# DethRaid/AndroidRenderer

Measured on AMD Instinct MI355X. Metric: lit Mpixels/sec (deferred+GI pass) at 4K, higher is better.
Workload: dtype f32

## Files before the change

androidrenderer_amd/_abi.py:

```python
import ctypes as C

SAH_OK = 0
SAH_ERR_INVALID_ARGUMENT = -1
SAH_ERR_UNSUPPORTED_FORMAT = -2
SAH_ERR_HIP = -3
SAH_ERR_NO_DEVICE = -4
SAH_ERR_COMM = -5
SAH_ERR_UNSUPPORTED = -6

FORMAT_R8_UNORM = 9
FORMAT_R8G8B8A8_UNORM = 37
FORMAT_R8G8B8A8_SRGB = 43
FORMAT_R16_SFLOAT = 76
FORMAT_R16G16_SFLOAT = 83
FORMAT_R16G16B16A16_SFLOAT = 97
FORMAT_R32_SFLOAT = 100
FORMAT_B10G11R11_UFLOAT_PACK32 = 122
FORMAT_D16_UNORM = 124
FORMAT_D32_SFLOAT = 126
FORMAT_R8_UINT = 13

FORMAT_BPP = {9: 1, 13: 1, 37: 4, 43: 4, 76: 2, 83: 4, 97: 8, 100: 4, 122: 4, 124: 2, 126: 4}

SHADOW_MODE_OFF, SHADOW_MODE_CSM, SHADOW_MODE_RT = 0, 1, 2
GI_NONE, GI_LPV, GI_CACHE, GI_RTGI = 0, 1, 2, 3
LIGHTING_QUIRK_SUN_BLEND = 1 << 0
LIGHTING_BRUTE_FORCE_LIGHTS = 1 << 1
LIGHTING_DEFAULT_FLAGS = LIGHTING_QUIRK_SUN_BLEND
MAX_BLOOM_MIPS = 8
TONEMAP_TOLERANCE_1CODE = 1 << 0
GENERATION_TRACKED = 0xFFFFFFFF


class Plane(C.Structure):
    _fields_ = [("ptr", C.c_void_p), ("width", C.c_uint32), ("height", C.c_uint32), ("row_pitch_bytes", C.c_uint32),
                ("format", C.c_uint32)]


class Volume(C.Structure):
    _fields_ = [("ptr", C.c_void_p), ("width", C.c_uint32), ("height", C.c_uint32), ("depth", C.c_uint32),
                ("row_pitch_bytes", C.c_uint32), ("slice_pitch_bytes", C.c_uint32), ("format", C.c_uint32)]


TAA_HISTORY_INVALID, TAA_HDR_WEIGHTS = 1, 2


class TaaParams(C.Structure):
    _fields_ = [("blend", C.c_float), ("jitter", C.c_float * 2), ("previous_jitter", C.c_float * 2), ("flags", C.c_uint32)]


class SsaoParams(C.Structure):
    _fields_ = [("radius", C.c_float), ("max_radius_pixels", C.c_float), ("shadow_multiplier", C.c_float), ("shadow_clamp", C.c_float),
                ("horizon_angle_threshold", C.c_float), ("fade_out_from", C.c_float), ("fade_out_to", C.c_float), ("edge_sharpness", C.c_float),
                ("blur_passes", C.c_uint32), ("flags", C.c_uint32)]

    @classmethod
    def default(cls, **changes):
        values = dict(radius=8.0, max_radius_pixels=32.0, shadow_multiplier=1.0, shadow_clamp=0.98, horizon_angle_threshold=0.06, fade_out_from=50.0,
                      fade_out_to=300.0, edge_sharpness=50.0, blur_passes=2, flags=0)
        values.update(changes)
        return cls(**values)


EXPOSURE_HISTORY_INVALID = 1


class ExposureParams(C.Structure):
    _fields_ = [("key", C.c_float), ("low_fraction", C.c_float), ("high_fraction", C.c_float), ("min_exposure", C.c_float), ("max_exposure", C.c_float),
                ("adaptation", C.c_float), ("max_workgroups", C.c_uint32), ("flags", C.c_uint32)]

    @classmethod
    def default(cls, **changes):
        values = dict(key=0.18, low_fraction=0.5, high_fraction=0.95, min_exposure=1.0 / 64.0, max_exposure=64.0, adaptation=1.0, max_workgroups=0, flags=0)
        values.update(changes)
        return cls(**values)


class ExposureState(C.Structure):
    _fields_ = [("exposure", C.c_float), ("adapted", C.c_float), ("metered", C.c_uint32), ("window", C.c_uint32)]


RT_DENOISE_HISTORY_INVALID = 1


class RtDenoiseParams(C.Structure):
    _fields_ = [("max_history", C.c_float), ("depth_tolerance", C.c_float), ("depth_sharpness", C.c_float), ("normal_squarings", C.c_uint32),
                ("passes", C.c_uint32), ("jitter", C.c_float * 2), ("previous_jitter", C.c_float * 2), ("flags", C.c_uint32)]

    @classmethod
    def default(cls, **changes):
        values = dict(max_history=32.0, depth_tolerance=0.1, depth_sharpness=50.0, normal_squarings=5, passes=3, jitter=(0.0, 0.0),
                      previous_jitter=(0.0, 0.0), flags=0)
        values.update(changes)
        for k in ("jitter", "previous_jitter"):
            values[k] = (C.c_float * 2)(*values[k])
        return cls(**values)


class RtDenoiseDesc(C.Structure):
    PLANES = ("noisy", "depth", "normals", "motion_vectors", "previous_depth", "history", "history_length", "accum_out", "length_out", "denoised")
    _fields_ = [(name, C.POINTER(Plane)) for name in PLANES]

    @classmethod
    def of(cls, **planes):
        unknown = set(planes) - set(cls.PLANES)
        if unknown:
            raise TypeError(f"not planes of sah_rt_denoise_desc: {sorted(unknown)}")
        self = cls()
        self._planes = dict(planes)
        for name, p in planes.items():
            if p is not None:
                setattr(self, name, C.pointer(p))
        return self


RTGI_DENOISE_HISTORY_INVALID = 1
FORMAT_R32G32_SFLOAT = 103
FORMAT_R32G32B32A32_SFLOAT = 109
FORMAT_BPP.update({FORMAT_R32G32_SFLOAT: 8, FORMAT_R32G32B32A32_SFLOAT: 16})


class RtgiDenoiseParams(C.Structure):
    _fields_ = [("max_history", C.c_float), ("min_history", C.c_float), ("depth_tolerance", C.c_float), ("depth_sharpness", C.c_float),
                ("normal_squarings", C.c_uint32), ("passes", C.c_uint32), ("luminance_sigma", C.c_float), ("luminance_floor", C.c_float),
                ("jitter", C.c_float * 2), ("previous_jitter", C.c_float * 2), ("flags", C.c_uint32)]

    @classmethod
    def default(cls, **changes):
        values = dict(max_history=32.0, min_history=4.0, depth_tolerance=0.1, depth_sharpness=50.0, normal_squarings=5, passes=3, luminance_sigma=4.0,
                      luminance_floor=1e-6, jitter=(0.0, 0.0), previous_jitter=(0.0, 0.0), flags=0)
        values.update(changes)
        for k in ("jitter", "previous_jitter"):
            values[k] = (C.c_float * 2)(*values[k])
        return cls(**values)


class RtgiDenoiseDesc(C.Structure):
    PLANES = ("ray_buffer", "ray_irradiance", "depth", "normals", "motion_vectors", "previous_depth", "history", "history_moments", "accum_out",
              "moments_out", "denoised_ray_buffer", "denoised_irradiance")
    _fields_ = [(name, C.POINTER(Plane)) for name in PLANES]

    @classmethod
    def of(cls, **planes):
        unknown = set(planes) - set(cls.PLANES)
        if unknown:
            raise TypeError(f"not planes of sah_rtgi_denoise_desc: {sorted(unknown)}")
        self = cls()
        self._planes = dict(planes)
        for name, p in planes.items():
            if p is not None:
                setattr(self, name, C.pointer(p))
        return self


class TaaUpscaleParams(C.Structure):
    _fields_ = [("blend", C.c_float), ("min_confidence", C.c_float), ("jitter", C.c_float * 2), ("previous_jitter", C.c_float * 2), ("flags", C.c_uint32)]


class ShadingRateParams(C.Structure):
    _fields_ = [("contrast_image_resolution", C.c_uint32 * 2), ("shading_rate_image_resolution", C.c_uint32 * 2), ("max_rate", C.c_uint32 * 2),
                ("num_shading_rates", C.c_uint32), ("rates", (C.c_uint32 * 2) * 8)]


class ProbeAtlases(C.Structure):
    _fields_ = [("rtgi", Volume), ("light_cache", Volume), ("depth", Volume), ("average", Volume), ("validity", Volume)]


PRIMITIVE_TYPE_SOLID, PRIMITIVE_TYPE_CUTOUT = 0, 1
RASTER_STATS_WORDS = 8
RT_STATS_WORDS = 4
IPC_HANDLE_BYTES = 128


class VertexData(C.Structure):
    _fields_ = [("normal", C.c_float * 3), ("tangent", C.c_float * 4), ("texcoord", C.c_float * 2), ("color", C.c_uint32)]


class Material(C.Structure):
    _fields_ = [("base_color_tint", C.c_float * 4), ("emission_factor", C.c_float * 4), ("metalness_factor", C.c_float),
                ("roughness_factor", C.c_float), ("opacity_threshold", C.c_float), ("padding1", C.c_float),
                ("base_color_texel", C.c_float * 4), ("normal_texel", C.c_float * 4), ("data_texel", C.c_float * 4),
                ("emission_texel", C.c_float * 4)]


class Primitive(C.Structure):
    _fields_ = [("model", C.c_float * 16), ("first_index", C.c_uint32), ("index_count", C.c_uint32), ("vertex_offset", C.c_int32),
                ("type", C.c_uint32), ("material", C.c_uint32), ("padding", C.c_uint32 * 3)]


FILTER_NEAREST, FILTER_LINEAR = 0, 1
ADDRESS_REPEAT, ADDRESS_MIRRORED_REPEAT, ADDRESS_CLAMP_TO_EDGE = 0, 1, 2
MAX_TEXTURE_MIPS = 14
TEXTURE_NONE = 0xFFFFFFFF


class Sampler(C.Structure):
    _fields_ = [("mag_filter", C.c_uint32), ("min_filter", C.c_uint32), ("mipmap_mode", C.c_uint32), ("address_u", C.c_uint32),
                ("address_v", C.c_uint32), ("mip_lod_bias", C.c_float), ("min_lod", C.c_float), ("max_lod", C.c_float),
                ("max_anisotropy", C.c_float), ("reserved", C.c_uint32)]


class Texture(C.Structure):
    _fields_ = [("mips", Plane * MAX_TEXTURE_MIPS), ("num_mips", C.c_uint32), ("padding", C.c_uint32), ("sampler", Sampler)]


class MaterialTextures(C.Structure):
    _fields_ = [("base_color", C.c_uint32), ("normal", C.c_uint32), ("data", C.c_uint32), ("emission", C.c_uint32)]


class SceneGeometry(C.Structure):
    _fields_ = [("vertex_positions", C.c_void_p), ("vertex_data", C.c_void_p), ("indices", C.c_void_p), ("primitives", C.c_void_p),
                ("materials", C.c_void_p), ("num_vertices", C.c_uint32), ("num_indices", C.c_uint32), ("num_primitives", C.c_uint32),
                ("num_materials", C.c_uint32), ("textures", C.c_void_p), ("material_textures", C.c_void_p), ("num_textures", C.c_uint32),
                ("padding", C.c_uint32)]


class RsmTargets(C.Structure):
    _fields_ = [("flux", Volume), ("normals", Volume), ("depth", Volume)]


class GBuffer(C.Structure):
    _fields_ = [("color", Plane), ("normals", Plane), ("data", Plane), ("emission", Plane), ("depth", Plane)]


class MipChain(C.Structure):
    _fields_ = [("mips", Plane * MAX_BLOOM_MIPS), ("num_mips", C.c_uint32)]


class ViewData(C.Structure):
    _fields_ = [("view", C.c_float * 16), ("projection", C.c_float * 16), ("inverse_view", C.c_float * 16),
                ("inverse_projection", C.c_float * 16), ("last_frame_view", C.c_float * 16),
                ("last_frame_projection", C.c_float * 16), ("frustum", C.c_float * 4), ("z_near", C.c_float),
                ("material_texture_mip_bias", C.c_float), ("render_resolution", C.c_float * 2), ("jitter", C.c_float * 2),
                ("previous_jitter", C.c_float * 2)]


class SunLightConstants(C.Structure):
    _fields_ = [("direction_and_tan_size", C.c_float * 4), ("color", C.c_float * 4), ("csm_resolution", C.c_uint32 * 4),
                ("data", (C.c_float * 4) * 4), ("cascade_matrices", (C.c_float * 16) * 4),
                ("cascade_inverse_matrices", (C.c_float * 16) * 4), ("shadow_mode", C.c_uint32),
                ("num_shadow_samples", C.c_float), ("padding1", C.c_uint32), ("padding2", C.c_uint32)]


class LpvCascadeMatrices(C.Structure):
    _fields_ = [("rsm_vp", C.c_float * 16), ("inverse_rsm_vp", C.c_float * 16), ("world_to_cascade", C.c_float * 16),
                ("cascade_to_world", C.c_float * 16)]


class ProbeCascade(C.Structure):
    _fields_ = [("min", C.c_float * 3), ("probe_spacing", C.c_float)]


class GI(C.Structure):
    _fields_ = [("kind", C.c_uint32),
                ("lpv_red", Volume), ("lpv_green", Volume), ("lpv_blue", Volume),
                ("lpv_cascades", C.POINTER(LpvCascadeMatrices)), ("lpv_num_cascades", C.c_uint32), ("lpv_exposure", C.c_float),
                ("probe_irradiance", Volume), ("probe_depth", Volume), ("probe_validity", Volume),
                ("probe_cascades", ProbeCascade * 4), ("probe_size", C.c_uint32 * 2), ("cache_debug_mode", C.c_uint32),
                ("ray_buffer", Plane), ("ray_irradiance", Plane), ("noise", Plane), ("num_extra_rays", C.c_uint32),
                ("extra_ray_radius", C.c_float), ("lpv_generation", C.c_uint32), ("probe_generation", C.c_uint32)]


class SkyLuts(C.Structure):
    _fields_ = [("transmittance", Plane), ("sky_view", Plane)]


class PointLight(C.Structure):
    _fields_ = [("position", C.c_float * 3), ("radius", C.c_float), ("color", C.c_float * 3), ("intensity", C.c_float)]


class LightList(C.Structure):
    _fields_ = [("lights", C.c_void_p), ("count", C.c_uint32)]


class LightingDesc(C.Structure):
    _fields_ = [("gbuffer", C.POINTER(GBuffer)), ("ao", C.POINTER(Plane)), ("lit", C.POINTER(Plane)),
                ("view", C.POINTER(ViewData)), ("sun", C.POINTER(SunLightConstants)), ("shadowmap", C.POINTER(Volume)),
                ("shadow_mask", C.POINTER(Plane)), ("lights", C.POINTER(LightList)), ("gi", C.POINTER(GI)),
                ("sky", C.POINTER(SkyLuts)), ("flags", C.c_uint32), ("row_begin", C.c_uint32), ("row_end", C.c_uint32)]


class ChainPlan(C.Structure):
    _fields_ = [("aa_rows", C.c_uint32 * 2), ("mip0_rows", C.c_uint32 * 2), ("mip1_rows", C.c_uint32 * 2), ("out_rows", C.c_uint32 * 2),
                ("mip1_rows_per_rank", C.c_uint32), ("mip1_allocated_rows", C.c_uint32), ("rows_per_rank", C.c_uint32),
                ("out_allocated_rows", C.c_uint32)]


class ChainFrame(C.Structure):
    _fields_ = [("lighting", C.POINTER(LightingDesc) * 2), ("lit", Plane), ("antialiased", Plane), ("bloom", MipChain), ("out", Plane)]


CHAIN_NO_EXCHANGE = 1 << 0
CHAIN_CAPTURE = 1 << 1

assert C.sizeof(ViewData) == 432
assert C.sizeof(SunLightConstants) == 640
assert C.sizeof(LpvCascadeMatrices) == 256
assert C.sizeof(ProbeCascade) == 16
assert C.sizeof(PointLight) == 32


class ProbeTraceDesc(C.Structure):
    _fields_ = [("cascades", ProbeCascade * 4), ("probes_to_update", C.c_void_p), ("num_probes", C.c_uint32),
                ("sun", C.POINTER(SunLightConstants)), ("sky", C.POINTER(SkyLuts)), ("noise", C.POINTER(Plane)),
                ("probe_irradiance", Volume), ("probe_depth", Volume), ("probe_validity", Volume), ("probe_size", C.c_uint32 * 2),
                ("trace_results", Volume)]
```

androidrenderer_amd/csrc/api.cpp:

```cpp
#include <dlfcn.h>
#include <hip/hip_runtime.h>

#include <cmath>
#include <cstdarg>
#include <cstdio>
#include <cstdlib>
#include <cstring>
#include <string>
#include <vector>

#include "../../include/sah_hip.h"
#include "ctx.hpp"
#include "fast_pixel_map.hpp"
#include "launch.hpp"

namespace {

bool vec_ok(const sah_plane* p, uint32_t bytes) { return ((uintptr_t)p->ptr % bytes) == 0 && (p->row_pitch_bytes % bytes) == 0; }

void normalize3(const float in[3], float out[3]) {
    const float d = in[0] * in[0] + in[1] * in[1] + in[2] * in[2];
    const float inv = 1.0f / std::sqrt(d);
    for (int i = 0; i < 3; i++) out[i] = in[i] * inv;
}
void cross3(const float a[3], const float b[3], float o[3]) {
    o[0] = a[1] * b[2] - b[1] * a[2];
    o[1] = a[2] * b[0] - b[2] * a[0];
    o[2] = a[0] * b[1] - b[0] * a[1];
}
float round_to_half(float f) { return (float)(_Float16)f; }

bool is_zero(float x) { return x == 0.0f; }
bool all_finite(const float* m, int n) {
    for (int i = 0; i < n; i++)
        if (!std::isfinite(m[i])) return false;
    return true;
}
bool all_bounded(const float* m, int n) {
    for (int i = 0; i < n; i++)
        if (!(std::fabs(m[i]) <= 0x1p+40f)) return false;
    return true;
}

}

namespace sah {
namespace {


enum DispatchField {
    kDispFamily, kDispPpt, kDispPosDivNr, kDispNcascPow2, kDispRowMagic, kDispSkyRatio, kDispSkyWorkgroups, kDispTiledFastGeom, kDispTiledFastLpv,
    kDispRepack, kDispTableRebuilt, kDispPosDivShared, kDispFields
};
static_assert(kDispFields == sizeof(sah_ctx::last_dispatch) / sizeof(uint32_t), "sah_debug_lighting_dispatch reports uint32_t[12]");

struct LightingCall {
    uint32_t W, H, r0, r1;
    uint32_t sun_mode, gi_kind;
    bool vec4ok;
};

int lighting_targets(sah_ctx* ctx, const sah_lighting_desc* d, LightingCall& call, LightingArgs& a) {
    if (!d->gbuffer || !d->lit || !d->view) return fail(ctx, SAH_ERR_INVALID_ARGUMENT, "gbuffer, lit and view are required");
    const sah_gbuffer& g = *d->gbuffer;
    const uint32_t W = d->lit->width, H = d->lit->height;
    if (W == 0 || H == 0) return fail(ctx, SAH_ERR_INVALID_ARGUMENT, "empty render target");
    if (!plane_ok(d->lit, SAH_FORMAT_R16G16B16A16_SFLOAT, SAH_FORMAT_R16G16B16A16_SFLOAT, W, H))
        return fail(ctx, SAH_ERR_UNSUPPORTED_FORMAT, "lit must be R16G16B16A16_SFLOAT");
    if (!plane_ok(&g.color, SAH_FORMAT_R8G8B8A8_SRGB, SAH_FORMAT_R8G8B8A8_SRGB, W, H) ||
        !plane_ok(&g.normals, SAH_FORMAT_R16G16B16A16_SFLOAT, SAH_FORMAT_R16G16B16A16_SFLOAT, W, H) ||
        !plane_ok(&g.data, SAH_FORMAT_R8G8B8A8_UNORM, SAH_FORMAT_R8G8B8A8_UNORM, W, H) ||
        !plane_ok(&g.emission, SAH_FORMAT_R8G8B8A8_SRGB, SAH_FORMAT_R8G8B8A8_SRGB, W, H) ||
        !plane_ok(&g.depth, SAH_FORMAT_D32_SFLOAT, SAH_FORMAT_R32_SFLOAT, W, H))
        return fail(ctx, SAH_ERR_UNSUPPORTED_FORMAT, "g-buffer planes must match the reference formats and the lit extent");
    uint32_t r0 = d->row_begin, r1 = d->row_end;
    if (r0 == 0 && r1 == 0) r1 = H;
    if (r1 > H || r0 > r1) return fail(ctx, SAH_ERR_INVALID_ARGUMENT, "row range [%u,%u) outside image height %u", r0, r1, H);

    const uint32_t sun_mode = d->sun ? d->sun->shadow_mode : SAH_SHADOW_MODE_OFF;
    if (sun_mode > SAH_SHADOW_MODE_RT) return fail(ctx, SAH_ERR_INVALID_ARGUMENT, "bad shadow_mode %u", sun_mode);
    const uint32_t gi_kind = d->gi ? d->gi->kind : SAH_GI_NONE;
    if (gi_kind > SAH_GI_RTGI) return fail(ctx, SAH_ERR_INVALID_ARGUMENT, "bad gi kind %u", gi_kind);
    if ((d->sky || d->lights) && !d->sun) return fail(ctx, SAH_ERR_INVALID_ARGUMENT, "sun constants are required with sky");

    memset(&a, 0, sizeof(a));
    a.color = parg(&g.color);
    a.normals = parg(&g.normals);
    a.data = parg(&g.data);
    a.emission = parg(&g.emission);
    a.depth = parg(&g.depth);
    a.lit = parg(d->lit);
    a.width = W;
    a.height = H;
    a.row_begin = r0;
    a.row_end = r1;
    a.flags = d->flags;
    a.res[0] = d->view->render_resolution[0];
    a.res[1] = d->view->render_resolution[1];
    memcpy(a.inv_proj, d->view->inverse_projection, 64);
    memcpy(a.inv_view, d->view->inverse_view, 64);
    for (int i = 0; i < 3; i++) a.view_pos[i] = -d->view->view[12 + i];
    a.luts = ctx->luts;
    if (d->sun) {
        const float neg[3] = {-d->sun->direction_and_tan_size[0], -d->sun->direction_and_tan_size[1], -d->sun->direction_and_tan_size[2]};
        normalize3(neg, a.sun_L);
        for (int i = 0; i < 3; i++) a.sun_color[i] = d->sun->color[i];
    }
    bool vec4ok = (W % 4 == 0) && vec_ok(&g.color, 16) && vec_ok(&g.normals, 16) && vec_ok(&g.data, 16) && vec_ok(&g.emission, 16) &&
                  vec_ok(&g.depth, 16) && vec_ok(d->lit, 16);

    if (gi_kind == SAH_GI_LPV && d->ao && d->ao->ptr) {
        if (!plane_ok(d->ao, SAH_FORMAT_R32_SFLOAT, SAH_FORMAT_R32_SFLOAT, W, H)) return fail(ctx, SAH_ERR_UNSUPPORTED_FORMAT, "ao must be R32_SFLOAT");
        a.ao = parg(d->ao);
        a.has_ao = 1;
        vec4ok = vec4ok && vec_ok(d->ao, 16);
    }
    if (sun_mode == SAH_SHADOW_MODE_RT && d->shadow_mask && d->shadow_mask->ptr) {
        if (!plane_ok(d->shadow_mask, SAH_FORMAT_R32_SFLOAT, SAH_FORMAT_R32_SFLOAT, W, H))
            return fail(ctx, SAH_ERR_UNSUPPORTED_FORMAT, "shadow_mask must be R32_SFLOAT");
        a.shadow_mask = parg(d->shadow_mask);
        a.has_mask = 1;
        vec4ok = vec4ok && vec_ok(d->shadow_mask, 16);
    }
    call = LightingCall{W, H, r0, r1, sun_mode, gi_kind, vec4ok};
    return SAH_OK;
}

int lighting_csm(sah_ctx* ctx, const sah_lighting_desc* d, const LightingCall& call, CsmArgs& csm) {
    memset(&csm, 0, sizeof(csm));
    if (call.sun_mode != SAH_SHADOW_MODE_CSM) return SAH_OK;
    if (d->shadowmap && d->shadowmap->ptr) {
        if (d->shadowmap->format != SAH_FORMAT_D16_UNORM && d->shadowmap->format != SAH_FORMAT_D32_SFLOAT)
            return fail(ctx, SAH_ERR_UNSUPPORTED_FORMAT, "shadowmap must be D16_UNORM or D32_SFLOAT");
        if (d->shadowmap->depth < 4) return fail(ctx, SAH_ERR_INVALID_ARGUMENT, "shadowmap needs 4 layers");
        csm.shadowmap = varg(*d->shadowmap);
        csm.is_d16 = d->shadowmap->format == SAH_FORMAT_D16_UNORM;
        csm.d16_recip = 1.0f / 65535.0f;
        static const bool recip_ok = [] {
            const float y = 1.0f / 65535.0f;
            for (uint32_t i = 0; i < 65536; i++) {
                const float v = (float)i;
                const float q = v * y;
                const float q2 = std::fmaf(std::fmaf(-q, 65535.0f, v), y, q);
                if (q2 != v / 65535.0f) return false;
            }
            return true;
        }();
        csm.d16_recip_ok = recip_ok;
    }
    for (int c = 0; c < 4; c++) {
        csm.splits[c] = d->sun->data[c][0];
        const float* M = d->sun->cascade_matrices[c];
        for (int col = 0; col < 4; col++) {
            const float* m = M + col * 4;
            csm.biased[c][col * 4 + 0] = ((0.5f * m[0] + 0.0f * m[1]) + 0.0f * m[2]) + 0.5f * m[3];
            csm.biased[c][col * 4 + 1] = ((0.0f * m[0] + 0.5f * m[1]) + 0.0f * m[2]) + 0.5f * m[3];
            csm.biased[c][col * 4 + 2] = ((0.0f * m[0] + 0.0f * m[1]) + 1.0f * m[2]) + 0.0f * m[3];
            csm.biased[c][col * 4 + 3] = ((0.0f * m[0] + 0.0f * m[1]) + 0.0f * m[2]) + 1.0f * m[3];
        }
    }
    return SAH_OK;
}

int lighting_gi_lpv(sah_ctx* ctx, const sah_lighting_desc* d, const LightingCall& call, LpvArgs& lpv) {
    memset(&lpv, 0, sizeof(lpv));
    if (call.gi_kind != SAH_GI_LPV) return SAH_OK;
    const sah_gi& gi = *d->gi;
    if (gi.lpv_num_cascades == 0 || gi.lpv_num_cascades > 4 || !gi.lpv_cascades)
        return fail(ctx, SAH_ERR_INVALID_ARGUMENT, "LPV needs 1..4 cascades and their matrices");
    const sah_volume* vols[3] = {&gi.lpv_red, &gi.lpv_green, &gi.lpv_blue};
    for (const sah_volume* v : vols) {
        if (!v->ptr || v->format != SAH_FORMAT_R16G16B16A16_SFLOAT) return fail(ctx, SAH_ERR_UNSUPPORTED_FORMAT, "LPV volumes must be RGBA16F");
        if ((uint64_t)v->row_pitch_bytes < (uint64_t)v->width * 8 || (uint64_t)v->slice_pitch_bytes < (uint64_t)v->row_pitch_bytes * v->height)
            return fail(ctx, SAH_ERR_INVALID_ARGUMENT, "LPV volume pitches too small");
    }
    lpv.red = varg(gi.lpv_red);
    lpv.green = varg(gi.lpv_green);
    lpv.blue = varg(gi.lpv_blue);
    for (uint32_t c = 0; c < gi.lpv_num_cascades; c++) memcpy(lpv.world_to_cascade[c], gi.lpv_cascades[c].world_to_cascade, 64);
    lpv.num_cascades = gi.lpv_num_cascades;
    lpv.num_cascades_f = (float)gi.lpv_num_cascades;
    lpv.exposure = gi.lpv_exposure;
    return SAH_OK;
}

int lighting_irr32_copy(sah_ctx* ctx, const sah_gi& gi, CacheArgs& cache) {
    if (cache.hot_ok) {
        const size_t need = 4 * (size_t)((uint64_t)gi.probe_irradiance.slice_pitch_bytes * gi.probe_irradiance.depth);
        const hipError_t ge = ctx->irr32_copy.reserve(ctx->stream, ctx->cache_epoch, need);
        if (ge == hipErrorOutOfMemory) {
            (void)hipGetLastError();
            cache.hot_ok = 0;
        } else {
            HIP_TRY(ctx, ge);
        }
    }
    if (cache.hot_ok) {
        if (!ctx->irr32_copy.reusable_for(gi.probe_generation, cache.irradiance)) {
            HIP_TRY(ctx, launch_probe_irr_unpack(cache.irradiance, ctx->irr32_copy.data(), ctx->stream));
            ctx->dbg_irr_unpacks++;
            ctx->irr32_copy.rebuilt(ctx->cache_epoch, gi.probe_generation, cache.irradiance);
        }
        cache.irr32 = ctx->irr32_copy.data();
    }
    return SAH_OK;
}

int lighting_gi_cache(sah_ctx* ctx, const sah_lighting_desc* d, const LightingCall& call, CacheArgs& cache) {
    memset(&cache, 0, sizeof(cache));
    if (call.gi_kind != SAH_GI_CACHE) return SAH_OK;
    const sah_gi& gi = *d->gi;
    if (!gi.probe_irradiance.ptr || gi.probe_irradiance.format != SAH_FORMAT_B10G11R11_UFLOAT_PACK32 || !gi.probe_depth.ptr ||
        gi.probe_depth.format != SAH_FORMAT_R16G16_SFLOAT || !gi.probe_validity.ptr || gi.probe_validity.format != SAH_FORMAT_R8_UNORM)
        return fail(ctx, SAH_ERR_UNSUPPORTED_FORMAT, "probe atlases must be B10G11R11 / R16G16F / R8_UNORM arrays");
    cache.irradiance = varg(gi.probe_irradiance);
    cache.depth = varg(gi.probe_depth);
    cache.validity = varg(gi.probe_validity);
    for (int c = 0; c < 4; c++) {
        const float ext[3] = {32.f, 8.f, 32.f};
        for (int i = 0; i < 3; i++) {
            cache.cascade_min[c][i] = gi.probe_cascades[c].min[i];
            cache.cascade_max[c][i] = gi.probe_cascades[c].min[i] + ext[i] * gi.probe_cascades[c].probe_spacing;
        }
        cache.spacing[c] = gi.probe_cascades[c].probe_spacing;
    }
    cache.spacing_pow2 = 1;
    for (int c = 0; c < 4; c++) {
        int e = 0;
        const float sp = cache.spacing[c], m = frexpf(sp, &e);
        cache.spacing_pow2 = cache.spacing_pow2 && m == 0.5f && e > -60 && e < 60;
        cache.inv_spacing[c] = 1.0f / sp;
    }
    cache.probe_size[0] = gi.probe_size[0];
    cache.probe_size[1] = gi.probe_size[1];
    for (int i = 0; i < 2; i++) cache.inv_tex[i] = 1.0f / (((float)gi.probe_size[i] + 2.0f) * 32.0f);
    cache.debug_mode = gi.cache_debug_mode;
    auto bytes = [](const sah_volume& v) { return (uint64_t)v.slice_pitch_bytes * v.depth; };
    cache.hot_ok = bytes(gi.probe_irradiance) < (1ull << 32) && bytes(gi.probe_depth) < (1ull << 32) && bytes(gi.probe_validity) < (1ull << 32) &&
                   gi.probe_validity.width <= 32 && gi.probe_validity.height <= 32 && gi.probe_validity.depth <= 32 &&
                   gi.probe_size[0] >= 1 && gi.probe_size[0] <= 30 && gi.probe_size[1] >= 1 && gi.probe_size[1] <= 30 &&
                   gi.probe_irradiance.width == 32u * (gi.probe_size[0] + 2u) && gi.probe_irradiance.height == 32u * (gi.probe_size[1] + 2u) &&
                   gi.probe_depth.width == 32u * 12u && gi.probe_depth.height == 32u * 12u &&
                   bytes(gi.probe_irradiance) < (1ull << 30) && gi.probe_irradiance.row_pitch_bytes % 4 == 0 && gi.probe_irradiance.slice_pitch_bytes % 4 == 0 &&
                   ((uintptr_t)gi.probe_irradiance.ptr % 4) == 0;
    return lighting_irr32_copy(ctx, gi, cache);
}

int lighting_gi_rtgi(sah_ctx* ctx, const sah_lighting_desc* d, const LightingCall& call, RtgiArgs& rtgi) {
    memset(&rtgi, 0, sizeof(rtgi));
    if (call.gi_kind != SAH_GI_RTGI) return SAH_OK;
    const sah_gi& gi = *d->gi;
    if (!plane_ok(&gi.ray_buffer, SAH_FORMAT_R16G16B16A16_SFLOAT, SAH_FORMAT_R16G16B16A16_SFLOAT, call.W, call.H) ||
        !plane_ok(&gi.ray_irradiance, SAH_FORMAT_R16G16B16A16_SFLOAT, SAH_FORMAT_R16G16B16A16_SFLOAT, call.W, call.H))
        return fail(ctx, SAH_ERR_UNSUPPORTED_FORMAT, "ray_buffer / ray_irradiance must be RGBA16F at render resolution");
    rtgi.ray_buffer = parg(&gi.ray_buffer);
    rtgi.ray_irradiance = parg(&gi.ray_irradiance);
    if (gi.num_extra_rays) {
        if (!gi.noise.ptr || gi.noise.format != SAH_FORMAT_R8G8B8A8_UNORM || gi.noise.width < 128 || gi.noise.height < 128)
            return fail(ctx, SAH_ERR_UNSUPPORTED_FORMAT, "noise must be R8G8B8A8_UNORM, at least 128x128");
        rtgi.noise = parg(&gi.noise);
        rtgi.noise_w = gi.noise.width;
        rtgi.noise_h = gi.noise.height;
    }
    rtgi.num_extra_rays = gi.num_extra_rays;
    rtgi.extra_ray_radius = gi.extra_ray_radius;
    return SAH_OK;
}

int lighting_sky(sah_ctx* ctx, const sah_lighting_desc* d, SkyArgs& sky) {
    memset(&sky, 0, sizeof(sky));
    if (!d->sky) return SAH_OK;
    const float dirn[3] = {d->sun->direction_and_tan_size[0], d->sun->direction_and_tan_size[1], d->sun->direction_and_tan_size[2]};
    float nd[3];
    normalize3(dirn, nd);
    const float sun_dir[3] = {-nd[0], -nd[1], -nd[2]};
    if (!fill_sky_args(*d->sky, sun_dir, &sky)) return fail(ctx, SAH_ERR_UNSUPPORTED_FORMAT, "sky LUTs must be RGBA16F");
    return SAH_OK;
}

int lighting_ppt(const sah_ctx* ctx, const LightingCall& call) {
    const uint32_t W = call.W;
    int ppt = call.vec4ok ? 4 : 1;
    while (ppt > 1 && (uint64_t)(W / (uint32_t)ppt) * (call.r1 - call.r0) < 1536ull * 256ull) ppt /= 2;
    if (ctx->force_ppt == 1 || ctx->force_ppt == 2 || ctx->force_ppt == 4) {
        if (ctx->force_ppt == 1 || (call.vec4ok && W % ctx->force_ppt == 0)) ppt = ctx->force_ppt;
    }
    return ppt;
}


bool fast_view_ok(const sah_lighting_desc* d, FastArgs* f) {
    const float* P = d->view->inverse_projection;
    const float* V = d->view->inverse_view;
    if (!all_finite(P, 16) || !all_finite(V, 16)) return false;
    if (!std::isfinite(d->view->render_resolution[0]) || !std::isfinite(d->view->render_resolution[1])) return false;
    if (!(is_zero(P[4]) && is_zero(P[8]) && is_zero(P[1]) && is_zero(P[9]) && is_zero(P[2]) && is_zero(P[6]) && is_zero(P[3]) && is_zero(P[7])))
        return false;
    if (!(is_zero(V[3]) && is_zero(V[7]) && is_zero(V[11]) && V[15] == 1.0f)) return false;
    if (!all_bounded(d->view->view + 12, 3)) return false;
    f->p0 = P[0]; f->p12 = P[12]; f->p5 = P[5]; f->p13 = P[13];
    f->p10 = P[10]; f->p14 = P[14]; f->p11 = P[11]; f->p15 = P[15];
    auto in = [](float v, float lo, float hi) { return std::fabs(v) >= lo && std::fabs(v) <= hi; };
    const float r0 = d->view->render_resolution[0], r1 = d->view->render_resolution[1];
    const bool bounded = P[10] == 0.0f && P[12] == 0.0f && P[13] == 0.0f && in(P[0], 0x1p-16f, 0x1p+30f) && in(P[5], 0x1p-16f, 0x1p+30f) &&
                         in(P[14], 0x1p-40f, 0x1p+40f) && r0 > 0.f && r1 > 0.f && (float)d->lit->width <= 256.0f * r0 &&
                         (float)d->lit->height <= 256.0f * r1;
    f->pos_div_nr = bounded && !std::signbit(P[12]) && !std::signbit(P[13]);
    f->pos_div_shared = bounded && !f->pos_div_nr;
    return true;
}

bool fast_csm_ok(const CsmArgs& csm) {
    if (!csm.shadowmap.ptr || (uint64_t)csm.shadowmap.slice_pitch * csm.shadowmap.depth >= (1ull << 32)) return false;
    if (!csm.is_d16 || !csm.d16_recip_ok) return false;
    for (int c = 0; c < 4; c++) {
        const float* b = csm.biased[c];
        if (!all_bounded(b, 16)) return false;
        if (!(is_zero(b[3]) && is_zero(b[7]) && is_zero(b[11]) && b[15] == 1.0f)) return false;
    }
    return true;
}

bool fast_lpv_ok(const sah_gi& gi, FastArgs* f) {
    if (gi.lpv_red.width != gi.lpv_green.width || gi.lpv_red.width != gi.lpv_blue.width || gi.lpv_red.height != gi.lpv_green.height ||
        gi.lpv_red.height != gi.lpv_blue.height || gi.lpv_red.depth != gi.lpv_green.depth || gi.lpv_red.depth != gi.lpv_blue.depth ||
        gi.lpv_red.row_pitch_bytes != gi.lpv_green.row_pitch_bytes || gi.lpv_red.row_pitch_bytes != gi.lpv_blue.row_pitch_bytes ||
        gi.lpv_red.slice_pitch_bytes != gi.lpv_green.slice_pitch_bytes || gi.lpv_red.slice_pitch_bytes != gi.lpv_blue.slice_pitch_bytes ||
        (uint64_t)gi.lpv_red.slice_pitch_bytes * gi.lpv_red.depth >= (1ull << 32))
        return false;
    for (uint32_t c = 0; c < gi.lpv_num_cascades; c++) {
        const float* m = gi.lpv_cascades[c].world_to_cascade;
        if (!all_bounded(m, 16)) return false;
        if (!(is_zero(m[1]) && is_zero(m[2]) && is_zero(m[3]) && is_zero(m[4]) && is_zero(m[6]) && is_zero(m[7]) && is_zero(m[8]) &&
              is_zero(m[9]) && is_zero(m[11]) && m[15] == 1.0f))
            return false;
        if (is_zero(m[0]) || is_zero(m[5]) || is_zero(m[10])) return false;
        f->lpv_s[c][0] = m[0]; f->lpv_s[c][1] = m[5]; f->lpv_s[c][2] = m[10];
        f->lpv_t[c][0] = m[12]; f->lpv_t[c][1] = m[13]; f->lpv_t[c][2] = m[14];
    }
    const uint32_t n = gi.lpv_num_cascades;
    f->ncasc_pow2 = (n & (n - 1)) == 0;
    f->inv_ncasc = 1.0f / (float)n;
    return std::isfinite(gi.lpv_exposure);
}

struct FastPath {
    bool use_fast;
    bool tiled_fast_geom;
    bool tiled_fast_lpv;
    LightingFamily family;
};
FastPath detect_fast_path(const sah_ctx* ctx, const sah_lighting_desc* d, const LightingCall& call, const LightingArgs& a, const CsmArgs& csm, FastArgs* f) {
    memset(f, 0, sizeof(*f));
    const bool lpv_gi = call.gi_kind == SAH_GI_LPV;
    const bool fast_kind = (call.gi_kind == SAH_GI_NONE || lpv_gi) && a.num_lights == 0;
    const bool geom = !ctx->force_general && fast_view_ok(d, f) && (call.sun_mode != SAH_SHADOW_MODE_CSM || fast_csm_ok(csm));
    const bool lpv = geom && lpv_gi && (fast_kind || ctx->state) && fast_lpv_ok(*d->gi, f);
    FastPath p;
    p.use_fast = fast_kind && geom && (!lpv_gi || lpv);
    p.family = !fast_kind ? kLightingTiled : (p.use_fast ? kLightingFast : kLightingGeneral);
    p.tiled_fast_geom = !fast_kind && geom;
    p.tiled_fast_lpv = p.tiled_fast_geom && lpv;
    f->lpv_fast = p.tiled_fast_lpv ? 1u : 0u;
    return p;
}

int prepare_lpv_copy(sah_ctx* ctx, const sah_lighting_desc* d, const LpvArgs& lpv, FastArgs& fast) {
    SahLpvCopy& copy = ctx->lpv_copy;
    const SahLpvPackLayout pk = SahLpvCopy::layout(lpv.red.width, lpv.red.height, lpv.red.depth);
    if (pk.total >= (1ull << 32)) return fail(ctx, SAH_ERR_UNSUPPORTED, "LPV volumes too large for the packed gather copy");
    HIP_TRY(ctx, copy.reserve(ctx->stream, ctx->cache_epoch, pk.total));
    fast.lpv_packed = copy.data();
    fast.pk_row_pitch = pk.row_pitch;
    fast.pk_slice_pitch = pk.slice_pitch;
    const VolumeArg src[3] = {lpv.red, lpv.green, lpv.blue};
    const uint32_t gen = d->gi->lpv_generation;
    const bool reuse = copy.reusable_for(gen, src);
    fast.repack = reuse ? 0u : 1u;
    if (!reuse) {
        ctx->dbg_lpv_packs++;
        copy.rebuilt_by_pack(ctx->cache_epoch, gen, src, lpv.red.width, lpv.red.height, lpv.red.depth);
    }
    return SAH_OK;
}

int lighting_fast_layout(sah_ctx* ctx, const sah_lighting_desc* d, const LightingCall& call, int ppt, const LpvArgs& lpv, const SkyArgs& sky, FastArgs& fast) {
    const uint32_t W = call.W, r0 = call.r0, r1 = call.r1;
    const uint64_t groups = (uint64_t)(W / (uint32_t)ppt) * (r1 - r0);
    const uint32_t nseg = (uint32_t)((groups + 63) / 64);
    const uint32_t seg_stride = 64u * (uint32_t)ppt;
    const size_t codes_bytes = ((size_t)nseg * seg_stride + 255) & ~(size_t)255;
    const size_t need = codes_bytes + (size_t)nseg * sizeof(uint16_t) + 256;
    HIP_TRY(ctx, ctx->list.grow_in_epoch(ctx->stream, ctx->cache_epoch, need));
    fast.seg_list = (uint8_t*)ctx->list.ptr;
    fast.seg_count = (uint16_t*)((uint8_t*)ctx->list.ptr + codes_bytes);
    fast.num_segments = nseg;
    fast.seg_stride = seg_stride;
    if (call.gi_kind == SAH_GI_LPV && r1 > r0) {
        if (const int rc = prepare_lpv_copy(ctx, d, lpv, fast); rc != SAH_OK) return rc;
    }
    fast.sky_enabled = sky.enabled;
    {
        const uint64_t blocks = (groups + 255) / 256;
        const uint64_t want = (blocks + 511) / 512;
        fast.sky_ratio = (uint32_t)(want < 4 ? 4 : (want > 32 ? 32 : want));
        fast.sky_first = sky.enabled ? (uint32_t)((blocks + fast.sky_ratio - 1u) / fast.sky_ratio) : 0u;
    }
    {
        const uint64_t gpr = W / (uint32_t)ppt, threads = (gpr * (r1 - r0) + 255) / 256 * 256;
        fast.row_magic = (gpr >= 2 && threads * gpr < (1ull << 32)) ? (uint32_t)((1ull << 32) / gpr) + 1u : 0u;
    }
    fast.tile_rows = fast_tile_rows_for(call.sun_mode == SAH_SHADOW_MODE_CSM || call.gi_kind == SAH_GI_LPV, W, r1 - r0, (uint32_t)ppt);
    fast.state = ctx->state;
    fast.hint_slot = ctx->hint_slot;
    ctx->hint_slot ^= 1u;
    return SAH_OK;
}

int lighting_colx_table(sah_ctx* ctx, const LightingCall& call, const LightingArgs& a, const FastPath& path, int ppt, FastArgs& fast, bool* table_rebuilt) {
    const uint32_t W = call.W, H = call.H;
    const bool lit_px = call.sun_mode != SAH_SHADOW_MODE_OFF || call.gi_kind == SAH_GI_LPV;
    const bool geom_fast = path.use_fast && (call.sun_mode == SAH_SHADOW_MODE_CSM || call.gi_kind == SAH_GI_LPV);
    *table_rebuilt = false;
    if ((path.use_fast && ppt == 4 && lit_px) || (geom_fast && fast.pos_div_shared) || path.tiled_fast_geom) {
        const struct {
            float f[7];
            uint32_t width;
        } key = {{a.res[0], fast.p0, fast.p12, a.res[1], fast.p5, fast.p13, (float)H}, W};
        const uint32_t stride = (W + 63u) & ~63u, row_stride = (H + 63u) & ~63u;
        HIP_TRY(ctx, ctx->colx.prepare(ctx->stream, ctx->cache_epoch, ((size_t)2 * stride + 2 * row_stride) * sizeof(float), &key, sizeof(key), true, table_rebuilt));
        fast.state = ctx->state;
        if (*table_rebuilt) {
            HIP_TRY(ctx, launch_colx_table(a, fast, (float*)ctx->colx.buf.ptr, stride, row_stride, ctx->stream));
            ctx->colx.built(ctx->cache_epoch, &key, sizeof(key));
        }
        fast.colx_tab = (const float*)ctx->colx.buf.ptr;
        fast.colx_stride = stride;
        fast.rowy_stride = row_stride;
    }
    if (!fast.colx_tab || !ctx->state || !(geom_fast || path.tiled_fast_geom)) fast.pos_div_shared = 0u;
    return SAH_OK;
}

void lighting_report(sah_ctx* ctx, const LightingCall& call, const FastPath& path, int ppt, const FastArgs& fast, bool table_rebuilt) {
    uint32_t* w = ctx->last_dispatch;
    w[kDispFamily] = path.family;
    w[kDispPpt] = path.family == kLightingTiled ? 0u : (uint32_t)ppt;
    w[kDispPosDivNr] = (path.use_fast || path.tiled_fast_geom) ? fast.pos_div_nr : 0u;
    w[kDispNcascPow2] = ((path.use_fast && call.gi_kind == SAH_GI_LPV) || path.tiled_fast_lpv) ? fast.ncasc_pow2 : 0u;
    w[kDispRowMagic] = (path.use_fast && fast.row_magic != 0u) ? 1u : 0u;
    w[kDispSkyRatio] = path.use_fast ? fast.sky_ratio : 0u;
    w[kDispSkyWorkgroups] = path.use_fast ? fast.sky_first : 0u;
    w[kDispTiledFastGeom] = path.tiled_fast_geom ? 1u : 0u;
    w[kDispTiledFastLpv] = path.tiled_fast_lpv ? 1u : 0u;
    w[kDispRepack] = fast.repack;
    w[kDispTableRebuilt] = table_rebuilt ? 1u : 0u;
    w[kDispPosDivShared] = fast.pos_div_shared;
}

}
}

void SahRange::resolve(push_fn& push, pop_fn& pop) {
    const char* on = getenv("SAH_ROCTX");
    if (!on || atoi(on) == 0) return;
    for (const char* lib : {"librocprofiler-sdk-roctx.so", "librocprofiler-sdk-roctx.so.1", "libroctx64.so", "libroctx64.so.4"}) {
        void* h = dlopen(lib, RTLD_NOW | RTLD_GLOBAL);
        if (!h) continue;
        push = reinterpret_cast<push_fn>(dlsym(h, "roctxRangePushA"));
        pop = reinterpret_cast<pop_fn>(dlsym(h, "roctxRangePop"));
        if (push && pop) return;
        push = nullptr;
        pop = nullptr;
    }
}

extern "C" {

int sah_abi_version(void) { return SAH_ABI_VERSION; }

const char* sah_status_string(int s) {
    switch (s) {
        case SAH_OK: return "ok";
        case SAH_ERR_INVALID_ARGUMENT: return "invalid argument";
        case SAH_ERR_UNSUPPORTED_FORMAT: return "unsupported format";
        case SAH_ERR_HIP: return "HIP error";
        case SAH_ERR_NO_DEVICE: return "no HIP device";
        case SAH_ERR_COMM: return "communicator error";
        case SAH_ERR_UNSUPPORTED: return "unsupported";
    }
    return "unknown";
}

const char* sah_last_error(const sah_ctx* ctx) { return ctx ? ctx->last_error.c_str() : ""; }

int sah_comm_init(sah_ctx* ctx, const void* comm_id);
void sah_comm_destroy(sah_ctx* ctx);
void sah_ipc_destroy(sah_ctx* ctx);

int sah_create(sah_ctx** out, int device, int rank, int world, const void* comm_id) {
    if (!out || world < 1 || rank < 0 || rank >= world) return SAH_ERR_INVALID_ARGUMENT;
    *out = nullptr;
    int n = 0;
    if (hipGetDeviceCount(&n) != hipSuccess || n == 0) return SAH_ERR_NO_DEVICE;
    if (device < 0 || device >= n) return SAH_ERR_INVALID_ARGUMENT;
    sah_ctx* ctx = new sah_ctx();
    ctx->device = device;
    ctx->rank = rank;
    ctx->world = world;
    if (hipSetDevice(device) != hipSuccess) { delete ctx; return SAH_ERR_HIP; }
    if (hipStreamCreateWithFlags(&ctx->stream, hipStreamNonBlocking) != hipSuccess) { delete ctx; return SAH_ERR_HIP; }
    ctx->own_stream = true;
    float host[512];
    for (int i = 0; i < 256; i++) {
        const double c = (double)i / 255.0;
        host[i] = (float)((c <= 0.04045) ? c / 12.92 : std::pow((c + 0.055) / 1.055, 2.4));
        host[256 + i] = (float)i / 255.0f;
    }
    if (hipMalloc((void**)&ctx->luts, sizeof(host)) != hipSuccess ||
        hipMemcpy(ctx->luts, host, sizeof(host), hipMemcpyHostToDevice) != hipSuccess) {
        sah_destroy(ctx);
        return SAH_ERR_HIP;
    }
    if (comm_id) {
        int rc = sah_comm_init(ctx, comm_id);
        if (rc != SAH_OK) { sah_destroy(ctx); return rc; }
    }
    if (hipMalloc((void**)&ctx->state, sizeof(sah::FrameState)) != hipSuccess ||
        hipMemset(ctx->state, 0, sizeof(sah::FrameState)) != hipSuccess) {
        sah_destroy(ctx);
        return SAH_ERR_HIP;
    }
    if (ctx->mip_chain_counter.create() != hipSuccess) {
        sah_destroy(ctx);
        return SAH_ERR_HIP;
    }
    const char* mc = getenv("SAH_RASTER_MERGE_CAPACITY");
    if (mc) ctx->raster_merge_cap = (uint32_t)atoi(mc);
    *out = ctx;
    return SAH_OK;
}

int sah_debug_create_detached(sah_ctx** out) {
    if (!out) return SAH_ERR_INVALID_ARGUMENT;
    *out = nullptr;
    int n = 0;
    if (hipGetDeviceCount(&n) == hipSuccess && n > 0) return SAH_ERR_UNSUPPORTED;
    (void)hipGetLastError();
    sah_ctx* ctx = new sah_ctx();
    ctx->device = -1;
    *out = ctx;
    return SAH_OK;
}

void sah_destroy(sah_ctx* ctx) {
    if (!ctx) return;
    (void)hipSetDevice(ctx->device);
    sah_comm_destroy(ctx);
    sah_ipc_destroy(ctx);
    if (ctx->comm_ready) (void)hipEventDestroy(ctx->comm_ready);
    if (ctx->comm_done) (void)hipEventDestroy(ctx->comm_done);
    if (ctx->luts) (void)hipFree(ctx->luts);
    if (ctx->probe_slots) (void)hipFree(ctx->probe_slots);
    if (ctx->probe_done) (void)hipEventDestroy(ctx->probe_done);
    if (ctx->state) (void)hipFree(ctx->state);
    std::vector<SahBuffer*> buffers = {&ctx->list, &ctx->lpv_copy.buf, &ctx->gv_keys, &ctx->gv_factors, &ctx->ml_scratch, &ctx->irr32_copy.buf, &ctx->colx.buf, &ctx->tm_axis.buf};
    for (SahBuffer& b : ctx->raster.buf) buffers.push_back(&b);
    for (SahBuffer& b : ctx->rt.buf) buffers.push_back(&b);
    for (SahBuffer* b : buffers) b->release();
    ctx->tm_codes.release();
    ctx->mip_chain_counter.release();
    for (SahCacheGuard* g : {&ctx->guard_lighting, &ctx->guard_tonemap, &ctx->guard_raster, &ctx->guard_rt, &ctx->guard_mip_chain})
        if (g->done) (void)hipEventDestroy(g->done);
    if (ctx->raster.half_to_srgb8) (void)hipFree(ctx->raster.half_to_srgb8);
    if (ctx->raster.host_counters) (void)hipHostFree(ctx->raster.host_counters);
    if (ctx->own_stream && ctx->stream) (void)hipStreamDestroy(ctx->stream);
    delete ctx;
}

int sah_set_stream(sah_ctx* ctx, void* hip_stream) {
    if (!ctx) return SAH_ERR_INVALID_ARGUMENT;
    if ((hipStream_t)hip_stream == ctx->stream && !ctx->own_stream) return SAH_OK;
    const bool drained = ctx->own_stream && ctx->stream;
    if (drained) (void)hipStreamSynchronize(ctx->stream);
    SahCacheGuard* guards[] = {&ctx->guard_lighting, &ctx->guard_tonemap, &ctx->guard_raster, &ctx->guard_rt, &ctx->guard_mip_chain};
    for (SahCacheGuard* g : guards) HIP_TRY(ctx, sah_guard_leave(ctx, *g, drained));
    if (drained) (void)hipStreamDestroy(ctx->stream);
    ctx->stream = (hipStream_t)hip_stream;
    ctx->own_stream = false;
    return SAH_OK;
}

void* sah_get_stream(sah_ctx* ctx) { return ctx ? (void*)ctx->stream : nullptr; }

int sah_debug_set(sah_ctx* ctx, int force_general, int force_ppt) {
    if (!ctx) return SAH_ERR_INVALID_ARGUMENT;
    ctx->force_general = force_general != 0;
    ctx->force_ppt = force_ppt;
    return SAH_OK;
}

int sah_debug_deferred_pixels(sah_ctx* ctx, uint64_t* out) {
    if (!ctx || !out) return SAH_ERR_INVALID_ARGUMENT;
    *out = 0;
    if (!ctx->last_seg_count || !ctx->last_num_segments) return SAH_OK;
    HIP_TRY(ctx, hipSetDevice(ctx->device));
    HIP_TRY(ctx, hipStreamSynchronize(ctx->stream));
    std::vector<uint16_t> counts(ctx->last_num_segments);
    HIP_TRY(ctx, hipMemcpy(counts.data(), ctx->last_seg_count, counts.size() * sizeof(uint16_t), hipMemcpyDeviceToHost));
    uint64_t n = 0;
    for (uint16_t c : counts) n += c;
    *out = n;
    return SAH_OK;
}

int sah_debug_copy_rebuilds(sah_ctx* ctx, uint32_t out[2]) {
    if (!ctx || !out) return SAH_ERR_INVALID_ARGUMENT;
    out[0] = ctx->dbg_lpv_packs;
    out[1] = ctx->dbg_irr_unpacks;
    return SAH_OK;
}

int sah_debug_cache_epoch(sah_ctx* ctx, uint64_t* out) {
    if (!ctx || !out) return SAH_ERR_INVALID_ARGUMENT;
    *out = ctx->cache_epoch;
    return SAH_OK;
}

int sah_debug_lighting_dispatch(sah_ctx* ctx, uint32_t out[12]) {
    if (!ctx || !out) return SAH_ERR_INVALID_ARGUMENT;
    memcpy(out, ctx->last_dispatch, sizeof(ctx->last_dispatch));
    if (out[sah::kDispPosDivShared] && ctx->state) {
        uint32_t neg_zero = 0;
        HIP_TRY(ctx, hipSetDevice(ctx->device));
        HIP_TRY(ctx, hipStreamSynchronize(ctx->stream));
        HIP_TRY(ctx, hipMemcpy(&neg_zero, &ctx->state->colx_neg_zero, sizeof(neg_zero), hipMemcpyDeviceToHost));
        out[sah::kDispPosDivShared] = neg_zero == 0u ? 1u : 0u;
    }
    return SAH_OK;
}

int sah_sync(sah_ctx* ctx) {
    if (!ctx) return SAH_ERR_INVALID_ARGUMENT;
    HIP_TRY(ctx, hipStreamSynchronize(ctx->stream));
    if (ctx->comm_stream && ctx->comm_stream != ctx->stream) HIP_TRY(ctx, hipStreamSynchronize(ctx->comm_stream));
    if (sah_ipc_timed_out(ctx)) return fail(ctx, SAH_ERR_COMM, "direct exchange: a peer did not arrive within 2 s; the gathered rows are not valid");
    return SAH_OK;
}

int sah_lighting(sah_ctx* ctx, const sah_lighting_desc* d) {
    SAH_RANGE();
    using namespace sah;
    if (!ctx || !d) return SAH_ERR_INVALID_ARGUMENT;
    memset(ctx->last_dispatch, 0, sizeof(ctx->last_dispatch));
    LightingCall call;
    LightingArgs a;
    CsmArgs csm;
    LpvArgs lpv;
    CacheArgs cache;
    RtgiArgs rtgi;
    SkyArgs sky;
    if (const int rc = lighting_targets(ctx, d, call, a); rc != SAH_OK) return rc;
    if (const int rc = lighting_csm(ctx, d, call, csm); rc != SAH_OK) return rc;
    if (const int rc = lighting_gi_lpv(ctx, d, call, lpv); rc != SAH_OK) return rc;
    if (const int rc = lighting_gi_cache(ctx, d, call, cache); rc != SAH_OK) return rc;
    if (const int rc = lighting_gi_rtgi(ctx, d, call, rtgi); rc != SAH_OK) return rc;
    if (const int rc = lighting_sky(ctx, d, sky); rc != SAH_OK) return rc;
    const int ppt = lighting_ppt(ctx, call);
    if (d->lights && d->lights->count) {
        if (!d->lights->lights) return fail(ctx, SAH_ERR_INVALID_ARGUMENT, "light list pointer is null");
        a.lights = d->lights->lights;
        a.num_lights = d->lights->count;
    }
    HIP_TRY(ctx, hipSetDevice(ctx->device));
    HIP_TRY(ctx, sah_guard_touch(ctx, ctx->guard_lighting));
    FastArgs fast;
    const FastPath path = detect_fast_path(ctx, d, call, a, csm, &fast);
    if (path.tiled_fast_lpv && call.r1 > call.r0) {
        if (const int rc = prepare_lpv_copy(ctx, d, lpv, fast); rc != SAH_OK) return rc;
        fast.state = ctx->state;
    }
    if (path.use_fast) {
        if (const int rc = lighting_fast_layout(ctx, d, call, ppt, lpv, sky, fast); rc != SAH_OK) return rc;
    }
    bool table_rebuilt = false;
    if (const int rc = lighting_colx_table(ctx, call, a, path, ppt, fast, &table_rebuilt); rc != SAH_OK) return rc;
    lighting_report(ctx, call, path, ppt, fast, table_rebuilt);
    HIP_TRY(ctx, launch_lighting(a, csm, lpv, cache, rtgi, sky, path.family, (path.use_fast || path.tiled_fast_geom) ? &fast : nullptr, (int)call.sun_mode,
                                 (int)call.gi_kind, ppt, (d->flags & SAH_LIGHTING_BRUTE_FORCE_LIGHTS) != 0, ctx->stream));
    if (path.use_fast) {
        ctx->last_seg_count = fast.seg_count;
        ctx->last_num_segments = fast.num_segments;
    } else {
        ctx->last_seg_count = nullptr;
        ctx->last_num_segments = 0;
    }
    return SAH_OK;
}

}
```

androidrenderer_amd/csrc/ctx.hpp:

```cpp
#pragma once
#include <hip/hip_runtime.h>

#include <cstdarg>
#include <cstdio>
#include <string>
#include <vector>

#include "../../include/sah_hip.h"
#include "ctx_cache.hpp"
#include "params.hpp"
#include "rt_args.hpp"

struct SahCacheGuard {
    hipEvent_t done = nullptr;
    hipStream_t last = nullptr;
    bool used = false, closed = false;
};

struct sah_ctx {
    int device = 0;
    int rank = 0, world = 1;
    hipStream_t stream = nullptr;
    bool own_stream = false;
    float* luts = nullptr;
    uint32_t* probe_slots = nullptr;
    hipEvent_t probe_done = nullptr;
    hipStream_t probe_stream = nullptr;
    bool lpv_tables_built = false;
    bool lpv_hot_structure = false;
    void* comm = nullptr;
    void* comm_reversed = nullptr;
    void* rccl = nullptr;
    hipStream_t comm_stream = nullptr;
    hipEvent_t comm_ready = nullptr, comm_done = nullptr;
    bool comm_pending = false;
    int force_ppt = 0;
    bool force_general = false;
    sah::FrameState* state = nullptr;
    SahBuffer list;
    SahBuffer gv_keys;
    SahBuffer gv_factors;
    SahBuffer ml_scratch;
    SahLpvCopy lpv_copy;
    SahIrr32Copy irr32_copy;
    SahKeyedTable colx;
    SahKeyedTable tm_axis;
    SahTonemapCodeTables tm_codes;
    SahTicketCounter mip_chain_counter;
    uint64_t cache_epoch = 0;
    uint32_t hint_slot = 0;
    uint32_t dbg_lpv_packs = 0, dbg_irr_unpacks = 0;
    const uint16_t* last_seg_count = nullptr;
    uint32_t last_num_segments = 0;
    uint32_t last_dispatch[12] = {};
    struct RasterScratch {
        SahBuffer buf[16];
        uint8_t* half_to_srgb8 = nullptr;
        uint32_t* host_counters = nullptr;
        uint32_t last_pass[4] = {};
    } raster;
    struct RtState {
        SahBuffer buf[7];
        sah::RtBvh bvh = {};
        sah::RtScene scene = {};
        bool built = false;
        bool refitted = false;
        uint32_t row_begin = 0, row_end = 0;
        uint32_t num_bounces = 0;
    } rt;
    struct IpcState {
        bool open = false, connected = false;
        uint32_t* mailbox = nullptr;
        uint32_t* peer_mailbox[SAH_IPC_MAX_WORLD] = {};
        uint32_t* timed_out = nullptr;
        struct Mapping {
            unsigned char handle[64];
            void* base;
            uint32_t users;
        };
        std::vector<Mapping> mappings;
        struct Buffer {
            bool in_use = false;
            uint8_t* local = nullptr;
            uint64_t bytes = 0;
            uint8_t* peer[SAH_IPC_MAX_WORLD] = {};
            unsigned char peer_handle[SAH_IPC_MAX_WORLD][SAH_IPC_HANDLE_BYTES] = {};
            uint32_t seq = 0;
        } buffers[SAH_IPC_MAX_BUFFERS];
    } ipc;
    SahCacheGuard guard_lighting, guard_tonemap, guard_raster, guard_rt, guard_mip_chain;
    uint32_t raster_merge_cap = 2048;
    std::string last_error;
};

struct SahRange {
    using push_fn = int (*)(const char*);
    using pop_fn = int (*)();
    static void resolve(push_fn& push, pop_fn& pop);
    explicit SahRange(const char* name) {
        static push_fn push = nullptr;
        static pop_fn pop_ = nullptr;
        static bool tried = false;
        if (!tried) {
            tried = true;
            resolve(push, pop_);
        }
        pop = pop_;
        if (push) push(name);
    }
    ~SahRange() {
        if (pop) pop();
    }
    pop_fn pop = nullptr;
};
#define SAH_RANGE() SahRange sah_range_(__func__)

inline int fail(sah_ctx* ctx, int code, const char* fmt, ...) {
    char buf[512];
    va_list ap;
    va_start(ap, fmt);
    vsnprintf(buf, sizeof(buf), fmt, ap);
    va_end(ap);
    if (ctx) ctx->last_error = buf;
    return code;
}

inline hipError_t sah_guard_touch(sah_ctx* ctx, SahCacheGuard& g) {
    hipError_t e = hipSuccess;
    if (g.used && g.closed && g.last != ctx->stream) e = hipStreamWaitEvent(ctx->stream, g.done, 0);
    g.used = true;
    g.closed = false;
    g.last = ctx->stream;
    return e;
}
inline hipError_t sah_guard_leave(sah_ctx* ctx, SahCacheGuard& g, bool drained) {
    if (!g.used || g.closed || g.last != ctx->stream) return hipSuccess;
    if (drained) {
        g.used = false;
        return hipSuccess;
    }
    hipError_t e = hipSuccess;
    if (!g.done) e = hipEventCreateWithFlags(&g.done, hipEventDisableTiming);
    if (e == hipSuccess) e = hipEventRecord(g.done, ctx->stream);
    g.closed = e == hipSuccess;
    return e;
}

#define HIP_TRY(ctx, expr)                                                                          \
    do {                                                                                            \
        hipError_t e_ = (expr);                                                                     \
        if (e_ != hipSuccess) return fail(ctx, SAH_ERR_HIP, "%s: %s", #expr, hipGetErrorString(e_)); \
    } while (0)

inline bool fill_sky_args(const sah_sky_luts& s, const float sun_dir[3], sah::SkyArgs* sky) {
    if (!s.transmittance.ptr || !s.sky_view.ptr || s.transmittance.format != SAH_FORMAT_R16G16B16A16_SFLOAT || s.sky_view.format != SAH_FORMAT_R16G16B16A16_SFLOAT)
        return false;
    auto cross3 = [](const float a[3], const float b[3], float o[3]) {
        o[0] = a[1] * b[2] - b[1] * a[2];
        o[1] = a[2] * b[0] - b[2] * a[0];
        o[2] = a[0] * b[1] - b[0] * a[1];
    };
    sky->enabled = 1;
    sky->transmittance = sah::PlaneArg{(const uint8_t*)s.transmittance.ptr, s.transmittance.row_pitch_bytes};
    sky->sky_view = sah::PlaneArg{(const uint8_t*)s.sky_view.ptr, s.sky_view.row_pitch_bytes};
    sky->t_w = s.transmittance.width;
    sky->t_h = s.transmittance.height;
    sky->s_w = s.sky_view.width;
    sky->s_h = s.sky_view.height;
    const float sky_pi = 3.14159265358f;
    const float ground = 6.360f;
    for (int i = 0; i < 3; i++) sky->sun_dir[i] = sun_dir[i];
    sky->view_pos_y = 6.360f + 0.0002f;
    sky->height = __builtin_sqrtf((0.0f * 0.0f + sky->view_pos_y * sky->view_pos_y) + 0.0f * 0.0f);
    sky->up_y = sky->view_pos_y / sky->height;
    {
        float q = __builtin_sqrtf(sky->height * sky->height - ground * ground) / sky->height;
        q = __builtin_fminf(__builtin_fmaxf(q, -1.0f), 1.0f);
        sky->horizon_angle = (float)__builtin_acos((double)q);
    }
    sky->azimuth_limit = 0.5f * sky_pi - .0001f;
    sky->min_sun_cos = (float)__builtin_cos((double)(0.53f * sky_pi / 180.0f));
    const float up[3] = {0.0f / sky->height, sky->up_y, 0.0f / sky->height};
    cross3(sky->sun_dir, up, sky->right);
    cross3(up, sky->right, sky->forward);
    sky->smooth_e0 = (float)(_Float16)0.002f;
    return true;
}

inline uint32_t format_bpp(uint32_t f) {
    switch (f) {
        case SAH_FORMAT_R8_UNORM: return 1;
        case SAH_FORMAT_R16_SFLOAT: case SAH_FORMAT_D16_UNORM: return 2;
        case SAH_FORMAT_R8G8B8A8_UNORM: case SAH_FORMAT_R8G8B8A8_SRGB: case SAH_FORMAT_R16G16_SFLOAT: case SAH_FORMAT_R32_SFLOAT:
        case SAH_FORMAT_B10G11R11_UFLOAT_PACK32: case SAH_FORMAT_D32_SFLOAT: return 4;
        case SAH_FORMAT_R16G16B16A16_SFLOAT: return 8;
    }
    return 0;
}

inline bool plane_ok(const sah_plane* p, uint32_t fmt_a, uint32_t fmt_b, uint32_t w, uint32_t h) {
    if (!p || !p->ptr) return false;
    if (p->format != fmt_a && p->format != fmt_b) return false;
    if (p->width != w || p->height != h) return false;
    return (uint64_t)p->row_pitch_bytes >= (uint64_t)w * format_bpp(p->format);
}

inline bool rgba16f_ok(const sah_plane* p) {
    return p && p->ptr && p->format == SAH_FORMAT_R16G16B16A16_SFLOAT && p->width && p->height &&
           (uint64_t)p->row_pitch_bytes >= (uint64_t)p->width * 8 && ((uintptr_t)p->ptr % 8) == 0 && (p->row_pitch_bytes % 8) == 0;
}

inline sah::PlaneArg parg(const sah_plane* p) { return sah::PlaneArg{p ? (const uint8_t*)p->ptr : nullptr, p ? p->row_pitch_bytes : 0}; }
inline sah::VolumeArg varg(const sah_volume& v) {
    return sah::VolumeArg{(const uint8_t*)v.ptr, v.width, v.height, v.depth, v.row_pitch_bytes, v.slice_pitch_bytes};
}
```

androidrenderer_amd/csrc/ctx_cache.hpp:

```cpp
#pragma once
#include <hip/hip_runtime.h>

#include <cstring>

#include "../../include/sah_hip.h"
#include "params.hpp"

inline bool same_volume(const sah::VolumeArg& a, const sah::VolumeArg& b) {
    return a.ptr == b.ptr && a.width == b.width && a.height == b.height && a.depth == b.depth && a.row_pitch == b.row_pitch && a.slice_pitch == b.slice_pitch;
}

struct SahBuffer {
    void* ptr = nullptr;
    size_t bytes = 0;

    hipError_t grow(hipStream_t stream, size_t need, bool* grew = nullptr) {
        if (grew) *grew = false;
        if (bytes >= need) return hipSuccess;
        if (ptr) {
            const hipError_t e = hipStreamSynchronize(stream);
            if (e != hipSuccess) return e;
            (void)hipFree(ptr);
        }
        ptr = nullptr;
        bytes = 0;
        const hipError_t e = hipMalloc(&ptr, need);
        if (e != hipSuccess) return e;
        bytes = need;
        if (grew) *grew = true;
        return hipSuccess;
    }
    hipError_t grow_in_epoch(hipStream_t stream, uint64_t& cache_epoch, size_t need) {
        bool grew = false;
        const hipError_t e = grow(stream, need, &grew);
        if (grew) cache_epoch++;
        return e;
    }
    void release() {
        if (ptr) (void)hipFree(ptr);
        ptr = nullptr;
        bytes = 0;
    }
};

struct SahLpvPackLayout {
    uint32_t row_pitch, slice_pitch;
    uint64_t total;
};

struct SahLpvCopy {
    SahBuffer buf;
    uint32_t generation = 0;
    sah::VolumeArg source[3] = {};
    uint32_t extent[3] = {0, 0, 0};
    bool all_zero = false;

    uint8_t* data() const { return (uint8_t*)buf.ptr; }

    static SahLpvPackLayout layout(uint32_t w, uint32_t h, uint32_t d) {
        const uint64_t row = (uint64_t)(w + 2 * sah::kLpvPackBorder) * sah::kLpvPackTexel;
        const uint64_t slice = row * (h + 2 * sah::kLpvPackBorder);
        return {(uint32_t)row, (uint32_t)slice, slice * (d + 2 * sah::kLpvPackBorder) + 64};
    }
    void drop(uint64_t& cache_epoch) {
        if (generation != 0) cache_epoch++;
        generation = 0;
    }
    hipError_t reserve(hipStream_t stream, uint64_t& cache_epoch, uint64_t total) {
        if (buf.bytes >= total) return hipSuccess;
        const hipError_t e = buf.grow(stream, total);
        if (e != hipSuccess && buf.ptr) return e;
        generation = 0;
        cache_epoch++;
        if (e != hipSuccess) return e;
        extent[0] = extent[1] = extent[2] = 0;
        all_zero = true;
        return hipMemsetAsync(buf.ptr, 0, total, stream);
    }
    bool reusable_for(uint32_t gen, const sah::VolumeArg src[3]) const {
        return gen != 0 && gen == generation && same_volume(src[0], source[0]) && same_volume(src[1], source[1]) && same_volume(src[2], source[2]);
    }
    void rebuilt_by_pack(uint64_t& cache_epoch, uint32_t gen, const sah::VolumeArg src[3], uint32_t w, uint32_t h, uint32_t d) {
        if (gen != 0) cache_epoch++;
        generation = gen;
        for (int i = 0; i < 3; i++) source[i] = src[i];
        extent[0] = w, extent[1] = h, extent[2] = d;
        all_zero = false;
    }
    hipError_t borders_for(hipStream_t stream, uint32_t w, uint32_t h, uint32_t d, uint64_t total) {
        const bool same = extent[0] == w && extent[1] == h && extent[2] == d;
        hipError_t e = hipSuccess;
        if (!same && !all_zero) e = hipMemsetAsync(buf.ptr, 0, total, stream);
        extent[0] = w, extent[1] = h, extent[2] = d;
        all_zero = false;
        return e;
    }
    struct Rewrite {
        uint32_t generation;
        uint64_t epoch;
        sah::VolumeArg source[3];
    };
    Rewrite begin_rewrite(uint64_t& cache_epoch) {
        const Rewrite was = {generation, cache_epoch, {source[0], source[1], source[2]}};
        drop(cache_epoch);
        return was;
    }
    void commit_rewrite(uint64_t& cache_epoch, const Rewrite& was, const sah::VolumeArg* last) {
        if (last) {
            generation = SAH_GENERATION_TRACKED;
            for (int i = 0; i < 3; i++) source[i] = last[i];
        }
        bool same = last && was.generation == SAH_GENERATION_TRACKED;
        for (int i = 0; i < 3 && same; i++) same = same_volume(was.source[i], last[i]);
        if (same && cache_epoch == was.epoch + 1) cache_epoch = was.epoch;
        else if (!same && last && was.generation == 0) cache_epoch++;
    }
};

struct SahIrr32Copy {
    SahBuffer buf;
    uint32_t generation = 0;
    sah::VolumeArg source = {};

    uint8_t* data() const { return (uint8_t*)buf.ptr; }

    void drop(uint64_t& cache_epoch) {
        if (generation != 0) cache_epoch++;
        generation = 0;
    }
    hipError_t reserve(hipStream_t stream, uint64_t& cache_epoch, size_t need) {
        bool grew = false;
        const hipError_t e = buf.grow(stream, need, &grew);
        if (grew) {
            generation = 0;
            cache_epoch++;
        }
        return e;
    }
    bool reusable_for(uint32_t gen, const sah::VolumeArg& atlas) const { return gen != 0 && gen == generation && same_volume(atlas, source); }
    void rebuilt(uint64_t& cache_epoch, uint32_t gen, const sah::VolumeArg& atlas) {
        if (gen != 0) cache_epoch++;
        generation = gen;
        source = atlas;
    }
    bool patchable_for(const sah::VolumeArg& atlas) const { return buf.ptr && generation == SAH_GENERATION_TRACKED && same_volume(atlas, source); }
};

struct SahKeyedTable {
    SahBuffer buf;
    uint32_t key[20] = {};
    bool valid = false;

    hipError_t prepare(hipStream_t stream, uint64_t& cache_epoch, size_t need, const void* k, size_t k_bytes, bool new_buffer_in_epoch, bool* rebuild) {
        static_assert(sizeof(key) >= 7 * sizeof(float) + sizeof(uint32_t) && sizeof(key) >= 19 * sizeof(uint32_t), "the two keys in use");
        bool grew = false;
        const hipError_t e = buf.grow(stream, need, &grew);
        if (grew) {
            valid = false;
            if (new_buffer_in_epoch) cache_epoch++;
        }
        *rebuild = !valid || memcmp(k, key, k_bytes) != 0;
        return e;
    }
    void built(uint64_t& cache_epoch, const void* k, size_t k_bytes) {
        cache_epoch++;
        memcpy(key, k, k_bytes);
        valid = true;
    }
};

struct SahTicketCounter {
    uint32_t* word = nullptr;

    hipError_t create() {
        const hipError_t e = hipMalloc((void**)&word, sizeof(uint32_t));
        return e != hipSuccess ? e : hipMemset(word, 0, sizeof(uint32_t));
    }
    void release() {
        if (word) (void)hipFree(word);
        word = nullptr;
    }
};

struct SahTonemapCodeTables {
    float* thresholds = nullptr;
    float* code_table = nullptr;
    uint32_t bucket_base = 0, bucket_count = 0;
    float thr_lo = 0.f, thr_hi = 0.f;

    bool ready() const { return thresholds && code_table; }
    void publish(uint64_t& cache_epoch, float* d_thresholds, float* d_code_table, uint32_t base, uint32_t count, float lo, float hi) {
        release();
        thresholds = d_thresholds;
        cache_epoch++;
        code_table = d_code_table;
        bucket_base = base;
        bucket_count = count;
        thr_lo = lo;
        thr_hi = hi;
    }
    void release() {
        if (thresholds) (void)hipFree(thresholds);
        if (code_table) (void)hipFree(code_table);
        thresholds = code_table = nullptr;
    }
};
```

androidrenderer_amd/csrc/launch.hpp:

```cpp
#pragma once
#include <hip/hip_runtime.h>
#include <stdint.h>

#include "../../include/sah_exposure.h"
#include "../../include/sah_hip.h"
#include "../../include/sah_mip_chain.h"
#include "../../include/sah_rt_denoise.h"
#include "../../include/sah_rtgi_denoise.h"
#include "../../include/sah_ssao.h"
#include "../../include/sah_taa.h"
#include "../../include/sah_taa_upscale.h"
#include "../../include/sah_vrsaa.h"
#include "params.hpp"
#include "post_args.hpp"
#include "raster_args.hpp"
#include "rt_args.hpp"

struct sah_ctx;

namespace sah {

hipError_t launch_lighting(const LightingArgs& a, const CsmArgs& csm, const LpvArgs& lpv, const CacheArgs& cache, const RtgiArgs& rtgi,
                           const SkyArgs& sky, LightingFamily family, const FastArgs* fast, int sun_mode, int gi, int ppt, bool brute_force_lights,
                           hipStream_t st);
hipError_t launch_lighting_tiled(const LightingArgs& a, const CsmArgs& csm, const LpvArgs& lpv, const CacheArgs& cache, const RtgiArgs& rtgi,
                                 const SkyArgs& sky, int sun_mode, int gi, bool brute_force_lights, const FastArgs* fast, hipStream_t st);
hipError_t launch_colx_table(const LightingArgs& a, const FastArgs& f, float* out, uint32_t stride, uint32_t row_stride, hipStream_t st);
hipError_t launch_probe_irr_unpack(const VolumeArg& src, uint8_t* dst, hipStream_t st);
hipError_t launch_probe_irr_unpack_probes(const VolumeArg& src, uint8_t* dst, const uint32_t* probes, uint32_t num_probes, hipStream_t st);

hipError_t launch_copy_scene(const PlaneArg& src, uint32_t sw, uint32_t sh, const PlaneArg& dst, uint32_t dw, uint32_t dh, uint32_t row_begin,
                             uint32_t row_end, hipStream_t st);
hipError_t launch_bloom_downsample(const PlaneArg& src, uint32_t sw, uint32_t sh, const PlaneArg& dst, uint32_t dw, uint32_t dh, uint32_t row_begin,
                                   uint32_t row_end, hipStream_t st);
bool launch_copy_bloom_mip0(const PlaneArg& lit, uint32_t lw, uint32_t lh, const PlaneArg& aa, uint32_t aw, uint32_t ah, const PlaneArg& mip0, uint32_t mw, uint32_t mh,
                            uint32_t mip_row_begin, uint32_t mip_row_end, uint32_t aa_row_begin, uint32_t aa_row_end, hipStream_t st, hipError_t* err);
bool launch_bloom_pair(const PlaneArg& s, uint32_t sw, uint32_t sh, const PlaneArg& a, uint32_t aw, uint32_t ah, const PlaneArg& b, uint32_t bw, uint32_t bh,
                       hipStream_t st, hipError_t* err);
hipError_t launch_fill_r32f(const PlaneArg& dst, uint32_t w, uint32_t h, float value, hipStream_t st);
hipError_t launch_tonemap(const TonemapArgs& t, hipStream_t st);
hipError_t launch_tonemap_tol(const TonemapArgs& t, hipStream_t st);
hipError_t launch_tonemap_axis_tables(const TonemapArgs& t, TmAxis* out, hipStream_t st);
hipError_t launch_sky_luts(const PlaneArg& transmittance, const PlaneArg& multiscattering, const PlaneArg& sky_view, const float light_vector[3], hipStream_t st);

hipError_t launch_vrsaa_contrast(const PlaneArg& color, const PlaneArg& depth, const PlaneArg& out, uint32_t w, uint32_t h, uint32_t row_begin,
                                 uint32_t row_end, const float* luts, hipStream_t st);
hipError_t launch_vrsaa_shading_rate(const PlaneArg& contrast, uint32_t cw, uint32_t ch, const PlaneArg& out, uint32_t sw, uint32_t sh, uint32_t d,
                                     const sah_shading_rate_params& params, hipStream_t st);

struct TaaArgs {
    PlaneArg lit, depth, mv, history, out;
    uint32_t W, H, row_begin, row_end;
    float blend, djx, djy;
};
hipError_t launch_taa_resolve(const TaaArgs& a, bool history, bool hdr_weights, hipStream_t st);

struct TaaUpscaleArgs {
    PlaneArg lit, depth, mv, history, out;
    uint32_t w, h, W, H, row_begin, row_end;
    float blend, min_confidence, jx, jy, djx, djy;
    float sx, sy, rx, ry;
};
hipError_t launch_taa_upscale(const TaaUpscaleArgs& a, bool history, bool hdr_weights, hipStream_t st);

struct SsaoArgs {
    PlaneArg depth, normals, raw, out;
    uint32_t W, H;
    uint32_t raw_begin, raw_end;
    uint32_t row_begin, row_end;
    float m[9];
    float p20, p21, ipx, ipy, tx, ty;
    float sx, rs, z_near;
    float max_radius_pixels, threshold, shadow_multiplier, shadow_clamp, fade_to, fade_span, edge_sharpness;
};
hipError_t launch_ssao(const SsaoArgs& a, uint32_t blur_passes, hipStream_t st);

struct ExposureArgs {
    PlaneArg scene, out;
    uint32_t W, H;
    uint32_t row_begin, row_end;
    uint32_t tiles_x, tiles;
    uint32_t* work;
    const sah_exposure_state* state_in;
    sah_exposure_state* state_out;
    float key, low_fraction, high_fraction, min_exposure, max_exposure, adaptation;
    bool history;
};
hipError_t launch_exposure_meter(const ExposureArgs& a, bool apply, uint32_t max_workgroups, hipStream_t st);
hipError_t launch_exposure_apply(const ExposureArgs& a, hipStream_t st);

struct RtDenoiseArgs {
    PlaneArg noisy, depth, normals, mv, prev_depth, history, hist_len, accum, length, out;
    uint32_t W, H;
    uint32_t acc_begin, acc_end;
    uint32_t row_begin, row_end;
    float iv[12];
    float l2[4];
    float p20, p21, ipx, ipy, tx, ty;
    float z_near, djx, djy;
    float max_history, depth_tolerance, depth_sharpness;
    uint32_t normal_squarings;
};
hipError_t launch_rt_denoise(const RtDenoiseArgs& a, uint32_t passes, bool history, hipStream_t st);

struct RtgiDenoiseArgs {
    PlaneArg rays, irr, depth, normals, mv, prev_depth, history, hist_mom, accum, moments, out_rays, out_irr;
    uint32_t W, H;
    uint32_t acc_begin, acc_end;
    uint32_t row_begin, row_end;
    float iv[12];
    float l2[4];
    float p20, p21, ipx, ipy, tx, ty;
    float z_near, djx, djy;
    float max_history, min_history, depth_tolerance, depth_sharpness, luminance_sigma, luminance_floor;
    uint32_t normal_squarings;
};
hipError_t launch_rtgi_denoise(const RtgiDenoiseArgs& a, uint32_t passes, bool history, hipStream_t st);

struct MipChainArgs {
    PlaneArg src;
    uint32_t src_w, src_h;
    float inv_w, inv_h;
    PlaneArg slot[SAH_MIP_CHAIN_MAX_LEVELS];
    uint32_t slot_w[SAH_MIP_CHAIN_MAX_LEVELS], slot_h[SAH_MIP_CHAIN_MAX_LEVELS];
    uint32_t mips, num_workgroups;
    uint32_t* counter;
};
enum MipChainKind : int { kMipChainR32Min = 0, kMipChainR16 = 1, kMipChainRGBA16 = 2, kMipChainR11G11B10 = 3 };
hipError_t launch_mip_chain(const MipChainArgs& a, MipChainKind kind, hipStream_t st);

hipError_t launch_lpv_clear(const VolumeArg* vols, int n, uint32_t num_cascades, hipStream_t st);
hipError_t launch_lpv_build_tables(hipStream_t st, bool* hot_structure);
hipError_t launch_lpv_propagate(const VolumeArg src[3], const VolumeArg dst[3], uint32_t num_cascades, const LpvPackEmit* emit, bool hot, hipStream_t st,
                                const LpvGvStep* gv = nullptr);
hipError_t launch_lpv_gv_factors(const VolumeArg& gv, void* factors, uint32_t num_cascades, hipStream_t st);
hipError_t launch_gv_inject_rsm(const VolumeArg& normals, const VolumeArg& depth, const sah_lpv_cascade_matrices* cascades, uint32_t first_cascade,
                                uint32_t cascade_count, uint32_t num_cascades, const VolumeArg& gv, uint32_t* keys, hipStream_t st);
hipError_t launch_gv_inject_scene(const PlaneArg& depth, const PlaneArg& normals, uint32_t width, uint32_t height, const sah_view_data& view,
                                  const sah_lpv_cascade_matrices* cascades, uint32_t num_cascades, const VolumeArg& gv, uint32_t* keys, hipStream_t st);
hipError_t launch_extract_vpls(const VolumeArg& flux, const VolumeArg& normals, const VolumeArg& depth, const sah_lpv_cascade_matrices& c, uint32_t cascade,
                               float grid_cell_size, const float* luts, sah_packed_vpl* list, uint32_t* count, void* scratch, hipStream_t st);
hipError_t launch_inject_vpls(const sah_packed_vpl* list, const uint32_t* count, uint32_t capacity, const sah_lpv_cascade_matrices& c, uint32_t cascade,
                              uint32_t num_cascades, const VolumeArg rgb[3], uint32_t* cells_scratch, hipStream_t st);

hipError_t launch_probe_copy(const ProbeAtlasArgs& src, const ProbeAtlasArgs& dst, const float movement[4][3], hipStream_t st);
hipError_t launch_probe_update(const ProbeAtlasArgs& atl, const VolumeArg& trace, const uint32_t* probes, uint32_t num_probes, uint32_t* slots,
                               hipStream_t st);

hipError_t launch_raster_setup(const RasterArgs& a, hipStream_t st);
void launch_raster_fill_bins(const RasterArgs& a, hipStream_t st);
hipError_t launch_raster_tiles(const RasterArgs& a, hipStream_t st);

hipError_t launch_rt_scan(const sah_primitive* prims, uint32_t n, uint32_t* tri_base, RtBuildState* st, hipStream_t s);
hipError_t launch_rt_world(const RtScene& sc, const uint32_t* tri_base, uint32_t total, RtTriangle* out, RtBuildState* st, hipStream_t s);
hipError_t launch_rt_sort(const RtTriangle* tris, const RtBuildState* st, unsigned long long* keys, uint32_t padded, hipStream_t s);
hipError_t launch_rt_nodes(const RtTriangle* unsorted, const unsigned long long* keys, RtTriangle* sorted, RtNodeGroup* nodes, const RtBvh& bvh, hipStream_t s);
hipError_t launch_rtao(const RtaoArgs& a, const RtBvh& bvh, const RtScene& sc, hipStream_t s);
hipError_t launch_sun_shadow_mask(const ShadowMaskArgs& a, const RtBvh& bvh, const RtScene& sc, hipStream_t s);
hipError_t launch_noise_dirs(const PlaneArg& noise, const float* luts, float* out, hipStream_t s);
hipError_t launch_probe_trace(const ProbeTraceArgs& a, const RtBvh& bvh, const RtScene& sc, hipStream_t s);
hipError_t launch_rtgi_trace(const RtgiTraceArgs& a, const RtBvh& bvh, const RtScene& sc, hipStream_t s);

hipError_t launch_rt_refit(const RtScene& sc, const RtBvh& bvh, RtTriangle* tris, RtNodeGroup* nodes, RtBuildState* st, uint32_t* stats, hipStream_t s);

struct IpcPeers {
    uint32_t* slot[SAH_IPC_MAX_WORLD];
};
struct IpcCopies {
    uint8_t* dst[SAH_IPC_MAX_WORLD];
};
hipError_t launch_ipc_signal(const IpcPeers& peers, uint32_t value, const uint32_t* abort, hipStream_t st);
hipError_t launch_ipc_wait(const IpcPeers& own, uint32_t value, uint32_t* abort, uint32_t* timed_out, const IpcPeers& notes, hipStream_t st);
hipError_t launch_ipc_copy(const IpcCopies& c, int world, const uint8_t* src, uint64_t bytes, const uint32_t* abort, const uint32_t* gave_up, hipStream_t st);

}

int sah_ipc_find(const sah_ctx* ctx, const void* ptr, uint64_t bytes);
int sah_ipc_gather(sah_ctx* ctx, uint32_t id, uint8_t* buffer, uint64_t bytes_per_rank, bool reversed, hipStream_t st);
bool sah_ipc_timed_out(const sah_ctx* ctx);
```

androidrenderer_amd/csrc/lighting.hip:

```cpp
#include <hip/hip_runtime.h>

#include <type_traits>

#include "../../include/sah_hip.h"
#include "fast_pixel_map.hpp"
#include "lighting_common.hpp"
#include "lighting_fast.hpp"
#include "launch.hpp"
#include "numerics.hpp"
#include "params.hpp"

namespace sah {

template <int SUN, int GI, int PPT>
__global__ void __launch_bounds__(256) k_lighting_general(const LightingArgs a, const CsmArgs csm, const LpvArgs lpv, const SkyArgs sky) {
    __shared__ float s_lut[512];
    stage_format_tables(s_lut, a.luts);
    __syncthreads();

    const uint32_t groups_per_row = a.width / PPT;
    const uint32_t gid = blockIdx.x * 256u + threadIdx.x;
    const uint32_t rows = a.row_end - a.row_begin;
    if (gid >= groups_per_row * rows) return;
    const uint32_t ry = gid / groups_per_row;
    const uint32_t y = a.row_begin + ry;
    const uint32_t x0 = (gid - ry * groups_per_row) * PPT;

    uint32_t wc[PPT], wd[PPT], we[PPT], wz[PPT], wn[2 * PPT], wao[PPT], wm[PPT];
    load_words<PPT>(a.color.ptr + (size_t)y * a.color.pitch + (size_t)x0 * 4, wc);
    load_words<PPT>(a.data.ptr + (size_t)y * a.data.pitch + (size_t)x0 * 4, wd);
    load_words<PPT>(a.emission.ptr + (size_t)y * a.emission.pitch + (size_t)x0 * 4, we);
    load_words<PPT>(a.depth.ptr + (size_t)y * a.depth.pitch + (size_t)x0 * 4, wz);
    load_words<2 * PPT>(a.normals.ptr + (size_t)y * a.normals.pitch + (size_t)x0 * 8, wn);
    if (GI == SAH_GI_LPV && a.has_ao) load_words<PPT>(a.ao.ptr + (size_t)y * a.ao.pitch + (size_t)x0 * 4, wao);
    if (SUN == SAH_SHADOW_MODE_RT && a.has_mask) load_words<PPT>(a.shadow_mask.ptr + (size_t)y * a.shadow_mask.pitch + (size_t)x0 * 4, wm);

    uint32_t out[2 * PPT];
#pragma unroll
    for (int i = 0; i < PPT; i++) {
        Px p;
        p.color = wc[i];
        p.data = wd[i];
        p.emission = we[i];
        p.n01 = wn[2 * i];
        p.n23 = wn[2 * i + 1];
        p.depth = __uint_as_float(wz[i]);
        p.ao = (GI == SAH_GI_LPV && a.has_ao) ? __uint_as_float(wao[i]) : 1.0f;
        p.mask = (SUN == SAH_SHADOW_MODE_RT && a.has_mask) ? __uint_as_float(wm[i]) : 1.0f;
        const uint2 r = shade_pixel_general<SUN, GI>(a, csm, lpv, sky, x0 + i, y, p, s_lut);
        out[2 * i] = r.x;
        out[2 * i + 1] = r.y;
    }
    uint8_t* dst = const_cast<uint8_t*>(a.lit.ptr) + (size_t)y * a.lit.pitch + (size_t)x0 * 8;
    if constexpr (PPT == 1) {
        *reinterpret_cast<uint2*>(dst) = make_uint2(out[0], out[1]);
    } else {
        store_words<2 * PPT>(dst, out);
    }
}

constexpr uint32_t kFixupSegs = 16;
constexpr uint32_t kFixupMaxWorkgroups = 2048;
template <int SUN, int GI, int PPT>
__global__ void __launch_bounds__(256) k_lighting_fixup(const LightingArgs a, const CsmArgs csm, const LpvArgs lpv, const SkyArgs sky,
                                                        const FastArgs f) {
    if (__hip_atomic_load(&f.state->deferred_hint[f.hint_slot], __ATOMIC_RELAXED, __HIP_MEMORY_SCOPE_AGENT) == 0u) return;
    __shared__ uint32_t s_pref[kFixupSegs + 1];
    __shared__ float s_lut[512];
    stage_format_tables(s_lut, a.luts);
    const uint32_t ngroups = (f.num_segments + kFixupSegs - 1u) / kFixupSegs;
    for (uint32_t grp = blockIdx.x; grp < ngroups; grp += gridDim.x) {
    __syncthreads();
    const uint32_t seg0 = grp * kFixupSegs;
    if (threadIdx.x < 64) {
        const uint32_t lane = threadIdx.x;
        const uint32_t c = (lane < kFixupSegs && seg0 + lane < f.num_segments) ? (uint32_t)f.seg_count[seg0 + lane] : 0u;
        uint32_t incl = c;
#pragma unroll
        for (int d = 1; d < (int)kFixupSegs; d <<= 1) {
            const uint32_t t = __shfl_up(incl, d, 64);
            if ((int)lane >= d) incl += t;
        }
        if (lane < kFixupSegs) s_pref[lane + 1] = incl;
        if (lane == 0) s_pref[0] = 0;
    }
    __syncthreads();
    const uint32_t total = s_pref[kFixupSegs];
    if (total == 0) continue;
    const uint32_t groups_per_row = a.width / PPT;
    for (uint32_t i = threadIdx.x; i < total; i += 256u) {
        uint32_t s = 0;
#pragma unroll
        for (uint32_t step = kFixupSegs / 2; step >= 1; step >>= 1)
            if (s_pref[s + step] <= i) s += step;
        const uint32_t code = f.seg_list[(size_t)(seg0 + s) * f.seg_stride + (i - s_pref[s])];
        const uint32_t g = (seg0 + s) * 64u + code / PPT;
        const FastPixel at = fast_pixel_of(g, groups_per_row, a.row_end - a.row_begin, PPT, f.tile_rows, f.row_magic);
        const uint32_t y = a.row_begin + at.row, x = at.x0 + code % PPT;
        Px p;
        p.color = *reinterpret_cast<const uint32_t*>(a.color.ptr + (size_t)y * a.color.pitch + (size_t)x * 4);
        p.data = *reinterpret_cast<const uint32_t*>(a.data.ptr + (size_t)y * a.data.pitch + (size_t)x * 4);
        p.emission = *reinterpret_cast<const uint32_t*>(a.emission.ptr + (size_t)y * a.emission.pitch + (size_t)x * 4);
        p.depth = *reinterpret_cast<const float*>(a.depth.ptr + (size_t)y * a.depth.pitch + (size_t)x * 4);
        const uint2 n = *reinterpret_cast<const uint2*>(a.normals.ptr + (size_t)y * a.normals.pitch + (size_t)x * 8);
        p.n01 = n.x;
        p.n23 = n.y;
        p.ao = (GI == SAH_GI_LPV && a.has_ao) ? *reinterpret_cast<const float*>(a.ao.ptr + (size_t)y * a.ao.pitch + (size_t)x * 4) : 1.0f;
        p.mask = (SUN == SAH_SHADOW_MODE_RT && a.has_mask)
                     ? *reinterpret_cast<const float*>(a.shadow_mask.ptr + (size_t)y * a.shadow_mask.pitch + (size_t)x * 4)
                     : 1.0f;
        const uint2 r = shade_pixel_general<SUN, GI>(a, csm, lpv, sky, x, y, p, s_lut);
        *reinterpret_cast<uint2*>(const_cast<uint8_t*>(a.lit.ptr) + (size_t)y * a.lit.pitch + (size_t)x * 8) = r;
    }
    }
}

__global__ void __launch_bounds__(256) k_lpv_pack(const VolumeArg r, const VolumeArg g, const VolumeArg b, uint8_t* packed, uint32_t pk_row_pitch,
                                                  uint32_t pk_slice_pitch, FrameState* state) {
    const uint32_t prow = blockIdx.x;
    const uint32_t ph = r.height + 2 * kLpvPackBorder;
    const uint32_t pz = prow / ph, py = prow - pz * ph;
    const int z = (int)pz - (int)kLpvPackBorder, y = (int)py - (int)kLpvPackBorder;
    const bool row_inside = z >= 0 && z < (int)r.depth && y >= 0 && y < (int)r.height;
    uint32_t bad = 0;
    uint8_t* dst_row = packed + (size_t)pz * pk_slice_pitch + (size_t)py * pk_row_pitch;
    for (uint32_t px = threadIdx.x; px < r.width + 2 * kLpvPackBorder; px += 256) {
        const int x = (int)px - (int)kLpvPackBorder;
        uint2 t[3] = {make_uint2(0u, 0u), make_uint2(0u, 0u), make_uint2(0u, 0u)};
        if (row_inside && x >= 0 && x < (int)r.width) {
            t[0] = *reinterpret_cast<const uint2*>(r.ptr + (size_t)z * r.slice_pitch + (size_t)y * r.row_pitch + (size_t)x * 8);
            t[1] = *reinterpret_cast<const uint2*>(g.ptr + (size_t)z * g.slice_pitch + (size_t)y * g.row_pitch + (size_t)x * 8);
            t[2] = *reinterpret_cast<const uint2*>(b.ptr + (size_t)z * b.slice_pitch + (size_t)y * b.row_pitch + (size_t)x * 8);
#pragma unroll
            for (int c = 0; c < 3; c++) {
                bad |= ((t[c].x & 0x7c00u) == 0x7c00u) | ((t[c].x & 0x7c000000u) == 0x7c000000u) | ((t[c].y & 0x7c00u) == 0x7c00u) |
                       ((t[c].y & 0x7c000000u) == 0x7c000000u);
            }
        }
        uint2* dst = reinterpret_cast<uint2*>(dst_row + (size_t)px * kLpvPackTexel);
        dst[0] = t[0];
        dst[1] = t[1];
        dst[2] = t[2];
    }
    if (wave_any(bad != 0) && (threadIdx.x & 63) == 0) atomicMax(&state->nonfinite, 1u);
}

__global__ void __launch_bounds__(256) k_colx_table(const LightingArgs a, const FastArgs f, float* out, uint32_t stride, uint32_t row_stride) {
    const uint32_t i = blockIdx.x * 256u + threadIdx.x;
    bool neg_zero = false;
    auto put = [&](uint32_t at, float v) {
        out[at] = v;
        neg_zero = neg_zero || __float_as_uint(v) == 0x80000000u;
    };
    if (i < a.width) {
        put(i, colx_glsl_of(a, f, i));
        put(stride + i, colx_slang_of(a, f, i));
    }
    if (i < a.height) {
        put(2u * stride + i, rowy_glsl_of(a, f, i));
        put(2u * stride + row_stride + i, rowy_slang_of(a, f, i));
    }
    if (wave_any(neg_zero) && (threadIdx.x & 63u) == 0u) atomicOr(&f.state->colx_neg_zero, 1u);
}


template <int SUN, int GI, int PPT, bool SKY>
__global__ void __launch_bounds__(256, SKY ? 4 : 1) k_lighting_fast(const LightingArgs a, const CsmArgs csm, const LpvArgs lpv, const SkyArgs sky,
                                                                                 const FastArgs f) {
    uint32_t block_id = blockIdx.x;
    if (SKY) {
        if (blockIdx.x < f.sky_first) {
            const uint32_t ratio = f.sky_ratio;
            const uint32_t groups_per_row = a.width / PPT, rows = a.row_end - a.row_begin, total = groups_per_row * rows;
#pragma unroll 1
            for (uint32_t k = 0; k < ratio; k++) {
                const uint32_t gid = (blockIdx.x * ratio + k) * 256u + threadIdx.x;
                if (gid >= total) break;
                const FastPixel at = fast_pixel_of(gid, groups_per_row, rows, PPT, f.tile_rows, f.row_magic);
                const uint32_t y = a.row_begin + at.row, x0 = at.x0;
                uint32_t wz[PPT];
                load_words<PPT>(a.depth.ptr + (size_t)y * a.depth.pitch + (size_t)x0 * 4, wz);
#pragma unroll 1
                for (int i = 0; i < PPT; i++) {
                    if (__uint_as_float(wz[i]) != 0.f) continue;
                    Hn lit[4];
                    sky_frag(a, sky, x0 + (uint32_t)i, y, lit);
                    *reinterpret_cast<uint2*>(const_cast<uint8_t*>(a.lit.ptr) + (size_t)y * a.lit.pitch + (size_t)(x0 + i) * 8) = pack_lit(lit);
                }
            }
            return;
        }
        block_id = blockIdx.x - f.sky_first;
    }
    const uint32_t groups_per_row = a.width / PPT;
    const uint32_t gid = block_id * 256u + threadIdx.x;
    const uint32_t rows = a.row_end - a.row_begin;
    const bool active = gid < groups_per_row * rows;
    FastPixel at = {0u, 0u};
    if (active) at = fast_pixel_of(gid, groups_per_row, rows, PPT, f.tile_rows, f.row_magic);
    const uint32_t y = a.row_begin + at.row;
    const uint32_t x0 = at.x0;
    const bool lpv_bad = (GI == SAH_GI_LPV) ? (f.state->nonfinite != 0u) : false;
    const bool div_shared = (SUN == SAH_SHADOW_MODE_CSM || GI == SAH_GI_LPV) ? pos_div_shared_of(f) : false;

    uint32_t wc[PPT], wd[PPT], we[PPT], wz[PPT], wn[2 * PPT], wao[PPT], wm[PPT];
    float colx_g[PPT], colx_s[PPT];
    if (active) {
        load_words<PPT>(a.color.ptr + (size_t)y * a.color.pitch + (size_t)x0 * 4, wc);
        load_words<PPT>(a.data.ptr + (size_t)y * a.data.pitch + (size_t)x0 * 4, wd);
        load_words<PPT>(a.emission.ptr + (size_t)y * a.emission.pitch + (size_t)x0 * 4, we);
        load_words<PPT>(a.depth.ptr + (size_t)y * a.depth.pitch + (size_t)x0 * 4, wz);
        load_words<2 * PPT>(a.normals.ptr + (size_t)y * a.normals.pitch + (size_t)x0 * 8, wn);
        if (GI == SAH_GI_LPV && a.has_ao) load_words<PPT>(a.ao.ptr + (size_t)y * a.ao.pitch + (size_t)x0 * 4, wao);
        if (SUN == SAH_SHADOW_MODE_RT && a.has_mask) load_words<PPT>(a.shadow_mask.ptr + (size_t)y * a.shadow_mask.pitch + (size_t)x0 * 4, wm);
        if (f.colx_tab) {
            uint32_t t[PPT];
            if (SUN == SAH_SHADOW_MODE_CSM || GI == SAH_GI_LPV) {
                load_words<PPT>(reinterpret_cast<const uint8_t*>(f.colx_tab + x0), t);
#pragma unroll
                for (int i = 0; i < PPT; i++) colx_g[i] = __uint_as_float(t[i]);
            }
            if (SUN == SAH_SHADOW_MODE_RT) {
                load_words<PPT>(reinterpret_cast<const uint8_t*>(f.colx_tab + f.colx_stride + x0), t);
#pragma unroll
                for (int i = 0; i < PPT; i++) colx_s[i] = __uint_as_float(t[i]);
            }
        }
    }
    __shared__ __attribute__((aligned(16))) float s_lut[TAB_SIZE];
    stage_fast_tables<SUN == SAH_SHADOW_MODE_CSM, GI == SAH_GI_LPV>(s_lut, a, csm, f);
    __syncthreads();
    LpvBox box;
    box.lds = nullptr;
    box.valid = false;
    if constexpr (GI == SAH_GI_LPV) {
        __shared__ __attribute__((aligned(16))) uint8_t s_box[4 * kLpvBoxBytes];
        box.lds = s_box + (uint32_t)__builtin_amdgcn_readfirstlane((int)(threadIdx.x >> 6)) * kLpvBoxBytes;
    }

    float rowy_glsl = 0.f, rowy_slang = 0.f;
    if (f.colx_tab) {
        if (SUN == SAH_SHADOW_MODE_CSM || GI == SAH_GI_LPV) rowy_glsl = f.colx_tab[2u * f.colx_stride + y];
        if (SUN == SAH_SHADOW_MODE_RT) rowy_slang = f.colx_tab[2u * f.colx_stride + f.rowy_stride + y];
    } else {
        if (SUN == SAH_SHADOW_MODE_CSM || GI == SAH_GI_LPV) rowy_glsl = rowy_glsl_of(a, f, y);
        if (SUN == SAH_SHADOW_MODE_RT) rowy_slang = rowy_slang_of(a, f, y);
    }

    uint32_t out[2 * PPT];
    uint32_t deferred_mask = 0, sky_mask = 0;
    bool emissive_wave;
    {
        uint32_t any_e = 0;
#pragma unroll
        for (int i = 0; i < PPT; i++) any_e |= we[i];
        emissive_wave = wave_any(active && (any_e & 0xffffffu) != 0u);
    }
#pragma unroll
    for (int i = 0; i < PPT; i++) {
        if (!active) break;
        Px p;
        p.color = wc[i];
        p.data = wd[i];
        p.emission = we[i];
        p.n01 = wn[2 * i];
        p.n23 = wn[2 * i + 1];
        p.depth = __uint_as_float(wz[i]);
        p.ao = (GI == SAH_GI_LPV && a.has_ao) ? __uint_as_float(wao[i]) : 1.0f;
        p.mask = (SUN == SAH_SHADOW_MODE_RT && a.has_mask) ? __uint_as_float(wm[i]) : 1.0f;
        const uint32_t x = x0 + i;
        float colx_glsl = 0.f, colx_slang = 0.f;
        if (f.colx_tab) {
            if (SUN == SAH_SHADOW_MODE_CSM || GI == SAH_GI_LPV) colx_glsl = colx_g[i];
            if (SUN == SAH_SHADOW_MODE_RT) colx_slang = colx_s[i];
        } else {
            if (SUN == SAH_SHADOW_MODE_CSM || GI == SAH_GI_LPV) colx_glsl = colx_glsl_of(a, f, x);
            if (SUN == SAH_SHADOW_MODE_RT) colx_slang = colx_slang_of(a, f, x);
        }
        const FastPixelOut r = shade_pixel_fast_sl<SUN, GI>(a, csm, lpv, f, colx_glsl, rowy_glsl, colx_slang, rowy_slang, p, s_lut, lpv_bad, emissive_wave, div_shared, box, i == 0,
                                                                   lpv_box_centre_lane(PPT));
        out[2 * i] = r.lit.x;
        out[2 * i + 1] = r.lit.y;
        if (r.deferred) deferred_mask |= 1u << i;
        if (p.depth == 0.f) sky_mask |= 1u << i;
    }
    if (active) {
        uint8_t* dst = const_cast<uint8_t*>(a.lit.ptr) + (size_t)y * a.lit.pitch + (size_t)x0 * 8;
        if (SKY && sky_mask != 0u) {
#pragma unroll
            for (int i = 0; i < PPT; i++)
                if (!((sky_mask >> i) & 1u)) *reinterpret_cast<uint2*>(dst + 8 * i) = make_uint2(out[2 * i], out[2 * i + 1]);
        } else if constexpr (PPT == 1) {
            *reinterpret_cast<uint2*>(dst) = make_uint2(out[0], out[1]);
        } else {
            store_words<2 * PPT>(dst, out);
        }
    }
    const uint32_t seg = gid >> 6, lane = threadIdx.x & 63u;
    uint32_t front = 0;
    const uint32_t listed = SKY ? deferred_mask & ~sky_mask : deferred_mask;
    if (wave_any(listed != 0u)) {
        uint8_t* seg_codes = f.seg_list + (size_t)seg * f.seg_stride;
#pragma unroll
        for (int i = 0; i < PPT; i++) {
            const bool mine = (listed >> i) & 1u;
            const uint64_t m = __ballot(mine);
            if (m) {
                const uint32_t before = __builtin_amdgcn_mbcnt_hi((uint32_t)(m >> 32), __builtin_amdgcn_mbcnt_lo((uint32_t)m, 0u));
                if (mine) seg_codes[front + before] = (uint8_t)(lane * PPT + (uint32_t)i);
                front += (uint32_t)__builtin_popcountll(m);
            }
        }
    }
    if (lane == 0 && seg < f.num_segments) {
        f.seg_count[seg] = (uint16_t)front;
        if (front != 0u) f.state->deferred_hint[f.hint_slot] = 1u;
    }
    if (gid == 0u) f.state->deferred_hint[f.hint_slot ^ 1u] = 0u;
}

static hipError_t launch_lpv_pack(const LpvArgs& lpv, const FastArgs& f, hipStream_t st) {
    const uint32_t prows = (lpv.red.height + 2 * kLpvPackBorder) * (lpv.red.depth + 2 * kLpvPackBorder);
    const hipError_t me = hipMemsetAsync(&f.state->nonfinite, 0, sizeof(uint32_t), st);
    if (me != hipSuccess) return me;
    hipLaunchKernelGGL(k_lpv_pack, dim3(prows), dim3(256), 0, st, lpv.red, lpv.green, lpv.blue, const_cast<uint8_t*>(f.lpv_packed), f.pk_row_pitch,
                       f.pk_slice_pitch, f.state);
    return hipGetLastError();
}
template <int SUN, int GI>
static hipError_t launch_general_ppt(const LightingArgs& a, const CsmArgs& csm, const LpvArgs& lpv, const SkyArgs& sky, int ppt, hipStream_t st) {
    const uint32_t rows = a.row_end - a.row_begin;
    const uint64_t groups = (uint64_t)(a.width / ppt) * rows;
    if (groups == 0) return hipSuccess;
    const dim3 grid((uint32_t)((groups + 255) / 256)), block(256);
    if (ppt == 4) hipLaunchKernelGGL((k_lighting_general<SUN, GI, 4>), grid, block, 0, st, a, csm, lpv, sky);
    else if (ppt == 2) hipLaunchKernelGGL((k_lighting_general<SUN, GI, 2>), grid, block, 0, st, a, csm, lpv, sky);
    else hipLaunchKernelGGL((k_lighting_general<SUN, GI, 1>), grid, block, 0, st, a, csm, lpv, sky);
    return hipGetLastError();
}

template <int SUN, int GI>
static hipError_t launch_fast_ppt(const LightingArgs& a, const CsmArgs& csm, const LpvArgs& lpv, const SkyArgs& sky, const FastArgs& f, int ppt,
                                  hipStream_t st) {
    const uint32_t rows = a.row_end - a.row_begin;
    const uint64_t groups = (uint64_t)(a.width / ppt) * rows;
    if (groups == 0) return hipSuccess;
    if (GI == SAH_GI_LPV && f.repack) {
        const hipError_t pe = launch_lpv_pack(lpv, f, st);
        if (pe != hipSuccess) return pe;
    }
    const uint32_t blocks = (uint32_t)((groups + 255) / 256);
    const dim3 block(256);
    auto launch = [&](auto ppt_c) {
        constexpr int P = decltype(ppt_c)::value;
        if (sky.enabled) hipLaunchKernelGGL((k_lighting_fast<SUN, GI, P, true>), dim3(f.sky_first + blocks), block, 0, st, a, csm, lpv, sky, f);
        else hipLaunchKernelGGL((k_lighting_fast<SUN, GI, P, false>), dim3(blocks), block, 0, st, a, csm, lpv, sky, f);
    };
    if (ppt == 4) launch(std::integral_constant<int, 4>{});
    else if (ppt == 2) launch(std::integral_constant<int, 2>{});
    else launch(std::integral_constant<int, 1>{});
    const uint32_t fgroups = (f.num_segments + kFixupSegs - 1) / kFixupSegs;
    const dim3 fgrid(fgroups < kFixupMaxWorkgroups ? fgroups : kFixupMaxWorkgroups);
    if (ppt == 4) hipLaunchKernelGGL((k_lighting_fixup<SUN, GI, 4>), fgrid, block, 0, st, a, csm, lpv, sky, f);
    else if (ppt == 2) hipLaunchKernelGGL((k_lighting_fixup<SUN, GI, 2>), fgrid, block, 0, st, a, csm, lpv, sky, f);
    else hipLaunchKernelGGL((k_lighting_fixup<SUN, GI, 1>), fgrid, block, 0, st, a, csm, lpv, sky, f);
    return hipGetLastError();
}

template <int SUN>
static hipError_t launch_gi(const LightingArgs& a, const CsmArgs& csm, const LpvArgs& lpv, const SkyArgs& sky, const FastArgs* f, int gi, int ppt,
                            hipStream_t st) {
    switch (gi) {
        case SAH_GI_NONE:
            return f ? launch_fast_ppt<SUN, SAH_GI_NONE>(a, csm, lpv, sky, *f, ppt, st) : launch_general_ppt<SUN, SAH_GI_NONE>(a, csm, lpv, sky, ppt, st);
        case SAH_GI_LPV:
            return f ? launch_fast_ppt<SUN, SAH_GI_LPV>(a, csm, lpv, sky, *f, ppt, st) : launch_general_ppt<SUN, SAH_GI_LPV>(a, csm, lpv, sky, ppt, st);
        default: return hipErrorNotSupported;
    }
}

hipError_t launch_colx_table(const LightingArgs& a, const FastArgs& f, float* out, uint32_t stride, uint32_t row_stride, hipStream_t st) {
    const hipError_t me = hipMemsetAsync(&f.state->colx_neg_zero, 0, sizeof(uint32_t), st);
    if (me != hipSuccess) return me;
    hipLaunchKernelGGL(k_colx_table, dim3((max(a.width, a.height) + 255u) / 256u), dim3(256), 0, st, a, f, out, stride, row_stride);
    return hipGetLastError();
}

hipError_t launch_lighting(const LightingArgs& a, const CsmArgs& csm, const LpvArgs& lpv, const CacheArgs& cache, const RtgiArgs& rtgi,
                           const SkyArgs& sky, LightingFamily family, const FastArgs* fast, int sun_mode, int gi, int ppt, bool brute_force_lights,
                           hipStream_t st) {
    if (family == kLightingTiled) {
        if (gi == SAH_GI_LPV && fast && fast->lpv_fast && fast->repack && a.row_end > a.row_begin) {
            const hipError_t pe = launch_lpv_pack(lpv, *fast, st);
            if (pe != hipSuccess) return pe;
        }
        return launch_lighting_tiled(a, csm, lpv, cache, rtgi, sky, sun_mode, gi, brute_force_lights, fast, st);
    }
    switch (sun_mode) {
        case SAH_SHADOW_MODE_OFF: return launch_gi<SAH_SHADOW_MODE_OFF>(a, csm, lpv, sky, fast, gi, ppt, st);
        case SAH_SHADOW_MODE_CSM: return launch_gi<SAH_SHADOW_MODE_CSM>(a, csm, lpv, sky, fast, gi, ppt, st);
        case SAH_SHADOW_MODE_RT: return launch_gi<SAH_SHADOW_MODE_RT>(a, csm, lpv, sky, fast, gi, ppt, st);
        default: return hipErrorInvalidValue;
    }
}

}
```

androidrenderer_amd/csrc/lighting_common.hpp:

```cpp
#pragma once
#include <hip/hip_runtime.h>

#include "../../include/sah_hip.h"
#include "lpv_box.hpp"
#include "numerics.hpp"
#include "params.hpp"

namespace sah {

static_assert(kLpvBoxSrcTexel == kLpvPackTexel && kLpvBoxPad == kLpvPackBorder, "lpv_box.hpp restates the gather copy's texel and border");

template <int NW> SAH_DEV void load_words(const uint8_t* p, uint32_t (&w)[NW]) {
    if constexpr (NW == 1) {
        w[0] = *reinterpret_cast<const uint32_t*>(p);
    } else if constexpr (NW == 2) {
        uint2 v = *reinterpret_cast<const uint2*>(p);
        w[0] = v.x; w[1] = v.y;
    } else if constexpr (NW == 4) {
        uint4 v = *reinterpret_cast<const uint4*>(p);
        w[0] = v.x; w[1] = v.y; w[2] = v.z; w[3] = v.w;
    } else {
        static_assert(NW == 8, "unsupported width");
        uint4 v0 = *reinterpret_cast<const uint4*>(p);
        uint4 v1 = *reinterpret_cast<const uint4*>(p + 16);
        w[0] = v0.x; w[1] = v0.y; w[2] = v0.z; w[3] = v0.w;
        w[4] = v1.x; w[5] = v1.y; w[6] = v1.z; w[7] = v1.w;
    }
}
template <int NW> SAH_DEV void store_words(uint8_t* p, const uint32_t (&w)[NW]) {
    if constexpr (NW == 2) {
        *reinterpret_cast<uint2*>(p) = make_uint2(w[0], w[1]);
    } else if constexpr (NW == 4) {
        *reinterpret_cast<uint4*>(p) = make_uint4(w[0], w[1], w[2], w[3]);
    } else {
        static_assert(NW == 8, "unsupported width");
        *reinterpret_cast<uint4*>(p) = make_uint4(w[0], w[1], w[2], w[3]);
        *reinterpret_cast<uint4*>(p + 16) = make_uint4(w[4], w[5], w[6], w[7]);
    }
}

struct Px {
    uint32_t color, data, emission, n01, n23;
    float depth, ao, mask;
};

SAH_DEV int clamp_to_int(float f) { return (int)__builtin_fminf(__builtin_fmaxf(f, -1.0e9f), 1.0e9f); }
SAH_DEV int clamp_index(float f, int hi) {
    int i, r;
    asm("v_cvt_i32_f32 %0, %1" : "=v"(i) : "v"(f));
    asm("v_med3_i32 %0, %1, 0, %2" : "=v"(r) : "v"(i), "s"(hi));
    return r;
}
SAH_DEV _Float16 hbits(uint32_t b) { return __builtin_bit_cast(_Float16, (uint16_t)b); }


struct TriSetup {
    float w[8];
    int x0, y0, z0;
    bool nan;
};
SAH_DEV TriSetup tri_setup(uint32_t W, uint32_t H, uint32_t D, float u, float v, float ww) {
    TriSetup s;
    const float px = u * (float)W - 0.5f, py = v * (float)H - 0.5f, pz = ww * (float)D - 0.5f;
    s.nan = isnan_f(px) || isnan_f(py) || isnan_f(pz);
    const float fx0 = __builtin_floorf(px), fy0 = __builtin_floorf(py), fz0 = __builtin_floorf(pz);
    const float fx = px - fx0, fy = py - fy0, fz = pz - fz0;
    const float wx0 = 1.0f - fx, wy0 = 1.0f - fy, wz0 = 1.0f - fz;
    s.x0 = clamp_to_int(fx0);
    s.y0 = clamp_to_int(fy0);
    s.z0 = clamp_to_int(fz0);
    const float wxy[4] = {wx0 * wy0, fx * wy0, wx0 * fy, fx * fy};
#pragma unroll
    for (int k = 0; k < 8; k++) s.w[k] = wxy[k & 3] * ((k >> 2) ? fz : wz0);
    return s;
}
typedef _Float16 half4_t __attribute__((ext_vector_type(4)));

SAH_DEV half4_t load_texel8_border(const VolumeArg& v, int x, int y, int z) {
    if ((unsigned)x < v.width && (unsigned)y < v.height && (unsigned)z < v.depth) {
        const uint32_t off = (uint32_t)z * v.slice_pitch + (uint32_t)y * v.row_pitch + (uint32_t)x * 8u;
        return *reinterpret_cast<const half4_t*>(v.ptr + off);
    }
    return half4_t{(_Float16)0.f, (_Float16)0.f, (_Float16)0.f, (_Float16)0.f};
}
SAH_DEV void tri_accumulate(const VolumeArg& v, const TriSetup& s, float (&out)[4]) {
    if (s.nan) {
        out[0] = out[1] = out[2] = out[3] = __builtin_nanf("");
        return;
    }
    half4_t t[8];
#pragma unroll
    for (int k = 0; k < 8; k++) t[k] = load_texel8_border(v, s.x0 + (k & 1), s.y0 + ((k >> 1) & 1), s.z0 + (k >> 2));
    out[0] = out[1] = out[2] = out[3] = 0.0f;
#pragma unroll
    for (int k = 0; k < 8; k++) {
#pragma unroll
        for (int c = 0; c < 4; c++) out[c] = __builtin_fmaf(s.w[k], (float)t[k][c], out[c]);
    }
}

SAH_DEV void sample_bilinear_repeat_rgba16f(const PlaneArg& p, uint32_t W, uint32_t H, float u, float v, float (&out)[4]) {
    const float px = u * (float)W - 0.5f, py = v * (float)H - 0.5f;
    if (isnan_f(px) || isnan_f(py)) {
        out[0] = out[1] = out[2] = out[3] = __builtin_nanf("");
        return;
    }
    const float fx0 = __builtin_floorf(px), fy0 = __builtin_floorf(py);
    const float fx = px - fx0, fy = py - fy0;
    const float wx0 = 1.0f - fx, wy0 = 1.0f - fy;
    int x0 = clamp_to_int(fx0) % (int)W, y0 = clamp_to_int(fy0) % (int)H;
    if (x0 < 0) x0 += (int)W;
    if (y0 < 0) y0 += (int)H;
    const int x1 = x0 + 1 == (int)W ? 0 : x0 + 1, y1 = y0 + 1 == (int)H ? 0 : y0 + 1;
    const int xs[4] = {x0, x1, x0, x1}, ys[4] = {y0, y0, y1, y1};
    const float w[4] = {wx0 * wy0, fx * wy0, wx0 * fy, fx * fy};
    half4_t q[4];
#pragma unroll
    for (int k = 0; k < 4; k++) q[k] = *reinterpret_cast<const half4_t*>(p.ptr + (size_t)ys[k] * p.pitch + (size_t)xs[k] * 8);
    out[0] = out[1] = out[2] = out[3] = 0.0f;
#pragma unroll
    for (int k = 0; k < 4; k++) {
#pragma unroll
        for (int c = 0; c < 4; c++) out[c] = __builtin_fmaf(w[k], (float)q[k][c], out[c]);
    }
}

SAH_DEV F3 viewspace_position_glsl(const LightingArgs& a, uint32_t x, uint32_t y, float depth) {
    const Fn fx = Fn((float)x + 0.5f) + Fn(0.5f), fy = Fn((float)y + 0.5f) + Fn(0.5f);
    const Fn tx = fx / Fn(a.res[0]), ty = fy / Fn(a.res[1]);
    const F4 ndc = {tx * Fn(2.0f) - Fn(1.0f), ty * Fn(2.0f) - Fn(1.0f), Fn(depth), Fn(1.0f)};
    const F4 vs = mul44(a.inv_proj, ndc);
    return {vs.x / vs.w, vs.y / vs.w, vs.z / vs.w};
}

SAH_DEV F3 worldspace_location_slang(const LightingArgs& a, float px, float py, float depth) {
    const Fn tx = (Fn(px) + Fn(0.5f)) / Fn(a.res[0]);
    const Fn ty = (Fn(py) + Fn(0.5f)) / Fn(a.res[1]);
    const F4 ndc = {tx * Fn(2.0f) - Fn(1.0f), ty * Fn(2.0f) - Fn(1.0f), Fn(depth), Fn(1.0f)};
    F4 vs = mul44(a.inv_proj, ndc);
    vs = {vs.x / vs.w, vs.y / vs.w, vs.z / vs.w, vs.w / vs.w};
    const F4 ws = mul44(a.inv_view, vs);
    return {ws.x, ws.y, ws.z};
}

struct SurfIn {
    float color[3];
    float normal[3];
    float rough, metal;
};

SAH_DEV SurfIn unpack_surface(const Px& p, const float* lut) {
    SurfIn s;
    s.color[0] = lut[p.color & 0xffu];
    s.color[1] = lut[(p.color >> 8) & 0xffu];
    s.color[2] = lut[(p.color >> 16) & 0xffu];
    s.normal[0] = (float)hbits(p.n01 & 0xffffu);
    s.normal[1] = (float)hbits(p.n01 >> 16);
    s.normal[2] = (float)hbits(p.n23 & 0xffffu);
    s.rough = lut[256 + ((p.data >> 8) & 0xffu)];
    s.metal = lut[256 + ((p.data >> 16) & 0xffu)];
    return s;
}

SAH_DEV float shadow_pcf(const CsmArgs& c, float u, float v, uint32_t layer, float ref) {
    const VolumeArg& sm = c.shadowmap;
    const float px = u * (float)sm.width - 0.5f, py = v * (float)sm.height - 0.5f;
    const float fx0 = __builtin_floorf(px), fy0 = __builtin_floorf(py);
    const float fx = px - fx0, fy = py - fy0;
    const int x0 = (int)fx0, y0 = (int)fy0;
    float cmp[4];
    const uint8_t* layer_base = sm.ptr + (size_t)layer * sm.slice_pitch;
    const int xa = x0 < 0 ? 0 : (x0 > (int)sm.width - 1 ? (int)sm.width - 1 : x0);
    const int xb = x0 + 1 < 0 ? 0 : (x0 + 1 > (int)sm.width - 1 ? (int)sm.width - 1 : x0 + 1);
    const int ya = y0 < 0 ? 0 : (y0 > (int)sm.height - 1 ? (int)sm.height - 1 : y0);
    const int yb = y0 + 1 < 0 ? 0 : (y0 + 1 > (int)sm.height - 1 ? (int)sm.height - 1 : y0 + 1);
    const uint32_t ra = (uint32_t)ya * sm.row_pitch, rb = (uint32_t)yb * sm.row_pitch;
    const int xs[4] = {xa, xb, xa, xb};
    const uint32_t rs[4] = {ra, ra, rb, rb};
    float d[4];
    if (c.is_d16) {
        uint16_t raw[4];
#pragma unroll
        for (int k = 0; k < 4; k++) raw[k] = *reinterpret_cast<const uint16_t*>(layer_base + rs[k] + (uint32_t)xs[k] * 2u);
        if (c.d16_recip_ok) {
#pragma unroll
            for (int k = 0; k < 4; k++) {
                const float v = (float)raw[k];
                const float q = v * c.d16_recip;
                d[k] = __builtin_fmaf(__builtin_fmaf(-q, 65535.0f, v), c.d16_recip, q);
            }
        } else {
#pragma unroll
            for (int k = 0; k < 4; k++) d[k] = (float)raw[k] / 65535.0f;
        }
    } else {
#pragma unroll
        for (int k = 0; k < 4; k++) d[k] = *reinterpret_cast<const float*>(layer_base + rs[k] + (uint32_t)xs[k] * 4u);
    }
#pragma unroll
    for (int k = 0; k < 4; k++) cmp[k] = (ref < d[k]) ? 1.0f : 0.0f;
    const float wx0 = 1.0f - fx, wy0 = 1.0f - fy;
    float r = __builtin_fmaf(wx0 * wy0, cmp[0], 0.0f);
    r = __builtin_fmaf(fx * wy0, cmp[1], r);
    r = __builtin_fmaf(wx0 * fy, cmp[2], r);
    r = __builtin_fmaf(fx * fy, cmp[3], r);
    return r;
}

SAH_DEV Fn sample_csm(const CsmArgs& c, F3 ws, Fn viewspace_depth, Fn ndotl) {
    uint32_t cascade = 0;
#pragma unroll
    for (uint32_t i = 0; i < 4; i++) {
        if (viewspace_depth.v < c.splits[i]) cascade = i + 1;
    }
    if (cascade > 3) return Fn(0.0f);
    const Fn bias = Fn(0.0005f) * nsqrt(Fn(1.0f) - ndotl * ndotl) / ndotl;
    F4 sp = mul44(c.biased[cascade], F4{ws.x, ws.y, ws.z, Fn(1.0f)});
    sp = {sp.x / sp.w, sp.y / sp.w, sp.z / sp.w, sp.w / sp.w};
    if (sp.x.v < 0.f || sp.y.v < 0.f || sp.z.v < 0.f || sp.x.v > 1.f || sp.y.v > 1.f || sp.z.v > 1.f) return Fn(1.0f);
    if (c.shadowmap.ptr == nullptr) return Fn(1.0f);
    if (isnan_f(sp.x.v) || isnan_f(sp.y.v)) return Fn(__builtin_nanf(""));
    float ref = (sp.z - bias).v;
    if (c.is_d16) ref = ref < 0.f ? 0.f : (ref > 1.f ? 1.f : ref);
    return Fn(shadow_pcf(c, sp.x.v, sp.y.v, cascade, ref));
}

SAH_DEV void sun_frag(const LightingArgs& a, const CsmArgs& csm, uint32_t x, uint32_t y, const Px& p, const SurfIn& si, Fn (&out)[4]) {
    Surface<Fn> s;
    s.base_color = {Fn(si.color[0]), Fn(si.color[1]), Fn(si.color[2])};
    s.normal = normalize(F3{Fn(si.normal[0]), Fn(si.normal[1]), Fn(si.normal[2])});
    s.roughness = Fn(si.rough);
    s.metalness = Fn(si.metal);
    const F3 vs = viewspace_position_glsl(a, x, y, p.depth);
    const F4 ws4 = mul44(a.inv_view, F4{vs.x, vs.y, vs.z, Fn(1.0f)});
    const F3 ws = {ws4.x, ws4.y, ws4.z};
    const F3 V = normalize(ws - F3{Fn(a.view_pos[0]), Fn(a.view_pos[1]), Fn(a.view_pos[2])});
    const F3 L = {Fn(a.sun_L[0]), Fn(a.sun_L[1]), Fn(a.sun_L[2])};
    const Fn ndotl = nclamp(dot(s.normal, L), Fn(0.f), Fn(1.f));
    Fn shadow = Fn(1.0f);
    if (ndotl.v > 0.f) shadow = sample_csm(csm, ws, vs.z, ndotl);
    const F3 b = brdf_sl(s, L, V);
    F3 direct = ndotl * b * F3{Fn(a.sun_color[0]), Fn(a.sun_color[1]), Fn(a.sun_color[2])} * shadow;
    if (any_nan(direct)) direct = F3(Fn(0.f));
    const Fn exposure = Fn(0.00031415927f);
    out[0] = direct.x * exposure;
    out[1] = direct.y * exposure;
    out[2] = direct.z * exposure;
    out[3] = Fn(1.0f);
}

SAH_DEV void sun_rt(const LightingArgs& a, uint32_t x, uint32_t y, const Px& p, const SurfIn& si, float (&add)[3]) {
    Surface<Hn> s;
    s.base_color = {Hn(si.color[0]), Hn(si.color[1]), Hn(si.color[2])};
    s.normal = normalize(H3{Hn(si.normal[0]), Hn(si.normal[1]), Hn(si.normal[2])});
    s.roughness = Hn(si.rough);
    s.metalness = Hn(si.metal);
    const F3 location = worldspace_location_slang(a, (float)x, (float)y, p.depth);
    const F3 L = {Fn(a.sun_L[0]), Fn(a.sun_L[1]), Fn(a.sun_L[2])};
    const Hn ndotl = Hn(nclamp(dot(L, to_f(s.normal)), Fn(0.f), Fn(1.f)).v);
    const H3 V = to_h(normalize(location - F3{Fn(a.view_pos[0]), Fn(a.view_pos[1]), Fn(a.view_pos[2])}));
    const H3 Lh = to_h(L);
    const H3 b = brdf_sl(s, Lh, V);
    const H3 nb = ndotl * b;
    F3 radiance = to_f(nb) * F3{Fn(a.sun_color[0]), Fn(a.sun_color[1]), Fn(a.sun_color[2])};
    if (tof(ndotl) > 0.f) radiance = radiance * Fn(p.mask);
    const Fn exposure = Fn(0.00031415927f);
    add[0] = (radiance.x * exposure).v;
    add[1] = (radiance.y * exposure).v;
    add[2] = (radiance.z * exposure).v;
}

SAH_DEV void dir_to_sh(F3 d, Fn (&o)[4]) {
    const Fn c0 = Fn(0.282094792f), c1 = Fn(0.488602512f);
    o[0] = c0;
    o[1] = -c1 * d.y;
    o[2] = c1 * d.z;
    o[3] = -c1 * d.x;
}
SAH_DEV Fn dot4(const float (&t)[4], const Fn (&n)[4]) { return Fn(t[0]) * n[0] + Fn(t[1]) * n[1] + Fn(t[2]) * n[2] + Fn(t[3]) * n[3]; }

SAH_DEV void lpv_fetch(const LpvArgs& L, F4 p, const Fn (&n)[4], Fn (&out)[3]) {
    const TriSetup s = tri_setup(L.red.width, L.red.height, L.red.depth, p.x.v, p.y.v, p.z.v);
    float r[4], g[4], b[4];
    tri_accumulate(L.red, s, r);
    tri_accumulate(L.green, s, g);
    tri_accumulate(L.blue, s, b);
    out[0] = dot4(r, n);
    out[1] = dot4(g, n);
    out[2] = dot4(b, n);
}

SAH_DEV void lpv_fetch_packed(const LpvArgs& L, const uint8_t* packed, uint32_t row_pitch, uint32_t slice_pitch, float u, float v, float w,
                              const Fn (&n)[4], Fn (&out)[3]) {
    const int W = (int)L.red.width, H = (int)L.red.height, D = (int)L.red.depth;
    const float px = u * (float)W - 0.5f, py = v * (float)H - 0.5f, pz = w * (float)D - 0.5f;
    const float fx0 = __builtin_floorf(px), fy0 = __builtin_floorf(py), fz0 = __builtin_floorf(pz);
    const float fx = px - fx0, fy = py - fy0, fz = pz - fz0;
    const float gx = 1.0f - fx, gy = 1.0f - fy, gz = 1.0f - fz;
    const int b = (int)kLpvPackBorder;
    const uint32_t x0 = (uint32_t)(min(max(clamp_to_int(fx0), -b), W) + b), y0 = (uint32_t)(min(max(clamp_to_int(fy0), -b), H) + b),
                   z0 = (uint32_t)(min(max(clamp_to_int(fz0), -b), D) + b);
    const uint32_t base = z0 * slice_pitch + y0 * row_pitch + x0 * kLpvPackTexel;
    const uint32_t ro[4] = {base, base + row_pitch, base + slice_pitch, base + slice_pitch + row_pitch};
    uint32_t d[4][12];
#pragma unroll
    for (int r = 0; r < 4; r++) {
#pragma unroll
        for (int j = 0; j < 3; j++) {
            const uint4 q = *reinterpret_cast<const uint4*>(packed + ro[r] + 16u * (uint32_t)j);
            d[r][4 * j] = q.x;
            d[r][4 * j + 1] = q.y;
            d[r][4 * j + 2] = q.z;
            d[r][4 * j + 3] = q.w;
        }
    }
    const float wxy[4] = {gx * gy, fx * gy, gx * fy, fx * fy};
    float wt[8];
#pragma unroll
    for (int k = 0; k < 8; k++) wt[k] = wxy[k & 3] * ((k >> 2) ? fz : gz);
#pragma unroll
    for (int c = 0; c < 3; c++) {
        float a[4] = {0.f, 0.f, 0.f, 0.f};
#pragma unroll
        for (int k = 0; k < 8; k++) {
            const int r = k >> 1, xs = k & 1;
            const uint32_t lo = d[r][xs * 6 + c * 2], hi = d[r][xs * 6 + c * 2 + 1];
            a[0] = fma_mix_lo(wt[k], lo, a[0]);
            a[1] = fma_mix_hi(wt[k], lo, a[1]);
            a[2] = fma_mix_lo(wt[k], hi, a[2]);
            a[3] = fma_mix_hi(wt[k], hi, a[3]);
        }
        out[c] = dot4(a, n);
    }
}

SAH_DEV void lpv_packed_base(const LpvArgs& L, float u, float v, float w, uint32_t (&base)[3]) {
    const int W = (int)L.red.width, H = (int)L.red.height, D = (int)L.red.depth;
    const float px = u * (float)W - 0.5f, py = v * (float)H - 0.5f, pz = w * (float)D - 0.5f;
    const float fx0 = __builtin_floorf(px), fy0 = __builtin_floorf(py), fz0 = __builtin_floorf(pz);
    const int b = (int)kLpvPackBorder;
    base[0] = (uint32_t)(min(max(clamp_to_int(fx0), -b), W) + b);
    base[1] = (uint32_t)(min(max(clamp_to_int(fy0), -b), H) + b);
    base[2] = (uint32_t)(min(max(clamp_to_int(fz0), -b), D) + b);
}

SAH_DEV void lpv_fetch_box(const LpvArgs& L, const uint8_t* box_px, float u, float v, float w, const Fn (&n)[4], Fn (&out)[3]) {
    const int W = (int)L.red.width, H = (int)L.red.height, D = (int)L.red.depth;
    const float px = u * (float)W - 0.5f, py = v * (float)H - 0.5f, pz = w * (float)D - 0.5f;
    const float fx0 = __builtin_floorf(px), fy0 = __builtin_floorf(py), fz0 = __builtin_floorf(pz);
    const float fx = px - fx0, fy = py - fy0, fz = pz - fz0;
    const float gx = 1.0f - fx, gy = 1.0f - fy, gz = 1.0f - fz;
    const float wxy[4] = {gx * gy, fx * gy, gx * fy, fx * fy};
    float wt[8];
#pragma unroll
    for (int k = 0; k < 8; k++) wt[k] = wxy[k & 3] * ((k >> 2) ? fz : gz);
#pragma unroll
    for (int c = 0; c < 3; c++) {
        float a[4] = {0.f, 0.f, 0.f, 0.f};
#pragma unroll
        for (int k = 0; k < 8; k++) {
            const float4 t = *reinterpret_cast<const float4*>(box_px + lpv_box_lds_row((uint32_t)k >> 1) + (uint32_t)(k & 1) * kLpvBoxTexel + 16u * (uint32_t)c);
            a[0] = __builtin_fmaf(wt[k], t.x, a[0]);
            a[1] = __builtin_fmaf(wt[k], t.y, a[1]);
            a[2] = __builtin_fmaf(wt[k], t.z, a[2]);
            a[3] = __builtin_fmaf(wt[k], t.w, a[3]);
        }
        out[c] = dot4(a, n);
    }
}

SAH_DEV void gi_lpv_frag(const LightingArgs& a, const LpvArgs& L, uint32_t x, uint32_t y, const Px& p, const SurfIn& si, Fn (&out)[4]) {
    Surface<Fn> s;
    s.base_color = {Fn(si.color[0]), Fn(si.color[1]), Fn(si.color[2])};
    s.normal = normalize(F3{Fn(si.normal[0]), Fn(si.normal[1]), Fn(si.normal[2])});
    s.roughness = Fn(si.rough);
    s.metalness = Fn(si.metal);
    const F3 vs = viewspace_position_glsl(a, x, y, p.depth);
    const F4 ws = mul44(a.inv_view, F4{vs.x, vs.y, vs.z, Fn(1.0f)});
    const F3 V = normalize(F3{ws.x, ws.y, ws.z} - F3{Fn(a.view_pos[0]), Fn(a.view_pos[1]), Fn(a.view_pos[2])});

    uint32_t selected = 0;
    for (int i = (int)L.num_cascades - 1; i >= 0; i--) {
        const F4 cp = mul44(L.world_to_cascade[i], ws);
        if (cp.x.v > 0.f && cp.y.v > 0.f && cp.z.v > 0.f && cp.x.v < 1.f && cp.y.v < 1.f && cp.z.v < 1.f) selected = (uint32_t)i;
    }
    F3 lpv_normal = -s.normal;
    lpv_normal.x = lpv_normal.x * Fn(-1.0f);
    Fn nc[4];
    dir_to_sh(lpv_normal, nc);

    Fn indirect[3];
    {
        const F4 pos = {ws.x + s.normal.x, ws.y + s.normal.y, ws.z + s.normal.z, ws.w + Fn(0.f)};
        F4 cp = mul44(L.world_to_cascade[selected], pos);
        cp.x = cp.x + Fn((float)selected);
        cp.x = cp.x / Fn(L.num_cascades_f);
        lpv_fetch(L, cp, nc, indirect);
    }
    const F3 I = -V;
    const F3 refl = I - s.normal * (Fn(2.0f) * dot(s.normal, I));
    Fn spec[3] = {Fn(0.f), Fn(0.f), Fn(0.f)};
    if (selected == 0) {
        const F4 cp = mul44(L.world_to_cascade[0], ws);
        Fn rc[4];
        dir_to_sh(refl, rc);
        lpv_fetch(L, cp, rc, spec);
        const F3 loc = F3{ws.x, ws.y, ws.z} + refl * Fn(1.0f);
        const F4 cp1 = mul44(L.world_to_cascade[0], F4{loc.x, loc.y, loc.z, Fn(1.f)});
        Fn more[3];
        lpv_fetch(L, cp1, rc, more);
#pragma unroll
        for (int i = 0; i < 3; i++) spec[i] = (spec[i] + more[i]) / Fn(2.0f);
    }
    const F3 diffuse_factor = Fd(s, s.normal, s.normal);
    const F3 fr = Fr(s, s.normal, refl);
    const F3 specular_factor = {fr.x * Fn(0.f), fr.y * Fn(0.f), fr.z * Fn(0.f)};
    const Fn ao = Fn(p.ao);
    F3 total = {indirect[0] * diffuse_factor.x * ao + spec[0] * specular_factor.x,
                indirect[1] * diffuse_factor.y * ao + spec[1] * specular_factor.y,
                indirect[2] * diffuse_factor.z * ao + spec[2] * specular_factor.z};
    if (any_nan(total)) total = F3(Fn(0.f));
    const Fn exposure = Fn(L.exposure);
    out[0] = total.x * exposure;
    out[1] = total.y * exposure;
    out[2] = total.z * exposure;
    out[3] = Fn(1.0f);
}

SAH_DEV Fn cr_acos(Fn x) { return Fn((float)acos((double)x.v)); }
SAH_DEV Fn cr_atan(Fn x) { return Fn((float)atan((double)x.v)); }
SAH_DEV Fn cr_exp(Fn x) { return Fn((float)exp((double)x.v)); }
SAH_DEV Fn fsign(Fn x) { return Fn(x.v > 0.f ? 1.0f : (x.v < 0.f ? -1.0f : 0.0f)); }

SAH_DEV Fn ray_intersect_sphere(F3 ro, F3 rd, Fn rad) {
    const Fn b = dot(ro, rd);
    const Fn c = dot(ro, ro) - rad * rad;
    if (c.v > 0.0f && b.v > 0.0f) return Fn(-1.0f);
    const Fn discr = b * b - c;
    if (discr.v < 0.0f) return Fn(-1.0f);
    if (discr.v > (b * b).v) return (-b + nsqrt(discr));
    return -b - nsqrt(discr);
}

SAH_DEV F3 sky_color(const SkyArgs& k, F3 rayDir) {
    const Fn sky_pi = Fn(3.14159265358f);
    const F3 sunDir = {Fn(k.sun_dir[0]), Fn(k.sun_dir[1]), Fn(k.sun_dir[2])};
    const F3 up = {Fn(0.0f) / Fn(k.height), Fn(k.up_y), Fn(0.0f) / Fn(k.height)};
    const F3 view_pos = {Fn(0.f), Fn(k.view_pos_y), Fn(0.f)};

    const Fn altitudeAngle = Fn(k.horizon_angle) - cr_acos(dot(rayDir, up));
    Fn azimuthAngle;
    if (__builtin_fabsf(altitudeAngle.v) > k.azimuth_limit) {
        azimuthAngle = Fn(0.0f);
    } else {
        const F3 right = {Fn(k.right[0]), Fn(k.right[1]), Fn(k.right[2])};
        const F3 forward = {Fn(k.forward[0]), Fn(k.forward[1]), Fn(k.forward[2])};
        const F3 projectedDir = normalize(rayDir - up * (dot(rayDir, up)));
        const Fn sinTheta = dot(projectedDir, right);
        const Fn cosTheta = dot(projectedDir, forward);
        azimuthAngle = cr_atan(cosTheta / sinTheta) + sky_pi;
    }
    const Fn v = Fn(0.5f) + Fn(0.5f) * fsign(altitudeAngle) * nsqrt(nabs(altitudeAngle) * Fn(2.0f) / sky_pi);
    const Fn u = azimuthAngle / (Fn(2.0f) * sky_pi);
    float lut[4];
    sample_bilinear_repeat_rgba16f(k.sky_view, k.s_w, k.s_h, u.v, v.v, lut);
    F3 lum = {Fn(lut[0]), Fn(lut[1]), Fn(lut[2])};

    Fn sun;
    {
        const Fn cosTheta = dot(rayDir, sunDir);
        if (cosTheta.v >= k.min_sun_cos) {
            sun = Fn(1.f);
        } else {
            const Fn offset = Fn(k.min_sun_cos) - cosTheta;
            const Fn ex = -offset * Fn(50000.0f);
            const Fn gaussianBloom = ex.v <= -110.0f ? Fn(0.0f) : cr_exp(ex) * Fn(0.5f);
            const Fn invBloom = Fn(1.0f) / (Fn(0.02f) + offset * Fn(300.0f)) * Fn(0.01f);
            sun = gaussianBloom + invBloom;
        }
    }
    const Fn t = nclamp((sun - Fn(k.smooth_e0)) / (Fn(1.0f) - Fn(k.smooth_e0)), Fn(0.0f), Fn(1.0f));
    const Fn s = t * t * (Fn(3.0f) - Fn(2.0f) * t);
    F3 sunLum = F3(s);
    if (length(sunLum).v > 0.0f) {
        if (ray_intersect_sphere(view_pos, rayDir, Fn(6.360f)).v >= 0.0f) {
            sunLum = F3(Fn(0.f));
        } else {
            const Fn sunCosZenithAngle = dot(sunDir, up);
            const Fn tu = nclamp(Fn(0.5f) + Fn(0.5f) * sunCosZenithAngle, Fn(0.0f), Fn(1.0f));
            const Fn tv = nmax(Fn(0.0f), nmin(Fn(1.0f), (Fn(k.height) - Fn(6.360f)) / (Fn(6.460f) - Fn(6.360f))));
            float tl[4];
            sample_bilinear_repeat_rgba16f(k.transmittance, k.t_w, k.t_h, tu.v, tv.v, tl);
            sunLum = sunLum * F3{Fn(tl[0]), Fn(tl[1]), Fn(tl[2])};
        }
    }
    lum = lum + sunLum;
    lum = lum * Fn(20.0f);
    lum = lum * Fn(1.0f);
    return lum;
}

SAH_DEV void sky_frag(const LightingArgs& a, const SkyArgs& k, uint32_t x, uint32_t y, Hn (&out)[4]) {
    const Fn sx = (Fn((float)x + 0.5f) + Fn(0.5f)) / Fn(a.res[0]);
    const Fn sy = (Fn((float)y + 0.5f) + Fn(0.5f)) / Fn(a.res[1]);
    F4 vs = mul44(a.inv_proj, F4{sx, sy, Fn(1.f), Fn(1.f)});
    vs = {vs.x / vs.w, vs.y / vs.w, vs.z / vs.w, vs.w / vs.w};
    const F4 wv = mul44(a.inv_view, F4{vs.x, vs.y, vs.z, Fn(0.f)});
    F3 rayDir = -normalize(F3{wv.x, wv.y, wv.z});
    rayDir.y = rayDir.y * Fn(-1.0f);
    const F3 lum = sky_color(k, rayDir);
    out[0] = Hn(lum.x.v);
    out[1] = Hn(lum.y.v);
    out[2] = Hn(lum.z.v);
    out[3] = Hn(1.0f);
}

SAH_DEV uint2 pack_lit(const Hn (&lit)[4]) {
    uint2 r;
    r.x = (uint32_t)__builtin_bit_cast(uint16_t, lit[0].v) | ((uint32_t)__builtin_bit_cast(uint16_t, lit[1].v) << 16);
    r.y = (uint32_t)__builtin_bit_cast(uint16_t, lit[2].v) | ((uint32_t)__builtin_bit_cast(uint16_t, lit[3].v) << 16);
    return r;
}

template <int SUN, int GI>
SAH_DEV uint2 shade_pixel_general(const LightingArgs& a, const CsmArgs& csm, const LpvArgs& lpv, const SkyArgs& sky, uint32_t x, uint32_t y,
                                  const Px& p, const float* lut) {
    Hn lit[4] = {Hn::lit(0.f), Hn::lit(0.f), Hn::lit(0.f), Hn::lit(0.f)};
    const bool surface = p.depth != 0.f;
    SurfIn si;
    if (surface) si = unpack_surface(p, lut);

    if constexpr (SUN == SAH_SHADOW_MODE_CSM) {
        if (surface) {
            Fn s[4];
            sun_frag(a, csm, x, y, p, si, s);
            if (a.flags & SAH_LIGHTING_QUIRK_SUN_BLEND) {
#pragma unroll
                for (int i = 0; i < 3; i++) lit[i] = Hn((s[i] * s[i] + Fn(tof(lit[i])) * Fn(tof(lit[i]))).v);
                lit[3] = Hn((s[3] * Fn(0.f) + Fn(tof(lit[3])) * Fn(0.f)).v);
            } else {
#pragma unroll
                for (int i = 0; i < 4; i++) lit[i] = Hn(tof(lit[i]) + s[i].v);
            }
        }
    }
    if constexpr (GI == SAH_GI_LPV) {
        if (surface) {
            Fn s[4];
            gi_lpv_frag(a, lpv, x, y, p, si, s);
#pragma unroll
            for (int i = 0; i < 4; i++) lit[i] = Hn(tof(lit[i]) + s[i].v);
        }
    }
    {
        const Fn e = Fn(3.1415927f);
        lit[0] = Hn(tof(lit[0]) + (Fn(lut[p.emission & 0xffu]) * e).v);
        lit[1] = Hn(tof(lit[1]) + (Fn(lut[(p.emission >> 8) & 0xffu]) * e).v);
        lit[2] = Hn(tof(lit[2]) + (Fn(lut[(p.emission >> 16) & 0xffu]) * e).v);
        lit[3] = Hn(tof(lit[3]) + 1.0f);
    }
    if (sky.enabled && !surface) sky_frag(a, sky, x, y, lit);
    if constexpr (SUN == SAH_SHADOW_MODE_RT) {
        if (surface) {
            float add[3];
            sun_rt(a, x, y, p, si, add);
#pragma unroll
            for (int i = 0; i < 3; i++) lit[i] = Hn(tof(lit[i]) + add[i]);
        }
    }
    return pack_lit(lit);
}

}
```

androidrenderer_amd/csrc/params.hpp:

```cpp
#pragma once
#include <stdint.h>

namespace sah {

struct PlaneArg {
    const uint8_t* ptr;
    uint32_t pitch;
};
struct VolumeArg {
    const uint8_t* ptr;
    uint32_t width, height, depth;
    uint32_t row_pitch, slice_pitch;
};

struct LpvArgs {
    VolumeArg red, green, blue;
    float world_to_cascade[4][16];
    uint32_t num_cascades;
    float num_cascades_f;
    float exposure;
};

struct ProbeAtlasArgs {
    VolumeArg rtgi, light_cache, depth, average, validity;
};

struct CacheArgs {
    VolumeArg irradiance, depth, validity;
    float cascade_min[4][3];
    float cascade_max[4][3];
    float spacing[4];
    float inv_spacing[4];
    uint32_t spacing_pow2;
    uint32_t probe_size[2];
    float inv_tex[2];
    uint32_t debug_mode;
    uint32_t hot_ok;
    const uint8_t* irr32;
};

struct RtgiArgs {
    PlaneArg ray_buffer, ray_irradiance, noise;
    uint32_t noise_w, noise_h;
    uint32_t num_extra_rays;
    float extra_ray_radius;
};

struct CsmArgs {
    VolumeArg shadowmap;
    uint32_t is_d16;
    uint32_t d16_recip_ok;
    float d16_recip;
    float splits[4];
    float biased[4][16];
};

struct SkyArgs {
    PlaneArg transmittance, sky_view;
    uint32_t t_w, t_h, s_w, s_h;
    float sun_dir[3];
    float height;
    float up_y;
    float view_pos_y;
    float horizon_angle;
    float azimuth_limit;
    float min_sun_cos;
    float right[3];
    float forward[3];
    float tlut_rgb[3];
    float smooth_e0;
    uint32_t enabled;
};

struct FrameState {
    uint32_t deferred_hint[2];
    uint32_t nonfinite;
    uint32_t colx_neg_zero;
};

struct FastArgs {
    float p0, p12, p5, p13, p10, p14, p11, p15;
    float lpv_s[4][3], lpv_t[4][3];
    float inv_ncasc;
    uint32_t ncasc_pow2;
    uint32_t pos_div_nr;
    uint32_t sky_enabled;
    uint32_t sky_ratio;
    uint32_t sky_first;
    uint32_t row_magic;
    uint32_t tile_rows;
    uint32_t repack;
    const float* colx_tab;
    uint32_t colx_stride;
    uint32_t rowy_stride;
    FrameState* state;
    uint8_t* seg_list;
    uint16_t* seg_count;
    uint32_t num_segments, seg_stride;
    uint32_t hint_slot;
    uint32_t pos_div_shared;
    const uint8_t* lpv_packed;
    uint32_t pk_row_pitch, pk_slice_pitch;
    uint32_t lpv_fast;
};
constexpr uint32_t kLpvPackTexel = 24, kLpvPackBorder = 2;
struct LpvGvStep {
    VolumeArg gv;
    void* factors;
};

struct LpvPackEmit {
    uint8_t* packed;
    uint32_t row_pitch, slice_pitch;
    FrameState* state;
};

enum LightingFamily : uint32_t { kLightingGeneral = 0, kLightingFast = 1, kLightingTiled = 2 };

struct LightingArgs {
    PlaneArg color, normals, data, emission, depth, ao, shadow_mask, lit;
    uint32_t width, height, row_begin, row_end;
    uint32_t flags;
    float res[2];
    float inv_proj[16];
    float inv_view[16];
    float view_pos[3];
    float sun_L[3];
    float sun_color[3];
    uint32_t has_ao, has_mask;
    const float* luts;
    const void* lights;
    uint32_t num_lights;
};

}
```

androidrenderer_amd/lib.py:

```python
import ctypes as C
import os

import numpy as np

from . import _abi

_HERE = os.path.dirname(os.path.abspath(__file__))
LIB_PATH = os.environ.get("SAH_HIP_LIBRARY") or os.path.join(_HERE, "libsah_hip.so")


class SahError(RuntimeError):
    def __init__(self, status, message):
        super().__init__(f"sah status {status}: {message}")
        self.status = status


_lib = None

EXPORTS = ["sah_abi_version", "sah_status_string", "sah_last_error", "sah_create", "sah_destroy", "sah_comm_unique_id", "sah_set_stream",
           "sah_sync", "sah_lighting", "sah_copy_scene", "sah_copy_scene_rows", "sah_copy_scene_bloom_mip0_rows", "sah_bloom", "sah_bloom_mip0_rows", "sah_bloom_from_mip0", "sah_bloom_mip_rows", "sah_bloom_from_mip", "sah_bloom_source_rows", "sah_tonemap", "sah_tonemap_ex", "sah_lpv_clear", "sah_lpv_propagate", "sah_probe_notify_updated",
           "sah_sky_update_luts", "sah_ao_clear", "sah_probe_copy", "sah_probe_update", "sah_shadow_render", "sah_gbuffer_render", "sah_rsm_render", "sah_lpv_extract_vpls",
           "sah_lpv_inject_vpls", "sah_rt_build", "sah_rtao", "sah_sun_shadow_mask", "sah_probe_trace", "sah_rtgi_trace", "sah_rt_set_rows", "sah_rt_set_bounces", "sah_debug_rt_structure", "sah_debug_raster_last_pass", "sah_allgather_rows", "sah_allgather_rows_reversed", "sah_allgather_bytes", "sah_comm_set_stream", "sah_comm_wait",
           "sah_ipc_open", "sah_ipc_connect", "sah_ipc_export", "sah_ipc_register", "sah_ipc_unregister", "sah_ipc_reset",
           "sah_chain_create", "sah_chain_submit", "sah_chain_flush", "sah_chain_counts", "sah_chain_destroy"]

GV_EXPORTS = ["sah_lpv_inject_rsm_gv", "sah_lpv_inject_scene_gv", "sah_lpv_propagate_gv"]

MV_EXPORTS = ["sah_motion_vectors_render"]

GBUFFER_MOTION_EXPORTS = ["sah_gbuffer_motion_render"]

VRSAA_EXPORTS = ["sah_vrsaa_measure_aliasing", "sah_vrsaa_shading_rate_image"]

TAA_EXPORTS = ["sah_taa_resolve"]

TAA_UPSCALE_EXPORTS = ["sah_taa_upscale"]

SSAO_EXPORTS = ["sah_ssao"]

RT_DENOISE_EXPORTS = ["sah_rt_denoise"]

RTGI_DENOISE_EXPORTS = ["sah_rtgi_denoise"]

EXPOSURE_EXPORTS = ["sah_exposure_meter", "sah_exposure_apply"]
EXPOSURE_WORK_BYTES = 1040
EXPOSURE_BINS = 256

MIP_CHAIN_EXPORTS = ["sah_mip_chain_generate"]
MIP_CHAIN_MAX_LEVELS = 12
MIP_CHAIN_MAX_SOURCE = 4096

RT_REFIT_EXPORTS = ["sah_rt_refit"]

ML_EXPORTS = ["sah_mesh_point_cloud", "sah_lpv_emissive_vpls", "sah_lpv_inject_emissive"]
POINT_CLOUD_ON_SURFACE = 1
EMISSIVE_MATERIAL_ZERO = 1
LPV_EMISSIVE_MAX_ENTRIES = 1 << 24

RT_STRUCTURE_HEADER_WORDS = 34
RT_MAX_LEVELS = 15


RT_TRIANGLE = np.dtype([("v0", np.float32, 3), ("primitive", np.uint32), ("v1", np.float32, 3), ("triangle", np.uint32), ("v2", np.float32, 3),
                        ("flags", np.uint32)])
assert RT_TRIANGLE.itemsize == 48


class EmissiveCloud(C.Structure):
    _fields_ = [("vpls", C.c_void_p), ("count", C.c_uint32), ("primitive", C.c_uint32), ("bounds_min", C.c_float * 3), ("bounds_max", C.c_float * 3)]


class LpvCascadeBounds(C.Structure):
    _fields_ = [("min_bounds", C.c_float * 3), ("max_bounds", C.c_float * 3)]


def mesh_point_cloud(positions, vertex_data, indices, first_index, index_count, vertex_offset, seed, flags=0):
    import numpy as np
    from . import mesh
    lib = load()
    pos = np.ascontiguousarray(positions, np.float32)
    vd = np.ascontiguousarray(vertex_data)
    idx = np.ascontiguousarray(indices, np.uint32)
    count, lo, hi = C.c_uint32(0), (C.c_float * 3)(), (C.c_float * 3)()
    args = (pos.ctypes.data if pos.size else None, vd.ctypes.data if vd.size else None, pos.shape[0], idx.ctypes.data if idx.size else None, idx.shape[0],
            first_index, index_count, vertex_offset, seed, flags)
    rc = lib.sah_mesh_point_cloud(*args, None, None, 0, C.byref(count), lo, hi)
    if rc != _abi.SAH_OK:
        raise SahError(rc, f"sah_mesh_point_cloud: {lib.sah_status_string(rc).decode()}")
    out_pos = np.zeros((count.value, 3), np.float32)
    out_vd = np.zeros(count.value, mesh.VERTEX_DATA)
    if count.value:
        rc = lib.sah_mesh_point_cloud(*args, out_pos.ctypes.data, out_vd.ctypes.data, count.value, C.byref(count), lo, hi)
        if rc != _abi.SAH_OK:
            raise SahError(rc, f"sah_mesh_point_cloud: {lib.sah_status_string(rc).decode()}")
    return out_pos, out_vd, np.array(lo[:], np.float32), np.array(hi[:], np.float32)


def load():
    global _lib
    if _lib is not None:
        return _lib
    if not os.path.exists(LIB_PATH):
        raise ImportError(f"{LIB_PATH} not found — build it with `python -m androidrenderer_amd.build` (needs hipcc); "
                          "there is no CPU fallback for the product path")
    lib = C.CDLL(LIB_PATH)
    lib.sah_abi_version.restype = C.c_int
    lib.sah_status_string.restype = C.c_char_p
    lib.sah_status_string.argtypes = [C.c_int]
    lib.sah_last_error.restype = C.c_char_p
    lib.sah_last_error.argtypes = [C.c_void_p]
    lib.sah_create.argtypes = [C.POINTER(C.c_void_p), C.c_int, C.c_int, C.c_int, C.c_void_p]
    lib.sah_destroy.argtypes = [C.c_void_p]
    lib.sah_destroy.restype = None
    lib.sah_comm_unique_id.argtypes = [C.c_void_p]
    lib.sah_set_stream.argtypes = [C.c_void_p, C.c_void_p]
    lib.sah_sync.argtypes = [C.c_void_p]
    lib.sah_debug_deferred_pixels.argtypes = [C.c_void_p, C.POINTER(C.c_uint64)]
    lib.sah_debug_copy_rebuilds.argtypes = [C.c_void_p, C.POINTER(C.c_uint32)]
    lib.sah_debug_cache_epoch.argtypes = [C.c_void_p, C.POINTER(C.c_uint64)]
    lib.sah_debug_lighting_dispatch.argtypes = [C.c_void_p, C.POINTER(C.c_uint32)]
    lib.sah_lighting.argtypes = [C.c_void_p, C.POINTER(_abi.LightingDesc)]
    lib.sah_copy_scene.argtypes = [C.c_void_p, C.POINTER(_abi.Plane), C.POINTER(_abi.Plane)]
    lib.sah_copy_scene_rows.argtypes = [C.c_void_p, C.POINTER(_abi.Plane), C.POINTER(_abi.Plane), C.c_uint32, C.c_uint32]
    lib.sah_bloom.argtypes = [C.c_void_p, C.POINTER(_abi.Plane), C.POINTER(_abi.MipChain)]
    lib.sah_copy_scene_bloom_mip0_rows.argtypes = [C.c_void_p, C.POINTER(_abi.Plane), C.POINTER(_abi.Plane), C.POINTER(_abi.MipChain)] + [C.c_uint32] * 4
    lib.sah_bloom_mip0_rows.argtypes = [C.c_void_p, C.POINTER(_abi.Plane), C.POINTER(_abi.MipChain), C.c_uint32, C.c_uint32]
    lib.sah_bloom_from_mip0.argtypes = [C.c_void_p, C.POINTER(_abi.Plane), C.POINTER(_abi.MipChain)]
    lib.sah_bloom_mip_rows.argtypes = [C.c_void_p, C.POINTER(_abi.Plane), C.POINTER(_abi.MipChain), C.c_uint32, C.c_uint32, C.c_uint32]
    lib.sah_bloom_from_mip.argtypes = [C.c_void_p, C.POINTER(_abi.Plane), C.POINTER(_abi.MipChain), C.c_uint32]
    lib.sah_bloom_source_rows.argtypes = [C.c_uint32] * 4 + [C.POINTER(C.c_uint32)]
    lib.sah_tonemap.argtypes = [C.c_void_p, C.POINTER(_abi.Plane), C.POINTER(_abi.MipChain), C.POINTER(_abi.Plane), C.c_uint32, C.c_uint32]
    lib.sah_tonemap_ex.argtypes = [C.c_void_p, C.POINTER(_abi.Plane), C.POINTER(_abi.MipChain), C.POINTER(_abi.Plane), C.c_uint32, C.c_uint32, C.c_uint32]
    lib.sah_lpv_clear.argtypes = [C.c_void_p] + [C.POINTER(_abi.Volume)] * 4 + [C.c_uint32]
    lib.sah_lpv_propagate.argtypes = [C.c_void_p, C.POINTER(_abi.Volume), C.POINTER(_abi.Volume), C.c_uint32, C.c_uint32]
    lib.sah_allgather_rows.argtypes = [C.c_void_p, C.POINTER(_abi.Plane), C.c_uint32, C.c_uint32]
    lib.sah_allgather_bytes.argtypes = [C.c_void_p, C.c_void_p, C.c_uint64]
    lib.sah_allgather_rows_reversed.argtypes = [C.c_void_p, C.POINTER(_abi.Plane), C.c_uint32, C.c_uint32]
    lib.sah_comm_set_stream.argtypes = [C.c_void_p, C.c_void_p]
    lib.sah_comm_wait.argtypes = [C.c_void_p]
    lib.sah_ao_clear.argtypes = [C.c_void_p, C.POINTER(_abi.Plane)]
    lib.sah_sky_update_luts.argtypes = [C.c_void_p, C.POINTER(_abi.Plane), C.POINTER(_abi.Plane), C.POINTER(_abi.Plane), C.POINTER(C.c_float)]
    lib.sah_probe_copy.argtypes =[C.c_void_p, C.POINTER(_abi.ProbeAtlases), C.POINTER(_abi.ProbeAtlases), C.POINTER(C.c_float * 3)]
    lib.sah_probe_update.argtypes = [C.c_void_p, C.POINTER(_abi.ProbeAtlases), C.POINTER(_abi.Volume), C.c_void_p, C.c_uint32]
    lib.sah_probe_notify_updated.argtypes = [C.c_void_p, C.POINTER(_abi.Volume), C.c_void_p, C.c_uint32]
    lib.sah_shadow_render.argtypes = [C.c_void_p, C.POINTER(_abi.SceneGeometry), C.POINTER(_abi.SunLightConstants), C.c_uint32,
                                      C.POINTER(_abi.Volume), C.c_void_p]
    lib.sah_gbuffer_render.argtypes = [C.c_void_p, C.POINTER(_abi.SceneGeometry), C.POINTER(_abi.ViewData), C.POINTER(_abi.GBuffer), C.c_void_p]
    lib.sah_motion_vectors_render.argtypes = [C.c_void_p, C.POINTER(_abi.SceneGeometry), C.POINTER(_abi.ViewData), C.POINTER(_abi.Plane), C.POINTER(_abi.Plane),
                                              C.c_void_p]
    lib.sah_gbuffer_motion_render.argtypes = [C.c_void_p, C.POINTER(_abi.SceneGeometry), C.POINTER(_abi.ViewData), C.POINTER(_abi.GBuffer), C.POINTER(_abi.Plane),
                                              C.c_void_p]
    lib.sah_rsm_render.argtypes = [C.c_void_p, C.POINTER(_abi.SceneGeometry), C.POINTER(_abi.SunLightConstants), C.POINTER(_abi.LpvCascadeMatrices),
                                   C.c_uint32, C.POINTER(_abi.RsmTargets), C.c_void_p]
    lib.sah_lpv_extract_vpls.argtypes = [C.c_void_p, C.POINTER(_abi.RsmTargets), C.POINTER(_abi.LpvCascadeMatrices), C.c_uint32, C.c_float, C.c_void_p,
                                         C.c_void_p]
    lib.sah_lpv_inject_vpls.argtypes = [C.c_void_p, C.c_void_p, C.c_void_p, C.c_uint32, C.POINTER(_abi.LpvCascadeMatrices), C.c_uint32, C.c_uint32,
                                        C.POINTER(_abi.Volume)]
    lib.sah_rt_build.argtypes = [C.c_void_p, C.POINTER(_abi.SceneGeometry), C.POINTER(C.c_uint32)]
    lib.sah_rtao.argtypes = [C.c_void_p, C.POINTER(_abi.ViewData), C.POINTER(_abi.Plane), C.POINTER(_abi.Plane), C.POINTER(_abi.Plane), C.c_uint32, C.c_float,
                             C.POINTER(_abi.Plane)]
    lib.sah_sun_shadow_mask.argtypes = [C.c_void_p, C.POINTER(_abi.ViewData), C.POINTER(_abi.SunLightConstants), C.POINTER(_abi.Plane), C.POINTER(_abi.Plane),
                                        C.POINTER(_abi.Plane), C.POINTER(_abi.Plane)]
    lib.sah_rt_set_rows.argtypes = [C.c_void_p, C.c_uint32, C.c_uint32]
    lib.sah_rt_set_bounces.argtypes = [C.c_void_p, C.c_uint32]
    lib.sah_debug_rt_structure.argtypes = [C.c_void_p, C.POINTER(C.c_uint32), C.c_void_p, C.c_uint64, C.c_void_p, C.c_uint64]
    lib.sah_debug_raster_last_pass.argtypes = [C.c_void_p, C.POINTER(C.c_uint32)]
    lib.sah_probe_trace.argtypes = [C.c_void_p, C.POINTER(_abi.ProbeTraceDesc)]
    lib.sah_rtgi_trace.argtypes = [C.c_void_p, C.POINTER(_abi.ViewData), C.POINTER(_abi.SunLightConstants), C.POINTER(_abi.SkyLuts)] + [C.POINTER(_abi.Plane)] * 5
    lib.sah_ipc_open.argtypes = [C.c_void_p, C.c_void_p]
    lib.sah_ipc_connect.argtypes = [C.c_void_p, C.c_void_p]
    lib.sah_ipc_export.argtypes = [C.c_void_p, C.c_void_p, C.c_uint64, C.c_void_p]
    lib.sah_ipc_register.argtypes = [C.c_void_p, C.c_void_p, C.c_uint64, C.c_void_p]
    lib.sah_ipc_unregister.argtypes = [C.c_void_p, C.c_void_p]
    lib.sah_ipc_reset.argtypes = [C.c_void_p]
    lib.sah_chain_create.argtypes = [C.c_void_p, C.POINTER(_abi.ChainPlan), C.POINTER(_abi.ChainFrame), C.c_uint32, C.c_uint32, C.c_void_p, C.c_void_p, C.c_void_p,
                                     C.POINTER(C.c_void_p)]
    lib.sah_chain_submit.argtypes = [C.c_void_p, C.c_void_p, C.c_void_p]
    lib.sah_chain_flush.argtypes = [C.c_void_p]
    lib.sah_chain_counts.argtypes = [C.c_void_p, C.POINTER(C.c_uint64), C.POINTER(C.c_uint64)]
    lib.sah_chain_destroy.argtypes = [C.c_void_p]
    lib.sah_debug_chain_graphs.argtypes = [C.c_void_p, C.POINTER(C.c_uint64)]
    lib.sah_chain_destroy.restype = None
    lib.sah_debug_set.argtypes = [C.c_void_p, C.c_int, C.c_int]
    lib.sah_lpv_inject_rsm_gv.argtypes = [C.c_void_p, C.POINTER(_abi.RsmTargets), C.POINTER(_abi.LpvCascadeMatrices), C.c_uint32, C.c_uint32, C.c_uint32,
                                          C.POINTER(_abi.Volume)]
    lib.sah_lpv_inject_scene_gv.argtypes = [C.c_void_p, C.POINTER(_abi.Plane), C.POINTER(_abi.Plane), C.POINTER(_abi.ViewData),
                                            C.POINTER(_abi.LpvCascadeMatrices), C.c_uint32, C.POINTER(_abi.Volume)]
    lib.sah_mesh_point_cloud.argtypes = [C.c_void_p, C.c_void_p, C.c_uint32, C.c_void_p, C.c_uint32, C.c_uint32, C.c_uint32, C.c_int32, C.c_uint64,
                                         C.c_uint32, C.c_void_p, C.c_void_p, C.c_uint32, C.POINTER(C.c_uint32), C.POINTER(C.c_float),
                                         C.POINTER(C.c_float)]
    lib.sah_lpv_emissive_vpls.argtypes = [C.c_void_p, C.POINTER(_abi.SceneGeometry), C.c_uint32, C.c_void_p, C.c_void_p, C.c_uint32, C.c_uint32,
                                          C.c_void_p]
    lib.sah_lpv_inject_emissive.argtypes = [C.c_void_p, C.POINTER(_abi.SceneGeometry), C.POINTER(EmissiveCloud), C.c_uint32,
                                            C.POINTER(_abi.LpvCascadeMatrices), C.POINTER(LpvCascadeBounds), C.c_uint32, C.POINTER(_abi.Volume)]
    lib.sah_lpv_propagate_gv.argtypes = [C.c_void_p, C.POINTER(_abi.Volume), C.POINTER(_abi.Volume), C.POINTER(_abi.Volume), C.c_uint32, C.c_uint32]
    lib.sah_vrsaa_measure_aliasing.argtypes = [C.c_void_p, C.POINTER(_abi.Plane), C.POINTER(_abi.Plane), C.POINTER(_abi.Plane), C.c_uint32, C.c_uint32]
    lib.sah_vrsaa_shading_rate_image.argtypes = [C.c_void_p, C.POINTER(_abi.Plane), C.POINTER(_abi.Plane), C.POINTER(_abi.ShadingRateParams)]
    lib.sah_taa_resolve.argtypes = [C.c_void_p] + [C.POINTER(_abi.Plane)] * 5 + [C.POINTER(_abi.TaaParams), C.c_uint32, C.c_uint32]
    lib.sah_taa_upscale.argtypes = [C.c_void_p] + [C.POINTER(_abi.Plane)] * 5 + [C.POINTER(_abi.TaaUpscaleParams), C.c_uint32, C.c_uint32]
    lib.sah_ssao.argtypes = [C.c_void_p, C.POINTER(_abi.ViewData)] + [C.POINTER(_abi.Plane)] * 4 + [C.POINTER(_abi.SsaoParams), C.c_uint32, C.c_uint32]
    lib.sah_rt_denoise.argtypes = [C.c_void_p, C.POINTER(_abi.ViewData), C.POINTER(_abi.RtDenoiseDesc), C.POINTER(_abi.RtDenoiseParams), C.c_uint32, C.c_uint32]
    lib.sah_rtgi_denoise.argtypes = [C.c_void_p, C.POINTER(_abi.ViewData), C.POINTER(_abi.RtgiDenoiseDesc), C.POINTER(_abi.RtgiDenoiseParams), C.c_uint32, C.c_uint32]
    lib.sah_exposure_meter.argtypes = [C.c_void_p, C.POINTER(_abi.Plane), C.c_void_p, C.c_void_p, C.c_void_p, C.POINTER(_abi.Plane), C.POINTER(_abi.ExposureParams)]
    lib.sah_exposure_apply.argtypes = [C.c_void_p, C.POINTER(_abi.Plane), C.c_void_p, C.POINTER(_abi.Plane), C.c_uint32, C.c_uint32]
    lib.sah_mip_chain_generate.argtypes =[C.c_void_p, C.POINTER(_abi.Plane), C.POINTER(_abi.Plane), C.c_uint32]
    lib.sah_rt_refit.argtypes = [C.c_void_p, C.POINTER(_abi.SceneGeometry), C.c_void_p]
    _lib = lib
    return lib


class Context:

    def __init__(self, device=0, rank=0, world=1, comm_id=None, stream=None):
        self.lib = load()
        h = C.c_void_p()
        idbuf = None
        if comm_id is not None:
            idbuf = C.create_string_buffer(bytes(comm_id), 128)
        rc = self.lib.sah_create(C.byref(h), device, rank, world, idbuf)
        if rc != _abi.SAH_OK:
            raise SahError(rc, self.lib.sah_status_string(rc).decode())
        self.handle = h
        if stream is not None:
            self.set_stream(stream)

    def _check(self, rc):
        if rc != _abi.SAH_OK:
            msg = self.lib.sah_last_error(self.handle).decode() or self.lib.sah_status_string(rc).decode()
            raise SahError(rc, msg)

    def set_stream(self, hip_stream_handle):
        self._check(self.lib.sah_set_stream(self.handle, C.c_void_p(hip_stream_handle)))

    def debug_set(self, force_general=False, force_ppt=0):
        self._check(self.lib.sah_debug_set(self.handle, int(force_general), int(force_ppt)))

    def deferred_pixels(self):
        n = C.c_uint64()
        self._check(self.lib.sah_debug_deferred_pixels(self.handle, C.byref(n)))
        return int(n.value)

    def copy_rebuilds(self):
        out = (C.c_uint32 * 2)()
        self._check(self.lib.sah_debug_copy_rebuilds(self.handle, out))
        return int(out[0]), int(out[1])

    def cache_epoch(self):
        e = C.c_uint64()
        self._check(self.lib.sah_debug_cache_epoch(self.handle, C.byref(e)))
        return int(e.value)

    DISPATCH_FIELDS = ("family", "ppt", "pos_div_nr", "ncasc_pow2", "row_magic", "sky_ratio", "sky_workgroups", "tiled_fast_geom", "tiled_fast_lpv",
                       "repack", "table_rebuilt", "pos_div_shared")

    def lighting_dispatch(self):
        out = (C.c_uint32 * len(self.DISPATCH_FIELDS))()
        self._check(self.lib.sah_debug_lighting_dispatch(self.handle, out))
        rep = {k: int(v) for k, v in zip(self.DISPATCH_FIELDS, out)}
        rep["family"] = ("general", "fast", "tiled")[rep["family"]]
        return rep

    def sync(self):
        self._check(self.lib.sah_sync(self.handle))

    def lighting(self, desc):
        self._check(self.lib.sah_lighting(self.handle, C.byref(desc)))

    def copy_scene(self, lit, out, row_begin=0, row_end=0):
        self._check(self.lib.sah_copy_scene_rows(self.handle, C.byref(lit), C.byref(out), row_begin, row_end))

    def copy_scene_bloom_mip0(self, lit, out, chain, aa_rows=(0, 0), mip_rows=(0, 0)):
        self._check(self.lib.sah_copy_scene_bloom_mip0_rows(self.handle, C.byref(lit), C.byref(out), C.byref(chain), aa_rows[0], aa_rows[1], mip_rows[0], mip_rows[1]))

    def bloom(self, scene, chain):
        self._check(self.lib.sah_bloom(self.handle, C.byref(scene), C.byref(chain)))

    def bloom_mip0_rows(self, scene, chain, row_begin, row_end):
        self._check(self.lib.sah_bloom_mip0_rows(self.handle, C.byref(scene), C.byref(chain), row_begin, row_end))

    def bloom_mip_rows(self, scene, chain, mip, row_begin, row_end):
        self._check(self.lib.sah_bloom_mip_rows(self.handle, C.byref(scene), C.byref(chain), mip, row_begin, row_end))

    def bloom_from_mip(self, scene, chain, mip):
        self._check(self.lib.sah_bloom_from_mip(self.handle, C.byref(scene), C.byref(chain), mip))

    def bloom_from_mip0(self, scene, chain):
        self._check(self.lib.sah_bloom_from_mip0(self.handle, C.byref(scene), C.byref(chain)))

    def tonemap(self, scene, chain, out, row_begin=0, row_end=0, flags=0):
        self._check(self.lib.sah_tonemap_ex(self.handle, C.byref(scene), C.byref(chain), C.byref(out), row_begin, row_end, flags))

    def lpv_clear(self, red, green, blue, geometry, num_cascades):
        null = C.POINTER(_abi.Volume)()
        args = [C.byref(v) if v is not None else null for v in (red, green, blue, geometry)]
        self._check(self.lib.sah_lpv_clear(self.handle, *args, num_cascades))

    def lpv_propagate(self, a_rgb, b_rgb, num_cascades, steps):
        a = (_abi.Volume * 3)(*a_rgb)
        b = (_abi.Volume * 3)(*b_rgb)
        self._check(self.lib.sah_lpv_propagate(self.handle, a, b, num_cascades, steps))

    def lpv_inject_rsm_gv(self, rsm, cascades, first_cascade, cascade_count, num_cascades, geometry):
        self._check(self.lib.sah_lpv_inject_rsm_gv(self.handle, C.byref(rsm), cascades, first_cascade, cascade_count, num_cascades, C.byref(geometry)))

    def lpv_inject_scene_gv(self, depth, normals, view, cascades, num_cascades, geometry):
        self._check(self.lib.sah_lpv_inject_scene_gv(self.handle, C.byref(depth), C.byref(normals), C.byref(view), cascades, num_cascades, C.byref(geometry)))

    def lpv_propagate_gv(self, a_rgb, b_rgb, geometry, num_cascades, steps):
        a = (_abi.Volume * 3)(*a_rgb)
        b = (_abi.Volume * 3)(*b_rgb)
        g = C.byref(geometry) if geometry is not None else C.POINTER(_abi.Volume)()
        self._check(self.lib.sah_lpv_propagate_gv(self.handle, a, b, g, num_cascades, steps))

    def lpv_emissive_vpls(self, geometry, primitive_index, positions_ptr, points_ptr, num_points, flags, out_ptr):
        self._check(self.lib.sah_lpv_emissive_vpls(self.handle, C.byref(geometry), primitive_index, C.c_void_p(positions_ptr), C.c_void_p(points_ptr),
                                                   num_points, flags, C.c_void_p(out_ptr)))

    def lpv_inject_emissive(self, geometry, clouds, cascades, bounds, num_cascades, a_rgb):
        table = (EmissiveCloud * max(len(clouds), 1))(*clouds)
        a = (_abi.Volume * 3)(*a_rgb)
        self._check(self.lib.sah_lpv_inject_emissive(self.handle, C.byref(geometry), table, len(clouds), cascades, bounds, num_cascades, a))

    def sky_update_luts(self, transmittance, multiscattering, sky_view, light_vector):
        lv = (C.c_float * 3)(*[float(v) for v in light_vector])
        self._check(self.lib.sah_sky_update_luts(self.handle, C.byref(transmittance), C.byref(multiscattering), C.byref(sky_view), lv))

    def ao_clear(self, ao):
        self._check(self.lib.sah_ao_clear(self.handle, C.byref(ao)))

    def probe_copy(self, src, dst, cascade_movement):
        mv = ((C.c_float * 3) * 4)(*[(C.c_float * 3)(*[float(v) for v in row]) for row in cascade_movement])
        self._check(self.lib.sah_probe_copy(self.handle, C.byref(src), C.byref(dst), mv))

    def probe_update(self, atlases, trace_results, probes_to_update_ptr, num_probes):
        self._check(self.lib.sah_probe_update(self.handle, C.byref(atlases), C.byref(trace_results), C.c_void_p(probes_to_update_ptr), num_probes))

    def probe_notify_updated(self, probe_irradiance, probes_ptr, num_probes):
        self._check(self.lib.sah_probe_notify_updated(self.handle, C.byref(probe_irradiance), C.c_void_p(probes_ptr), num_probes))

    def shadow_render(self, scene, sun, num_cascades, shadowmap, stats_ptr=None):
        self._check(self.lib.sah_shadow_render(self.handle, C.byref(scene), C.byref(sun), num_cascades, C.byref(shadowmap), C.c_void_p(stats_ptr)))

    def gbuffer_render(self, scene, view, gbuffer, stats_ptr=None):
        self._check(self.lib.sah_gbuffer_render(self.handle, C.byref(scene), C.byref(view), C.byref(gbuffer), C.c_void_p(stats_ptr)))

    def motion_vectors_render(self, scene, view, depth, out, stats=None):
        self._check(self.lib.sah_motion_vectors_render(self.handle, C.byref(scene), C.byref(view), C.byref(depth), C.byref(out), C.c_void_p(stats)))

    def gbuffer_motion_render(self, scene, view, gbuffer, out, stats=None):
        self._check(self.lib.sah_gbuffer_motion_render(self.handle, C.byref(scene), C.byref(view), C.byref(gbuffer), C.byref(out), C.c_void_p(stats)))

    RASTER_PASS_FIELDS = ("attempts", "record_capacity", "clip_capacity", "pairs_capacity")

    def raster_last_pass(self):
        out = (C.c_uint32 * len(self.RASTER_PASS_FIELDS))()
        self._check(self.lib.sah_debug_raster_last_pass(self.handle, out))
        return {k: int(v) for k, v in zip(self.RASTER_PASS_FIELDS, out)}

    def vrsaa_measure_aliasing(self, color, depth, contrast, rows=(0, 0)):
        self._check(self.lib.sah_vrsaa_measure_aliasing(self.handle, C.byref(color), C.byref(depth), C.byref(contrast), rows[0], rows[1]))

    def taa_resolve(self, lit, depth, motion_vectors, history, out, params, rows=(0, 0)):
        self._check(self.lib.sah_taa_resolve(self.handle, C.byref(lit), C.byref(depth), C.byref(motion_vectors), None if history is None else C.byref(history),
                                             C.byref(out), C.byref(params), rows[0], rows[1]))

    def taa_upscale(self, lit, depth, motion_vectors, history, out, params, rows=(0, 0)):
        self._check(self.lib.sah_taa_upscale(self.handle, C.byref(lit), C.byref(depth), C.byref(motion_vectors), None if history is None else C.byref(history),
                                             C.byref(out), C.byref(params), rows[0], rows[1]))

    def ssao(self, view_data, depth, normals, scratch, ao_out, params, rows=(0, 0)):
        self._check(self.lib.sah_ssao(self.handle, C.byref(view_data), C.byref(depth), C.byref(normals), None if scratch is None else C.byref(scratch),
                                      C.byref(ao_out), C.byref(params), rows[0], rows[1]))

    def rt_denoise(self, view_data, desc, params, rows=(0, 0)):
        self._check(self.lib.sah_rt_denoise(self.handle, C.byref(view_data), C.byref(desc), C.byref(params), rows[0], rows[1]))

    def rtgi_denoise(self, view_data, desc, params, rows=(0, 0)):
        self._check(self.lib.sah_rtgi_denoise(self.handle, C.byref(view_data), C.byref(desc), C.byref(params), rows[0], rows[1]))

    def exposure_meter(self, scene, state_in, state_out, work, exposed_out, params):
        self._check(self.lib.sah_exposure_meter(self.handle, C.byref(scene), C.c_void_p(state_in), C.c_void_p(state_out), C.c_void_p(work),
                                                None if exposed_out is None else C.byref(exposed_out), C.byref(params)))

    def exposure_apply(self, scene, state, out, rows=(0, 0)):
        self._check(self.lib.sah_exposure_apply(self.handle, C.byref(scene), C.c_void_p(state), C.byref(out), rows[0], rows[1]))

    def vrsaa_shading_rate_image(self, contrast, sri, params):
        self._check(self.lib.sah_vrsaa_shading_rate_image(self.handle, C.byref(contrast), C.byref(sri), C.byref(params)))

    def mip_chain_generate(self, src, levels):
        arr = (_abi.Plane * len(levels))(*levels)
        self._check(self.lib.sah_mip_chain_generate(self.handle, C.byref(src), arr, len(levels)))

    def rsm_render(self, scene, sun, cascades, num_cascades, rsm, stats_ptr=None):
        self._check(self.lib.sah_rsm_render(self.handle, C.byref(scene), C.byref(sun), cascades, num_cascades, C.byref(rsm), C.c_void_p(stats_ptr)))

    def lpv_extract_vpls(self, rsm, cascades, cascade_index, grid_cell_size, vpl_list_ptr, vpl_count_ptr):
        self._check(self.lib.sah_lpv_extract_vpls(self.handle, C.byref(rsm), cascades, cascade_index, grid_cell_size, C.c_void_p(vpl_list_ptr),
                                                  C.c_void_p(vpl_count_ptr)))

    def lpv_inject_vpls(self, vpl_list_ptr, vpl_count_ptr, capacity, cascades, cascade_index, num_cascades, rgb):
        vols = (_abi.Volume * 3)(*rgb)
        self._check(self.lib.sah_lpv_inject_vpls(self.handle, C.c_void_p(vpl_list_ptr), C.c_void_p(vpl_count_ptr), capacity, cascades, cascade_index,
                                                 num_cascades, vols))

    def rt_build(self, scene):
        stats = (C.c_uint32 * _abi.RT_STATS_WORDS)()
        self._check(self.lib.sah_rt_build(self.handle, C.byref(scene), stats))
        self._rt_scene = scene
        return list(stats)

    def rt_refit(self, scene, stats_ptr=None):
        self._check(self.lib.sah_rt_refit(self.handle, C.byref(scene), C.c_void_p(stats_ptr)))
        self._rt_scene = scene

    def rtao(self, view, depth, normals, noise, samples_per_pixel, max_ray_distance, ao_out):
        self._check(self.lib.sah_rtao(self.handle, C.byref(view), C.byref(depth), C.byref(normals), C.byref(noise), samples_per_pixel, max_ray_distance,
                                      C.byref(ao_out)))

    def sun_shadow_mask(self, view, sun, depth, normals, noise, mask_out):
        self._check(self.lib.sah_sun_shadow_mask(self.handle, C.byref(view), C.byref(sun), C.byref(depth), C.byref(normals), C.byref(noise), C.byref(mask_out)))

    def rt_set_rows(self, row_begin=0, row_end=0):
        self._check(self.lib.sah_rt_set_rows(self.handle, row_begin, row_end))

    def rt_set_bounces(self, num_bounces=0):
        self._check(self.lib.sah_rt_set_bounces(self.handle, num_bounces))

    def rt_structure(self):
        header = (C.c_uint32 * RT_STRUCTURE_HEADER_WORDS)()
        self._check(self.lib.sah_debug_rt_structure(self.handle, header, None, 0, None, 0))
        num_tris, num_levels, groups = int(header[0]), int(header[1]), int(header[2])
        tris, nodes = np.zeros(num_tris, RT_TRIANGLE), np.zeros((groups, 2, 3, 4), np.float32)
        self._check(self.lib.sah_debug_rt_structure(self.handle, header, tris.ctypes.data, tris.nbytes, nodes.ctypes.data, nodes.nbytes))
        assert (int(header[0]), int(header[1]), int(header[2])) == (num_tris, num_levels, groups)
        return {"num_tris": num_tris, "num_levels": num_levels, "pad_bits": int(header[3]),
                "level_offset": [int(v) for v in header[4:4 + num_levels]],
                "level_count": [int(v) for v in header[4 + RT_MAX_LEVELS:4 + RT_MAX_LEVELS + num_levels]],
                "header": [int(v) for v in header], "tris": tris, "nodes": nodes}

    def probe_trace(self, desc):
        self._check(self.lib.sah_probe_trace(self.handle, C.byref(desc)))

    def rtgi_trace(self, view, sun, sky, depth, normals, noise, ray_buffer, ray_irradiance):
        self._check(self.lib.sah_rtgi_trace(self.handle, C.byref(view), C.byref(sun), C.byref(sky), C.byref(depth), C.byref(normals), C.byref(noise),
                                            C.byref(ray_buffer), C.byref(ray_irradiance)))

    def allgather_rows(self, image, rows_per_rank, allocated_rows=None):
        self._check(self.lib.sah_allgather_rows(self.handle, C.byref(image), rows_per_rank, image.height if allocated_rows is None else allocated_rows))

    def allgather_rows_reversed(self, image, rows_per_rank, allocated_rows=None):
        self._check(self.lib.sah_allgather_rows_reversed(self.handle, C.byref(image), rows_per_rank,
                                                         image.height if allocated_rows is None else allocated_rows))

    def comm_set_stream(self, hip_stream_handle):
        self._check(self.lib.sah_comm_set_stream(self.handle, C.c_void_p(hip_stream_handle)))

    def comm_wait(self):
        self._check(self.lib.sah_comm_wait(self.handle))

    def ipc_open(self):
        buf = C.create_string_buffer(_abi.IPC_HANDLE_BYTES)
        self._check(self.lib.sah_ipc_open(self.handle, buf))
        return buf.raw

    def ipc_connect(self, handles):
        self._check(self.lib.sah_ipc_connect(self.handle, C.create_string_buffer(b"".join(handles), len(handles) * _abi.IPC_HANDLE_BYTES)))

    def ipc_export(self, device_ptr, nbytes):
        buf = C.create_string_buffer(_abi.IPC_HANDLE_BYTES)
        self._check(self.lib.sah_ipc_export(self.handle, C.c_void_p(device_ptr), nbytes, buf))
        return buf.raw

    def ipc_register(self, device_ptr, nbytes, handles):
        self._check(self.lib.sah_ipc_register(self.handle, C.c_void_p(device_ptr), nbytes,
                                              C.create_string_buffer(b"".join(handles), len(handles) * _abi.IPC_HANDLE_BYTES)))

    def ipc_unregister(self, device_ptr):
        self._check(self.lib.sah_ipc_unregister(self.handle, C.c_void_p(device_ptr)))

    def ipc_reset(self):
        self._check(self.lib.sah_ipc_reset(self.handle))

    def allgather_bytes(self, device_ptr, bytes_per_rank):
        self._check(self.lib.sah_allgather_bytes(self.handle, C.c_void_p(device_ptr), bytes_per_rank))

    def chain_create(self, plan, frames, tonemap_flags, chain_flags, work_stream, reduce_stream, post_stream):
        h = C.c_void_p()
        self._check(self.lib.sah_chain_create(self.handle, C.byref(plan), frames, tonemap_flags, chain_flags, C.c_void_p(work_stream),
                                              C.c_void_p(reduce_stream) if reduce_stream else None, C.c_void_p(post_stream) if post_stream else None, C.byref(h)))
        return h

    def chain_submit(self, chain, begin_event=None, end_event=None):
        self._check(self.lib.sah_chain_submit(chain, C.c_void_p(begin_event) if begin_event else None, C.c_void_p(end_event) if end_event else None))

    def chain_flush(self, chain):
        self._check(self.lib.sah_chain_flush(chain))

    def chain_graphs(self, chain):
        out = (C.c_uint64 * 3)()
        self._check(self.lib.sah_debug_chain_graphs(chain, out))
        if out[2]:
            print("[sah] " + self.lib.sah_last_error(self.handle).decode())
        return int(out[0]), int(out[1]), int(out[2])

    def chain_destroy(self, chain):
        self.lib.sah_chain_destroy(chain)

    def close(self):
        if getattr(self, "handle", None):
            self.lib.sah_destroy(self.handle)
            self.handle = None

    def __del__(self):
        try:
            self.close()
        except Exception:
            pass


def comm_unique_id():
    lib = load()
    buf = C.create_string_buffer(128)
    rc = lib.sah_comm_unique_id(buf)
    if rc != _abi.SAH_OK:
        raise SahError(rc, lib.sah_status_string(rc).decode())
    return buf.raw
```

Measured before the change: 60030.

## Shade stray deferred pixels inline in fast lighting kernel, skipping fixup launch

Adds a mode where the sky-enabled fast lighting kernel shades its own listed (deferred) pixels per wavefront at the end, so the separate fixup kernel launch can be skipped. A host-pinned record tracks, through kernel-written call counters, whether recent calls with the same key ran clean, and enables the inline path automatically after several stable calls when the stream is not being captured. This removes a second kernel launch and its grid-wide hint check. The cost is extra host-side bookkeeping, system-scope atomics from the GPU to host memory, and a heuristic that depends on earlier calls having completed.

```diff
diff --git a/androidrenderer_amd/_abi.py b/androidrenderer_amd/_abi.py
--- a/androidrenderer_amd/_abi.py
+++ b/androidrenderer_amd/_abi.py
@@ -29,6 +29,7 @@
 LIGHTING_DEFAULT_FLAGS = LIGHTING_QUIRK_SUN_BLEND
 MAX_BLOOM_MIPS = 8
 TONEMAP_TOLERANCE_1CODE = 1 << 0
+DEBUG_STRAYS_AUTO, DEBUG_STRAYS_LAUNCH, DEBUG_STRAYS_INLINE = 0, 1, 2
 GENERATION_TRACKED = 0xFFFFFFFF
 
 
diff --git a/androidrenderer_amd/csrc/api.cpp b/androidrenderer_amd/csrc/api.cpp
--- a/androidrenderer_amd/csrc/api.cpp
+++ b/androidrenderer_amd/csrc/api.cpp
@@ -50,9 +50,9 @@
 
 enum DispatchField {
     kDispFamily, kDispPpt, kDispPosDivNr, kDispNcascPow2, kDispRowMagic, kDispSkyRatio, kDispSkyWorkgroups, kDispTiledFastGeom, kDispTiledFastLpv,
-    kDispRepack, kDispTableRebuilt, kDispPosDivShared, kDispFields
+    kDispRepack, kDispTableRebuilt, kDispPosDivShared, kDispStrays, kDispFields
 };
-static_assert(kDispFields == sizeof(sah_ctx::last_dispatch) / sizeof(uint32_t), "sah_debug_lighting_dispatch reports uint32_t[12]");
+static_assert(kDispFields == sizeof(sah_ctx::last_dispatch) / sizeof(uint32_t), "sah_debug_lighting_dispatch reports uint32_t[13]");
 
 struct LightingCall {
     uint32_t W, H, r0, r1;
@@ -442,6 +442,22 @@
     return SAH_OK;
 }
 
+int lighting_strays(sah_ctx* ctx, const LightingCall& call, const SkyArgs& sky, int ppt, FastArgs& fast) {
+    fast.strays_record = ctx->strays.rec;
+    fast.strays_inline = 0u;
+    if (!lighting_fast_finishes_strays(sky.enabled != 0u) || call.r1 <= call.r0) return SAH_OK;
+    hipStreamCaptureStatus capturing = hipStreamCaptureStatusNone;
+    if (hipStreamIsCapturing(ctx->stream, &capturing) != hipSuccess) {
+        (void)hipGetLastError();
+        return SAH_OK;
+    }
+    if (capturing != hipStreamCaptureStatusNone) return SAH_OK;
+    const uint32_t key[7] = {call.sun_mode, call.gi_kind, (uint32_t)ppt, sky.enabled, call.W, call.r0, call.r1};
+    const bool predicted_clean = ctx->strays.take(key);
+    fast.strays_inline = ctx->force_strays == 0 ? (predicted_clean ? 1u : 0u) : (ctx->force_strays == 2 ? 1u : 0u);
+    return SAH_OK;
+}
+
 void lighting_report(sah_ctx* ctx, const LightingCall& call, const FastPath& path, int ppt, const FastArgs& fast, bool table_rebuilt) {
     uint32_t* w = ctx->last_dispatch;
     w[kDispFamily] = path.family;
@@ -456,6 +472,7 @@
     w[kDispRepack] = fast.repack;
     w[kDispTableRebuilt] = table_rebuilt ? 1u : 0u;
     w[kDispPosDivShared] = fast.pos_div_shared;
+    w[kDispStrays] = path.use_fast ? 1u + fast.strays_inline : 0u;
 }
 
 }
@@ -535,6 +552,7 @@
         sah_destroy(ctx);
         return SAH_ERR_HIP;
     }
+    ctx->strays.create();
     const char* mc = getenv("SAH_RASTER_MERGE_CAPACITY");
     if (mc) ctx->raster_merge_cap = (uint32_t)atoi(mc);
     *out = ctx;
@@ -570,6 +588,7 @@
     for (SahBuffer* b : buffers) b->release();
     ctx->tm_codes.release();
     ctx->mip_chain_counter.release();
+    ctx->strays.release();
     for (SahCacheGuard* g : {&ctx->guard_lighting, &ctx->guard_tonemap, &ctx->guard_raster, &ctx->guard_rt, &ctx->guard_mip_chain})
         if (g->done) (void)hipEventDestroy(g->done);
     if (ctx->raster.half_to_srgb8) (void)hipFree(ctx->raster.half_to_srgb8);
@@ -593,10 +612,12 @@
 
 void* sah_get_stream(sah_ctx* ctx) { return ctx ? (void*)ctx->stream : nullptr; }
 
-int sah_debug_set(sah_ctx* ctx, int force_general, int force_ppt) {
+int sah_debug_set(sah_ctx* ctx, int force_general, int force_ppt, int strays) {
     if (!ctx) return SAH_ERR_INVALID_ARGUMENT;
+    if (strays < 0 || strays > 2) return fail(ctx, SAH_ERR_INVALID_ARGUMENT, "strays must be 0 (auto), 1 (launch) or 2 (inline), not %d", strays);
     ctx->force_general = force_general != 0;
     ctx->force_ppt = force_ppt;
+    ctx->force_strays = strays;
     return SAH_OK;
 }
 
@@ -627,7 +648,7 @@
     return SAH_OK;
 }
 
-int sah_debug_lighting_dispatch(sah_ctx* ctx, uint32_t out[12]) {
+int sah_debug_lighting_dispatch(sah_ctx* ctx, uint32_t out[13]) {
     if (!ctx || !out) return SAH_ERR_INVALID_ARGUMENT;
     memcpy(out, ctx->last_dispatch, sizeof(ctx->last_dispatch));
     if (out[sah::kDispPosDivShared] && ctx->state) {
@@ -682,6 +703,7 @@
     }
     if (path.use_fast) {
         if (const int rc = lighting_fast_layout(ctx, d, call, ppt, lpv, sky, fast); rc != SAH_OK) return rc;
+        if (const int rc = lighting_strays(ctx, call, sky, ppt, fast); rc != SAH_OK) return rc;
     }
     bool table_rebuilt = false;
     if (const int rc = lighting_colx_table(ctx, call, a, path, ppt, fast, &table_rebuilt); rc != SAH_OK) return rc;
diff --git a/androidrenderer_amd/csrc/ctx.hpp b/androidrenderer_amd/csrc/ctx.hpp
--- a/androidrenderer_amd/csrc/ctx.hpp
+++ b/androidrenderer_amd/csrc/ctx.hpp
@@ -36,6 +36,7 @@
     bool comm_pending = false;
     int force_ppt = 0;
     bool force_general = false;
+    int force_strays = 0;
     sah::FrameState* state = nullptr;
     SahBuffer list;
     SahBuffer gv_keys;
@@ -47,12 +48,13 @@
     SahKeyedTable tm_axis;
     SahTonemapCodeTables tm_codes;
     SahTicketCounter mip_chain_counter;
+    SahStraysRecord strays;
     uint64_t cache_epoch = 0;
     uint32_t hint_slot = 0;
     uint32_t dbg_lpv_packs = 0, dbg_irr_unpacks = 0;
     const uint16_t* last_seg_count = nullptr;
     uint32_t last_num_segments = 0;
-    uint32_t last_dispatch[12] = {};
+    uint32_t last_dispatch[13] = {};
     struct RasterScratch {
         SahBuffer buf[16];
         uint8_t* half_to_srgb8 = nullptr;
diff --git a/androidrenderer_amd/csrc/ctx_cache.hpp b/androidrenderer_amd/csrc/ctx_cache.hpp
--- a/androidrenderer_amd/csrc/ctx_cache.hpp
+++ b/androidrenderer_amd/csrc/ctx_cache.hpp
@@ -182,6 +182,44 @@
     }
 };
 
+struct SahStraysRecord {
+    static constexpr uint32_t kCleanCalls = 4;
+    sah::StraysRecord* rec = nullptr;
+    uint32_t issued = 0;
+    uint32_t key[7] = {};
+    uint32_t key_first = 0;
+    bool have_key = false;
+
+    void create() {
+        if (hipHostMalloc((void**)&rec, sizeof(sah::StraysRecord)) != hipSuccess) {
+            (void)hipGetLastError();
+            rec = nullptr;
+            return;
+        }
+        rec->started = rec->listed = 0;
+    }
+    bool take(const uint32_t (&k)[7]) {
+        if (!rec) return false;
+        const uint32_t started = __atomic_load_n(&rec->started, __ATOMIC_RELAXED), listed = __atomic_load_n(&rec->listed, __ATOMIC_RELAXED);
+        auto ahead = [](uint32_t a, uint32_t b) { return (int32_t)(a - b); };
+        if (ahead(started, issued) > 0) {
+            issued = started;
+            have_key = false;
+        }
+        if (!have_key || memcmp(k, key, sizeof(key)) != 0) {
+            memcpy(key, k, sizeof(key));
+            key_first = issued + 1;
+            have_key = true;
+        }
+        issued++;
+        return ahead(started, key_first) >= (int32_t)kCleanCalls - 1 && ahead(started, listed) >= (int32_t)kCleanCalls;
+    }
+    void release() {
+        if (rec) (void)hipHostFree(rec);
+        rec = nullptr;
+    }
+};
+
 struct SahTonemapCodeTables {
     float* thresholds = nullptr;
     float* code_table = nullptr;
diff --git a/androidrenderer_amd/csrc/launch.hpp b/androidrenderer_amd/csrc/launch.hpp
--- a/androidrenderer_amd/csrc/launch.hpp
+++ b/androidrenderer_amd/csrc/launch.hpp
@@ -25,6 +25,7 @@
                            hipStream_t st);
 hipError_t launch_lighting_tiled(const LightingArgs& a, const CsmArgs& csm, const LpvArgs& lpv, const CacheArgs& cache, const RtgiArgs& rtgi,
                                  const SkyArgs& sky, int sun_mode, int gi, bool brute_force_lights, const FastArgs* fast, hipStream_t st);
+bool lighting_fast_finishes_strays(bool sky_bound);
 hipError_t launch_colx_table(const LightingArgs& a, const FastArgs& f, float* out, uint32_t stride, uint32_t row_stride, hipStream_t st);
 hipError_t launch_probe_irr_unpack(const VolumeArg& src, uint8_t* dst, hipStream_t st);
 hipError_t launch_probe_irr_unpack_probes(const VolumeArg& src, uint8_t* dst, const uint32_t* probes, uint32_t num_probes, hipStream_t st);
diff --git a/androidrenderer_amd/csrc/lighting.hip b/androidrenderer_amd/csrc/lighting.hip
--- a/androidrenderer_amd/csrc/lighting.hip
+++ b/androidrenderer_amd/csrc/lighting.hip
@@ -61,10 +61,35 @@
 
 constexpr uint32_t kFixupSegs = 16;
 constexpr uint32_t kFixupMaxWorkgroups = 2048;
+
+template <int SUN, int GI, int PPT, bool SKY_FILL = true>
+SAH_DEV void shade_listed_pixel(const LightingArgs& a, const CsmArgs& csm, const LpvArgs& lpv, const SkyArgs& sky, const FastArgs& f, uint32_t seg,
+                                uint32_t code, const float* s_lut) {
+    const uint32_t g = seg * 64u + code / PPT;
+    const FastPixel at = fast_pixel_of(g, a.width / PPT, a.row_end - a.row_begin, PPT, f.tile_rows, f.row_magic);
+    const uint32_t y = a.row_begin + at.row, x = at.x0 + code % PPT;
+    Px p;
+    p.color = *reinterpret_cast<const uint32_t*>(a.color.ptr + (size_t)y * a.color.pitch + (size_t)x * 4);
+    p.data = *reinterpret_cast<const uint32_t*>(a.data.ptr + (size_t)y * a.data.pitch + (size_t)x * 4);
+    p.emission = *reinterpret_cast<const uint32_t*>(a.emission.ptr + (size_t)y * a.emission.pitch + (size_t)x * 4);
+    p.depth = *reinterpret_cast<const float*>(a.depth.ptr + (size_t)y * a.depth.pitch + (size_t)x * 4);
+    const uint2 n = *reinterpret_cast<const uint2*>(a.normals.ptr + (size_t)y * a.normals.pitch + (size_t)x * 8);
+    p.n01 = n.x;
+    p.n23 = n.y;
+    p.ao = (GI == SAH_GI_LPV && a.has_ao) ? *reinterpret_cast<const float*>(a.ao.ptr + (size_t)y * a.ao.pitch + (size_t)x * 4) : 1.0f;
+    p.mask = (SUN == SAH_SHADOW_MODE_RT && a.has_mask)
+                 ? *reinterpret_cast<const float*>(a.shadow_mask.ptr + (size_t)y * a.shadow_mask.pitch + (size_t)x * 4)
+                 : 1.0f;
+    const uint2 r = shade_pixel_general<SUN, GI, SKY_FILL>(a, csm, lpv, sky, x, y, p, s_lut);
+    *reinterpret_cast<uint2*>(const_cast<uint8_t*>(a.lit.ptr) + (size_t)y * a.lit.pitch + (size_t)x * 8) = r;
+}
+
 template <int SUN, int GI, int PPT>
 __global__ void __launch_bounds__(256) k_lighting_fixup(const LightingArgs a, const CsmArgs csm, const LpvArgs lpv, const SkyArgs sky,
                                                         const FastArgs f) {
     if (__hip_atomic_load(&f.state->deferred_hint[f.hint_slot], __ATOMIC_RELAXED, __HIP_MEMORY_SCOPE_AGENT) == 0u) return;
+    if (blockIdx.x == 0u && threadIdx.x == 0u && f.strays_record)
+        __hip_atomic_store(&f.strays_record->listed, f.state->call_no[f.hint_slot ^ 1u], __ATOMIC_RELAXED, __HIP_MEMORY_SCOPE_SYSTEM);
     __shared__ uint32_t s_pref[kFixupSegs + 1];
     __shared__ float s_lut[512];
     stage_format_tables(s_lut, a.luts);
@@ -87,30 +112,13 @@
     __syncthreads();
     const uint32_t total = s_pref[kFixupSegs];
     if (total == 0) continue;
-    const uint32_t groups_per_row = a.width / PPT;
     for (uint32_t i = threadIdx.x; i < total; i += 256u) {
         uint32_t s = 0;
 #pragma unroll
         for (uint32_t step = kFixupSegs / 2; step >= 1; step >>= 1)
             if (s_pref[s + step] <= i) s += step;
         const uint32_t code = f.seg_list[(size_t)(seg0 + s) * f.seg_stride + (i - s_pref[s])];
-        const uint32_t g = (seg0 + s) * 64u + code / PPT;
-        const FastPixel at = fast_pixel_of(g, groups_per_row, a.row_end - a.row_begin, PPT, f.tile_rows, f.row_magic);
-        const uint32_t y = a.row_begin + at.row, x = at.x0 + code % PPT;
-        Px p;
-        p.color = *reinterpret_cast<const uint32_t*>(a.color.ptr + (size_t)y * a.color.pitch + (size_t)x * 4);
-        p.data = *reinterpret_cast<const uint32_t*>(a.data.ptr + (size_t)y * a.data.pitch + (size_t)x * 4);
-        p.emission = *reinterpret_cast<const uint32_t*>(a.emission.ptr + (size_t)y * a.emission.pitch + (size_t)x * 4);
-        p.depth = *reinterpret_cast<const float*>(a.depth.ptr + (size_t)y * a.depth.pitch + (size_t)x * 4);
-        const uint2 n = *reinterpret_cast<const uint2*>(a.normals.ptr + (size_t)y * a.normals.pitch + (size_t)x * 8);
-        p.n01 = n.x;
-        p.n23 = n.y;
-        p.ao = (GI == SAH_GI_LPV && a.has_ao) ? *reinterpret_cast<const float*>(a.ao.ptr + (size_t)y * a.ao.pitch + (size_t)x * 4) : 1.0f;
-        p.mask = (SUN == SAH_SHADOW_MODE_RT && a.has_mask)
-                     ? *reinterpret_cast<const float*>(a.shadow_mask.ptr + (size_t)y * a.shadow_mask.pitch + (size_t)x * 4)
-                     : 1.0f;
-        const uint2 r = shade_pixel_general<SUN, GI>(a, csm, lpv, sky, x, y, p, s_lut);
-        *reinterpret_cast<uint2*>(const_cast<uint8_t*>(a.lit.ptr) + (size_t)y * a.lit.pitch + (size_t)x * 8) = r;
+        shade_listed_pixel<SUN, GI, PPT>(a, csm, lpv, sky, f, seg0 + s, code, s_lut);
     }
     }
 }
@@ -164,7 +172,9 @@
 }
 
 
-template <int SUN, int GI, int PPT, bool SKY>
+constexpr bool strays_inline_body(bool sky) { return sky; }
+
+template <int SUN, int GI, int PPT, bool SKY, bool FINISH = false>
 __global__ void __launch_bounds__(256, SKY ? 4 : 1) k_lighting_fast(const LightingArgs a, const CsmArgs csm, const LpvArgs lpv, const SkyArgs sky,
                                                                                  const FastArgs f) {
     uint32_t block_id = blockIdx.x;
@@ -311,12 +321,28 @@
                 front += (uint32_t)__builtin_popcountll(m);
             }
         }
+        if constexpr (FINISH) {
+            static_assert(strays_inline_body(SKY), "no such body");
+            __builtin_amdgcn_fence(__ATOMIC_RELEASE, "wavefront");
+            __builtin_amdgcn_s_waitcnt(0x0f70);
+            __builtin_amdgcn_wave_barrier();
+            __builtin_amdgcn_fence(__ATOMIC_ACQUIRE, "wavefront");
+            if (lane == 0u && f.strays_record)
+                __hip_atomic_store(&f.strays_record->listed, f.state->call_no[f.hint_slot] + 1u, __ATOMIC_RELAXED, __HIP_MEMORY_SCOPE_SYSTEM);
+#pragma unroll 1
+            for (uint32_t i = lane; i < front; i += 64u) shade_listed_pixel<SUN, GI, PPT, false>(a, csm, lpv, sky, f, seg, seg_codes[i], s_lut);
+        }
     }
     if (lane == 0 && seg < f.num_segments) {
         f.seg_count[seg] = (uint16_t)front;
         if (front != 0u) f.state->deferred_hint[f.hint_slot] = 1u;
     }
-    if (gid == 0u) f.state->deferred_hint[f.hint_slot ^ 1u] = 0u;
+    if (gid == 0u) {
+        f.state->deferred_hint[f.hint_slot ^ 1u] = 0u;
+        const uint32_t call = f.state->call_no[f.hint_slot] + 1u;
+        f.state->call_no[f.hint_slot ^ 1u] = call;
+        if (f.strays_record) __hip_atomic_store(&f.strays_record->started, call, __ATOMIC_RELAXED, __HIP_MEMORY_SCOPE_SYSTEM);
+    }
 }
 
 static hipError_t launch_lpv_pack(const LpvArgs& lpv, const FastArgs& f, hipStream_t st) {
@@ -353,12 +379,14 @@
     const dim3 block(256);
     auto launch = [&](auto ppt_c) {
         constexpr int P = decltype(ppt_c)::value;
-        if (sky.enabled) hipLaunchKernelGGL((k_lighting_fast<SUN, GI, P, true>), dim3(f.sky_first + blocks), block, 0, st, a, csm, lpv, sky, f);
+        if (sky.enabled && f.strays_inline) hipLaunchKernelGGL((k_lighting_fast<SUN, GI, P, true, true>), dim3(f.sky_first + blocks), block, 0, st, a, csm, lpv, sky, f);
+        else if (sky.enabled) hipLaunchKernelGGL((k_lighting_fast<SUN, GI, P, true>), dim3(f.sky_first + blocks), block, 0, st, a, csm, lpv, sky, f);
         else hipLaunchKernelGGL((k_lighting_fast<SUN, GI, P, false>), dim3(blocks), block, 0, st, a, csm, lpv, sky, f);
     };
     if (ppt == 4) launch(std::integral_constant<int, 4>{});
     else if (ppt == 2) launch(std::integral_constant<int, 2>{});
     else launch(std::integral_constant<int, 1>{});
+    if (f.strays_inline && strays_inline_body(sky.enabled != 0u)) return hipGetLastError();
     const uint32_t fgroups = (f.num_segments + kFixupSegs - 1) / kFixupSegs;
     const dim3 fgrid(fgroups < kFixupMaxWorkgroups ? fgroups : kFixupMaxWorkgroups);
     if (ppt == 4) hipLaunchKernelGGL((k_lighting_fixup<SUN, GI, 4>), fgrid, block, 0, st, a, csm, lpv, sky, f);
@@ -379,6 +407,8 @@
     }
 }
 
+bool lighting_fast_finishes_strays(bool sky_bound) { return strays_inline_body(sky_bound); }
+
 hipError_t launch_colx_table(const LightingArgs& a, const FastArgs& f, float* out, uint32_t stride, uint32_t row_stride, hipStream_t st) {
     const hipError_t me = hipMemsetAsync(&f.state->colx_neg_zero, 0, sizeof(uint32_t), st);
     if (me != hipSuccess) return me;
diff --git a/androidrenderer_amd/csrc/lighting_common.hpp b/androidrenderer_amd/csrc/lighting_common.hpp
--- a/androidrenderer_amd/csrc/lighting_common.hpp
+++ b/androidrenderer_amd/csrc/lighting_common.hpp
@@ -522,7 +522,7 @@
     return r;
 }
 
-template <int SUN, int GI>
+template <int SUN, int GI, bool SKY_FILL = true>
 SAH_DEV uint2 shade_pixel_general(const LightingArgs& a, const CsmArgs& csm, const LpvArgs& lpv, const SkyArgs& sky, uint32_t x, uint32_t y,
                                   const Px& p, const float* lut) {
     Hn lit[4] = {Hn::lit(0.f), Hn::lit(0.f), Hn::lit(0.f), Hn::lit(0.f)};
@@ -559,7 +559,7 @@
         lit[2] = Hn(tof(lit[2]) + (Fn(lut[(p.emission >> 16) & 0xffu]) * e).v);
         lit[3] = Hn(tof(lit[3]) + 1.0f);
     }
-    if (sky.enabled && !surface) sky_frag(a, sky, x, y, lit);
+    if (SKY_FILL && sky.enabled && !surface) sky_frag(a, sky, x, y, lit);
     if constexpr (SUN == SAH_SHADOW_MODE_RT) {
         if (surface) {
             float add[3];
diff --git a/androidrenderer_amd/csrc/params.hpp b/androidrenderer_amd/csrc/params.hpp
--- a/androidrenderer_amd/csrc/params.hpp
+++ b/androidrenderer_amd/csrc/params.hpp
@@ -76,6 +76,11 @@
     uint32_t deferred_hint[2];
     uint32_t nonfinite;
     uint32_t colx_neg_zero;
+    uint32_t call_no[2];
+};
+
+struct StraysRecord {
+    uint32_t started, listed;
 };
 
 struct FastArgs {
@@ -98,6 +103,8 @@
     uint16_t* seg_count;
     uint32_t num_segments, seg_stride;
     uint32_t hint_slot;
+    uint32_t strays_inline;
+    StraysRecord* strays_record;
     uint32_t pos_div_shared;
     const uint8_t* lpv_packed;
     uint32_t pk_row_pitch, pk_slice_pitch;
diff --git a/androidrenderer_amd/lib.py b/androidrenderer_amd/lib.py
--- a/androidrenderer_amd/lib.py
+++ b/androidrenderer_amd/lib.py
@@ -181,7 +181,7 @@
     lib.sah_chain_destroy.argtypes = [C.c_void_p]
     lib.sah_debug_chain_graphs.argtypes = [C.c_void_p, C.POINTER(C.c_uint64)]
     lib.sah_chain_destroy.restype = None
-    lib.sah_debug_set.argtypes = [C.c_void_p, C.c_int, C.c_int]
+    lib.sah_debug_set.argtypes = [C.c_void_p, C.c_int, C.c_int, C.c_int]
     lib.sah_lpv_inject_rsm_gv.argtypes = [C.c_void_p, C.POINTER(_abi.RsmTargets), C.POINTER(_abi.LpvCascadeMatrices), C.c_uint32, C.c_uint32, C.c_uint32,
                                           C.POINTER(_abi.Volume)]
     lib.sah_lpv_inject_scene_gv.argtypes = [C.c_void_p, C.POINTER(_abi.Plane), C.POINTER(_abi.Plane), C.POINTER(_abi.ViewData),
@@ -232,8 +232,12 @@
     def set_stream(self, hip_stream_handle):
         self._check(self.lib.sah_set_stream(self.handle, C.c_void_p(hip_stream_handle)))
 
-    def debug_set(self, force_general=False, force_ppt=0):
-        self._check(self.lib.sah_debug_set(self.handle, int(force_general), int(force_ppt)))
+    STRAYS_MODES = {"auto": _abi.DEBUG_STRAYS_AUTO, "launch": _abi.DEBUG_STRAYS_LAUNCH, "inline": _abi.DEBUG_STRAYS_INLINE}
+
+    def debug_set(self, force_general=False, force_ppt=0, strays="auto"):
+        if strays not in self.STRAYS_MODES:
+            raise ValueError(f"strays must be one of {tuple(self.STRAYS_MODES)}, not {strays!r}")
+        self._check(self.lib.sah_debug_set(self.handle, int(force_general), int(force_ppt), self.STRAYS_MODES[strays]))
 
     def deferred_pixels(self):
         n = C.c_uint64()
@@ -251,13 +255,14 @@
         return int(e.value)
 
     DISPATCH_FIELDS = ("family", "ppt", "pos_div_nr", "ncasc_pow2", "row_magic", "sky_ratio", "sky_workgroups", "tiled_fast_geom", "tiled_fast_lpv",
-                       "repack", "table_rebuilt", "pos_div_shared")
+                       "repack", "table_rebuilt", "pos_div_shared", "strays")
 
     def lighting_dispatch(self):
         out = (C.c_uint32 * len(self.DISPATCH_FIELDS))()
         self._check(self.lib.sah_debug_lighting_dispatch(self.handle, out))
         rep = {k: int(v) for k, v in zip(self.DISPATCH_FIELDS, out)}
         rep["family"] = ("general", "fast", "tiled")[rep["family"]]
+        rep["strays"] = (None, "launch", "inline")[rep["strays"]]
         return rep
 
     def sync(self):
```

Result: faster. 60930, median of 6 (+1.5%).
